# yxyxcyx/Real-Time-Recommendation-System-with-Feature-Store

Hardware: AMD Instinct MI355X
Metric: user-item pairs scored/sec (train) + top-K queries/sec, emb_dim=128 (higher is better)
Workload: dtype f32; 1 GPU; C2: MovieLens-1M two-tower train step, emb 128, batch 1024, 16 negatives, hidden [256,128], dropout 0.2, tau 0.05, Adam+clip; global_batch=1024, emb_dim=128, num_negatives=16, parallelism=dp1

## Files before the change

### include/rtrec_hip.h

```cpp
#ifndef RTREC_HIP_H
#define RTREC_HIP_H

#include <stddef.h>
#include <stdint.h>

#ifdef __cplusplus
extern "C" {
#endif

typedef enum {
    RT_OK = 0,
    RT_ERR_INVALID = -1,
    RT_ERR_UNSUPPORTED = -2,
    RT_ERR_WORKSPACE = -3,
    RT_ERR_HIP = -4
} rt_status;

typedef enum { RT_F32 = 0, RT_F16 = 1, RT_BF16 = 2 } rt_dtype;

typedef enum {
    RT_ACT_RELU = 0,
    RT_ACT_GELU = 1,
    RT_ACT_LEAKY_RELU = 2,
    RT_ACT_TANH = 3,
    RT_ACT_SIGMOID = 4,
    RT_ACT_NONE = 5
} rt_act;

int rt_abi_version(void);
const char* rt_status_string(int status);
const char* rt_last_error(void);

int rt_gather_rows(const void* table, int64_t row_begin, int64_t n_rows, int64_t row_bytes,
                   const int64_t* ids, int64_t n_ids, void* out, int32_t* oob_count, void* stream);

int rt_scatter_add_rows_f32(float* grad_table, int64_t n_rows, int dim, const int64_t* ids,
                            int64_t n_ids, const float* grad_out, int64_t padding_idx, void* stream);

int rt_l2_renorm_f32(float* x, int64_t n, int d, void* stream);

size_t rt_flatip_topk_workspace_bytes(int64_t nq, int64_t nx, int d, int dtype, int k);
int rt_flatip_topk(const void* queries, int64_t nq, const void* items, int64_t nx, int d, int dtype,
                   int k, const uint32_t* exclude_bits, int64_t exclude_words, int64_t id_offset,
                   float* out_scores, int64_t* out_ids, void* workspace, size_t workspace_bytes,
                   void* stream);

size_t rt_flatip_topk_shard_workspace_bytes(int64_t nq, int64_t nx, int d, int dtype, int k);
int rt_flatip_topk_shard_plan(int64_t nq, int64_t nx, int d, int dtype, int k, int stride, int64_t* stage_counts);
int rt_flatip_topk_shard_sample(const void* queries, int64_t nq, const void* items, int64_t nx, int d, int dtype,
                                int k, int stride, float* top32, int64_t* stage_counts, void* workspace,
                                size_t workspace_bytes, void* stream);
int rt_topk_sample_rank(int k, int64_t sampled_stages, int64_t stages, int* rank);
int rt_topk_sample_threshold(const float* lists, int n_lists, int64_t nq, int rank, float* thr, void* stream);
int rt_flatip_topk_shard_search(const void* queries, int64_t nq, const void* items, int64_t nx, int d, int dtype,
                                int k, const float* thr, int64_t id_offset, float* out_scores, int64_t* out_ids,
                                void* workspace, size_t workspace_bytes, void* stream);

int rt_flatip_topk_tuning(int v4_mode, int v4_stride, int v4_rank);

int rt_l2_augment_f32(const float* x, int64_t n, int d, float* out, int ld_out, int role, void* stream);
int rt_l2_finish_f32(const float* q_aug, int ld_q, const float* x_aug, int ld_x, int d, int64_t nq, int k_sel,
                     const int64_t* sel_ids, const float* sel_scores, int k, float* scores, int64_t* ids,
                     int32_t* unverified, int64_t id_offset, void* stream);

int rt_topk_merge(const float* scores, const int64_t* ids, int64_t nq, int n_lists, int k_in,
                  int k_out, float* out_scores, int64_t* out_ids, void* stream);

int rt_sample_negatives(const int64_t* pos_offsets, const int32_t* pos_items, int64_t n_users,
                        const int64_t* users, int64_t n, int64_t num_items, int num_neg, uint64_t seed,
                        const uint64_t* seed_offset, int64_t* out, void* stream);

int rt_feeder_batch(const int64_t* order, const int64_t* inter_u, const int64_t* inter_m, const int64_t* state,
                    int64_t batch, int64_t* users, int64_t* pos, void* stream);
int rt_feeder_commit(const double* loss, double* losses, int64_t n_losses, int64_t* state, void* stream);

#ifndef RT_STAT_SLOTS
#define RT_STAT_SLOTS 8
#endif
#if RT_STAT_SLOTS > 15
#error "RT_STAT_SLOTS > 15: the host arenas (rtrec_amd/models/fused.py STAT_SLOTS) hold 16 slot rows, one of them for ticket counters"
#endif

typedef struct {
    const float* src;
    int64_t src_rows;
    int ld_src;
    const int64_t* ids;
    int64_t m;
    int k;
    int n;
    const float* w;
    const float* bias;
    int prev_mode;
    int prev_act;
    const double* prev_stats;
    const float* bn_gamma;
    const float* bn_beta;
    float* running_mean;
    float* running_var;
    float* save_mean;
    float* save_invstd;
    float bn_eps;
    float bn_momentum;
    float drop_p;
    uint64_t drop_seed;
    const uint64_t* seed_offset;
    float* z_out;
    int act;
    double* stats_out;
    float* l2_out;
    float* norms_out;
    int64_t* num_batches_tracked;
    int64_t seg_split;
    double* zero_buf;
    int64_t zero_words;
    float* wt_out;
    float* a_out;
    float* fin_save_mean;
    float* fin_save_invstd;
    float* fin_running_mean;
    float* fin_running_var;
    int64_t* fin_num_batches_tracked;
    float fin_eps;
    float fin_momentum;
    int prev_final;
    const uint16_t* w_planes;
    uint16_t* wt_planes_out;
    const float* next_w;
    uint16_t* next_w_planes;
    int next_n;
    int next_k;
} rt_linear_fwd_args;

int rt_linear_fwd_f32(const rt_linear_fwd_args* args, void* stream);

typedef struct {
    int64_t m; int k; int n;
    const float* w;
    float* dw;
    float* dbias;
    float* dz_ws;
    int grad_mode;
    const float* dout;
    const float* l2_out;
    const float* norms;
    const float* g;
    const float* z;
    int act;
    const double* g_stats;
    const float* save_mean;
    const float* save_invstd;
    const float* bn_gamma;
    float* dgamma;
    float* dbeta;
    const float* src; int64_t src_rows; int ld_src; const int64_t* ids;
    int prev_mode; int prev_act;
    const float* prev_mean; const float* prev_invstd;
    const float* prev_gamma; const float* prev_beta;
    float prev_drop_p; uint64_t prev_drop_seed; const uint64_t* seed_offset;
    float* g_prev;
    double* g_prev_stats;
    float* dsrc;
    int64_t seg_split;
    double* dbias_slots;
    const float* wt;
    int fuse_dz;
    const float* a_in;
    float* dw_part;
    const float* fold_src;
    float* fold_dst;
    int64_t fold_words;
    int fold_splits;
    int fold_in;
    const uint16_t* wt_planes;
} rt_linear_bwd_args;

int rt_linear_bwd_f32(const rt_linear_bwd_args* args, void* stream);
int rt_linear_bwd_dz_fused(const rt_linear_bwd_args* args, int n_args);
int rt_linear_bwd_dw_splits(const rt_linear_bwd_args* args, int n_args, int64_t* splits);
int rt_linear_bwd_dz_f32(const rt_linear_bwd_args* args, void* stream);
int rt_linear_bwd_dw_f32(const rt_linear_bwd_args* args, void* stream);
int rt_linear_fwd_f32_multi(const rt_linear_fwd_args* args, int n_args, void* stream);
int rt_linear_bwd_dz_f32_multi(const rt_linear_bwd_args* args, int n_args, void* stream);
int rt_linear_bwd_dw_f32_multi(const rt_linear_bwd_args* args, int n_args, void* stream);

size_t rt_twotower_loss_workspace_bytes(int64_t b, int d);
int rt_twotower_loss_fwd_bwd(const void* u, const void* p, const void* q, int dtype, int64_t b,
                             int d, int n_neg, float inv_tau, const float* user_bias,
                             const float* item_bias, float w_explicit, float w_in_batch,
                             double* loss_out, float* du, float* dp, float* dq, float* d_user_bias,
                             float* d_item_bias, void* workspace, size_t workspace_bytes, void* stream);

int rt_twotower_loss_fwd(const void* u, const void* p, const void* q, int dtype, int64_t b, int d,
                         int n_neg, float inv_tau, const float* user_bias, const float* item_bias,
                         float w_explicit, float w_in_batch, double* loss_out, void* workspace,
                         size_t workspace_bytes, void* stream);

size_t rt_inbatch_loss_workspace_bytes(int64_t b, int64_t n_items, int d);
int rt_inbatch_loss_fwd_bwd(const void* u, const void* p, int dtype, int64_t b, int64_t n_items, int d,
                            int64_t label_offset, float inv_tau, double* loss_out, float* du, float* dp,
                            void* workspace, size_t workspace_bytes, void* stream);

int rt_similarity_f32(const float* u, const float* v, int64_t b, int d, float inv_tau,
                      const float* user_bias, const float* item_bias, float* out, void* stream);

int rt_grad_sqnorm(const float* grads, const int64_t* offsets, int n_tensors, double* sumsq_out,
                   int32_t* step_counter, int64_t* seed_counter, void* stream);
int rt_clip_adam_step(float* params, float* grads, float* exp_avg, float* exp_avg_sq,
                      int64_t n, const double* sumsq, int n_tensors, float max_norm, float lr,
                      const float* lr_dev, float beta1, float beta2, float eps, float weight_decay,
                      int step, const int32_t* step_dev, double* zero_buf, int64_t zero_words,
                      void* stream);

#define RT_METRICS_MAX_K 16

int rt_exclusion_bitmap(const int64_t* offsets, const int32_t* items, int64_t n_csr_rows, const int64_t* rows,
                        int64_t n_rows, int64_t n_items, uint32_t* bits, int64_t words, void* stream);
int rt_rank_metrics(const int64_t* preds, int64_t n_rows, int list_len, const int64_t* gt_offsets,
                    const int32_t* gt_items, const int64_t* gt_rows, int64_t n_gt_rows,
                    const int64_t* ex_offsets, const int32_t* ex_items, const int64_t* ex_rows,
                    int64_t n_ex_rows, const int32_t* k_values, int n_k, int64_t num_items,
                    double* per_row, int32_t* valid, uint32_t* coverage_bits, void* stream);
int rt_rank_metrics_reduce(const double* per_row, const int32_t* valid, int64_t n_rows, int n_cols,
                           const uint32_t* coverage_bits, int64_t num_items, double* out, void* stream);

#ifdef __cplusplus
}
#endif

#endif
```

### real-time-recommendation-system-with-feature-store_amd/csrc/mlp.hip

```cpp
#include "rt_common.h"
#include "split3.h"

namespace rt {
namespace mlp {

typedef float f32x16 __attribute__((ext_vector_type(16)));



constexpr float kNormEps = 1e-12f;

struct FwdLaunch {
    rt_linear_fwd_args a0, a1;
    unsigned split;
};
struct BwdLaunch {
    rt_linear_bwd_args a0, a1;
    unsigned split;
    int64_t rps0, rps1;
    unsigned tn0, tk0, tn1, tk1;
    bool vec0, vec1;
    int ngroups;
    unsigned ksplit = 1;
};

constexpr int kFoldG = 8;
__device__ __forceinline__ void fold_side(const BwdLaunch& L, int which) {
    const int64_t nt = static_cast<int64_t>(gridDim.x) * blockDim.x;
    const int64_t gt = static_cast<int64_t>(blockIdx.x) * blockDim.x + threadIdx.x;
    for (int g = 0; g < L.ngroups; ++g) {
        const rt_linear_bwd_args& f = g ? L.a1 : L.a0;
        if (!f.fold_src || f.fold_in != which || f.fold_splits <= 0) continue;
        const int64_t n4 = f.fold_words / 4;
        const int ng = (f.fold_splits + kFoldG - 1) / kFoldG;
        for (int64_t it = gt; it < n4 * ng; it += nt) {
            const int64_t e = it % n4;
            const int s0 = static_cast<int>(it / n4) * kFoldG;
            float4 v[kFoldG];
#pragma unroll
            for (int j = 0; j < kFoldG; ++j)
                v[j] = s0 + j < f.fold_splits
                           ? reinterpret_cast<const float4*>(f.fold_src + static_cast<int64_t>(s0 + j) * f.fold_words)[e]
                           : make_float4(0.f, 0.f, 0.f, 0.f);
            float4 t = v[0];
#pragma unroll
            for (int j = 1; j < kFoldG; ++j) { t.x += v[j].x; t.y += v[j].y; t.z += v[j].z; t.w += v[j].w; }
            float* d = f.fold_dst + 4 * e;
            if (ng == 1) {
                const float4 o = *reinterpret_cast<const float4*>(d);
                *reinterpret_cast<float4*>(d) = make_float4(o.x + t.x, o.y + t.y, o.z + t.z, o.w + t.w);
            } else {
                atomicAdd(d, t.x); atomicAdd(d + 1, t.y); atomicAdd(d + 2, t.z); atomicAdd(d + 3, t.w);
            }
        }
    }
}


#ifdef RT_PHASE_PROBE
__device__ unsigned long long* g_probe_buf = nullptr;
__device__ unsigned int g_probe_ctr[64];
__device__ unsigned int g_probe_cap = 0;
struct PhaseProbe {
    uint64_t rt0 = 0, t0 = 0, m[4] = {0, 0, 0, 0};
    __device__ __forceinline__ void start() {
        if (threadIdx.x == 0) {
            rt0 = __builtin_amdgcn_s_memrealtime();
            t0 = __builtin_amdgcn_s_memtime();
        }
    }
    __device__ __forceinline__ void mark(int i) {
        if (threadIdx.x == 0) m[i] = __builtin_amdgcn_s_memtime() - t0;
    }
    __device__ __forceinline__ void end(unsigned tag) {
        if (threadIdx.x == 0) {
            asm volatile("s_waitcnt vmcnt(0)" ::: "memory");
            m[3] = __builtin_amdgcn_s_memtime() - t0;
            const uint64_t rt1 = __builtin_amdgcn_s_memrealtime();
            const unsigned xcc = __builtin_amdgcn_s_getreg((20) | (0 << 6) | ((4 - 1) << 11));
            const unsigned sh = blockIdx.x & 63u;
            const unsigned slot = atomicAdd(&g_probe_ctr[sh], 1u);
            if (slot < g_probe_cap && g_probe_buf) {
                unsigned long long* o = g_probe_buf + (static_cast<uint64_t>(slot) * 64 + sh) * 8;
                o[0] = (static_cast<uint64_t>(tag) << 32) | blockIdx.x;
                o[1] = rt0; o[2] = m[0]; o[3] = m[1]; o[4] = m[2]; o[5] = m[3]; o[6] = rt1; o[7] = xcc;
            }
        }
    }
};
#define RT_PP_DECL PhaseProbe pp_; pp_.start();
#define RT_PP_MARK(i) pp_.mark(i);
#define RT_PP_END(tag) pp_.end(tag);
#else
#define RT_PP_DECL
#define RT_PP_MARK(i)
#define RT_PP_END(tag)
#endif

#if !defined(RT_NO_WT_STORES)
#define RT_WT_STORES 1
#endif
__device__ __forceinline__ void st_act(float* p, float v) {
#ifdef RT_WT_STORES
    __hip_atomic_store(p, v, __ATOMIC_RELAXED, __HIP_MEMORY_SCOPE_AGENT);
#else
    *p = v;
#endif
}
__device__ __forceinline__ void st_act4(float* p, float4 v) {
#ifdef RT_WT_STORES
    typedef float f4v __attribute__((ext_vector_type(4)));
    const f4v x = {v.x, v.y, v.z, v.w};
    asm volatile("global_store_dwordx4 %0, %1, off sc1" ::"v"(p), "v"(x) : "memory");
#else
    *reinterpret_cast<float4*>(p) = v;
#endif
}

__device__ __forceinline__ f32x16 mfma(float a, float b, f32x16 c) {
    return __builtin_amdgcn_mfma_f32_32x32x2f32(a, b, c, 0, 0, 0);
}

using fsplit::Pieces;
using fsplit::s16x8;
using fsplit::split8;
using fsplit::mfma3;
using fsplit::split3;

struct Pro {
    int mode;
    int act;
    float drop_p, drop_scale;
    uint64_t seed;
    const float* scale;
    const float* shift;
};

__device__ __forceinline__ float pro_apply(const Pro& p, int64_t r, int c, float v) {
    if (p.mode == 0) return v;
    v = act_eval(p.act, v);
    if (p.mode != 3) v = __builtin_fmaf(v, p.scale[c], p.shift[c]);
    if (p.drop_p > 0.f) v = dropout_keep(p.seed, r, c, p.drop_p) ? v * p.drop_scale : 0.f;
    return v;
}

__device__ __forceinline__ void slot_sums(const double* __restrict__ base, int w, int c, double& s1, double& s2) {
    double v1[RT_STAT_SLOTS], v2[RT_STAT_SLOTS];
#pragma unroll
    for (int sl = 0; sl < RT_STAT_SLOTS; ++sl) {
        v1[sl] = base[static_cast<int64_t>(sl) * 2 * w + c];
        v2[sl] = base[static_cast<int64_t>(sl) * 2 * w + w + c];
    }
    s1 = 0.0;
    s2 = 0.0;
#pragma unroll
    for (int sl = 0; sl < RT_STAT_SLOTS; ++sl) {
        s1 += v1[sl];
        s2 += v2[sl];
    }
}

__device__ __forceinline__ void bn_affine(float gamma, float beta, float mean, float invstd, float& scale,
                                          float& shift) {
    scale = gamma * invstd;
    shift = __builtin_fmaf(-mean, scale, beta);
}

__device__ __forceinline__ void ticket_release() {
#ifdef RT_TICKET_WBL2
    __builtin_amdgcn_fence(__ATOMIC_RELEASE, "agent");
#endif
    asm volatile("s_waitcnt vmcnt(0)" ::: "memory");
}

__device__ __forceinline__ void bn_finalize_last(const rt_linear_fwd_args& a, unsigned nblk) {
    __shared__ int last_s;
    const int tid = threadIdx.x, n = a.n;
    const bool two = a.seg_split > 0;
    const int nseg = two ? 2 : 1;
    asm volatile("s_waitcnt vmcnt(0)" ::: "memory");
    __syncthreads();
    if (tid == 0) {
        ticket_release();
        unsigned long long* cnt =
            reinterpret_cast<unsigned long long*>(a.stats_out + static_cast<int64_t>(nseg) * RT_STAT_SLOTS * 2 * n);
        last_s = atomicAdd(cnt, 1ull) == static_cast<unsigned long long>(nblk) - 1ull ? 1 : 0;
    }
    __syncthreads();
    if (!last_s) return;
    for (int c = tid; c < n; c += blockDim.x) {
        for (int sg = 0; sg < nseg; ++sg) {
            const int64_t ms = two ? (sg == 0 ? a.seg_split : a.m - a.seg_split) : a.m;
            double* ps = a.stats_out + static_cast<int64_t>(sg) * RT_STAT_SLOTS * 2 * n;
            double v1[RT_STAT_SLOTS], v2[RT_STAT_SLOTS];
#pragma unroll
            for (int sl = 0; sl < RT_STAT_SLOTS; ++sl) {
                v1[sl] = atomicAdd(&ps[static_cast<int64_t>(sl) * 2 * n + c], 0.0);
                v2[sl] = atomicAdd(&ps[static_cast<int64_t>(sl) * 2 * n + n + c], 0.0);
            }
            double s1 = 0.0, s2 = 0.0;
#pragma unroll
            for (int sl = 0; sl < RT_STAT_SLOTS; ++sl) {
                s1 += v1[sl];
                s2 += v2[sl];
            }
            const double md = s1 / static_cast<double>(ms);
            double vd = s2 / static_cast<double>(ms) - md * md;
            vd = vd > 0.0 ? vd : 0.0;
            const float mean = static_cast<float>(md);
            const float invstd = static_cast<float>(1.0 / sqrt(vd + static_cast<double>(a.fin_eps)));
            const float var_f = static_cast<float>(ms > 1 ? vd * static_cast<double>(ms) / static_cast<double>(ms - 1) : vd);
            a.fin_save_mean[sg * n + c] = mean;
            if (a.fin_save_invstd) a.fin_save_invstd[sg * n + c] = invstd;
            if (a.fin_running_mean) {
                const float mo = a.fin_momentum;
                a.fin_running_mean[c] = (1.f - mo) * a.fin_running_mean[c] + mo * mean;
                a.fin_running_var[c] = (1.f - mo) * a.fin_running_var[c] + mo * var_f;
            }
        }
    }
    if (tid == 0 && a.fin_num_batches_tracked) *a.fin_num_batches_tracked += nseg;
}

constexpr int FM = 32;

__host__ __device__ __forceinline__ int pad8(int k) { return (k + 31) / 32 * 32; }

template <int TPW, bool KVEC, bool WPL>
__global__ __launch_bounds__(256) __attribute__((amdgpu_waves_per_eu(TPW == 1 ? 3 : 2))) void linear_fwd_kernel(FwdLaunch L) {
    static_assert(!WPL || (TPW == 1 && KVEC), "split-weight planes: one-tile waves, k % 4 == 0");
    const bool g1 = blockIdx.x >= L.split;
    const rt_linear_fwd_args& a = g1 ? L.a1 : L.a0;
    const unsigned bid = blockIdx.x - (g1 ? L.split : 0u);
    constexpr int NT = 4 * TPW;
    extern __shared__ __attribute__((aligned(16))) float sm[];
    const int k = a.k, n = a.n;
    const int kp = pad8(k), aplane = FM * kp, aw = 3 * aplane / 2;
    const int nch = kp / 8, am = ((nch & -nch) < 16 ? (nch & -nch) : 16) - 1;
    float* scale = sm;
    float* shift = scale + kp;
    float* As = shift + kp;
    uint16_t* const Ap = reinterpret_cast<uint16_t*>(As);
    float* rowpart = As + aw;
    int64_t* srow = reinterpret_cast<int64_t*>(rowpart + NT * FM);

    const int tid = threadIdx.x, lane = tid & 63, w = tid >> 6, h = lane >> 5, c32 = lane & 31;
    const int64_t row0 = static_cast<int64_t>(bid) * FM;
    const int64_t m = a.m;
    auto put_a = [&](int r, int c, float4 o) {
        if (a.a_out && c < k && row0 + r < m) st_act4(a.a_out + (row0 + r) * k + c, o);
        uint32_t h0, m0, l0, h1, m1, l1;
        split3(o.x, o.y, h0, m0, l0);
        split3(o.z, o.w, h1, m1, l1);
        uint16_t* q = Ap + r * kp + ((((c >> 3) ^ (r & am)) << 3) | (c & 7));
        *reinterpret_cast<uint2*>(q) = make_uint2(h0, h1);
        *reinterpret_cast<uint2*>(q + aplane) = make_uint2(m0, m1);
        *reinterpret_cast<uint2*>(q + 2 * aplane) = make_uint2(l0, l1);
    };
    RT_PP_DECL
    if (blockIdx.x == 0 && a.zero_buf)
        for (int64_t e = tid; e < a.zero_words; e += 256) a.zero_buf[e] = 0.0;

    const int vpr = kp / 4;
    const bool vec = (a.ld_src % 4) == 0 && (reinterpret_cast<uintptr_t>(a.src) & 15) == 0;
    const bool fast = vec && (a.k % 4) == 0 && (256 % vpr) == 0 &&
                      (a.prev_mode == 0 || act_is_piecewise_linear(a.prev_act));
    const bool early = fast && !a.ids && 8 * (256 / vpr) >= FM;
    if (a.wt_out) {
        const int tk = (k + 31) / 32, tiles = tk * ((n + 31) / 32);
        const int nblk = static_cast<int>(g1 ? gridDim.x - L.split : L.split);
        for (int wt = static_cast<int>(bid); wt < tiles; wt += nblk) {
            const int n0 = (wt / tk) * 32, k0 = (wt % tk) * 32;
            const int r = tid >> 3, c = (tid & 7) * 4;
            if (n0 + r < n) {
#pragma unroll
                for (int j = 0; j < 4; ++j)
                    if (k0 + c + j < k) a.wt_out[static_cast<int64_t>(k0 + c + j) * n + n0 + r] = a.w[static_cast<int64_t>(n0 + r) * k + k0 + c + j];
            }
        }
    }
    if (a.wt_planes_out || a.next_w_planes) {
        const int nblk = static_cast<int>(g1 ? gridDim.x - L.split : L.split);
        if (a.wt_planes_out) {
            const int64_t plane = static_cast<int64_t>(n) * k;
            const int nq = (n + 3) / 4;
            for (int64_t e = static_cast<int64_t>(bid) * 256 + tid; e < static_cast<int64_t>(k) * nq;
                 e += static_cast<int64_t>(nblk) * 256) {
                const int kk = static_cast<int>(e / nq), n0 = static_cast<int>(e % nq) * 4;
                float x[4];
#pragma unroll
                for (int j = 0; j < 4; ++j) x[j] = n0 + j < n ? a.w[static_cast<int64_t>(n0 + j) * k + kk] : 0.f;
                uint32_t h0, m0, l0, h1, m1, l1;
                split3(x[0], x[1], h0, m0, l0);
                split3(x[2], x[3], h1, m1, l1);
                uint16_t* q = a.wt_planes_out + static_cast<int64_t>(kk) * n + n0;
                if (n0 + 4 <= n && (n % 4) == 0) {
                    *reinterpret_cast<uint2*>(q) = make_uint2(h0, h1);
                    *reinterpret_cast<uint2*>(q + plane) = make_uint2(m0, m1);
                    *reinterpret_cast<uint2*>(q + 2 * plane) = make_uint2(l0, l1);
                } else {
                    const uint32_t hv[2] = {h0, h1}, mv[2] = {m0, m1}, lv[2] = {l0, l1};
                    for (int j = 0; j < 4 && n0 + j < n; ++j) {
                        const int sh = 16 * (j & 1);
                        q[j] = static_cast<uint16_t>(hv[j >> 1] >> sh);
                        q[j + plane] = static_cast<uint16_t>(mv[j >> 1] >> sh);
                        q[j + 2 * plane] = static_cast<uint16_t>(lv[j >> 1] >> sh);
                    }
                }
            }
        }
        if (a.next_w_planes) {
            const int64_t tot8 = static_cast<int64_t>(a.next_n) * a.next_k / 8;
            const float4* src4 = reinterpret_cast<const float4*>(a.next_w);
            s16x8* dst = reinterpret_cast<s16x8*>(a.next_w_planes);
            for (int64_t e = static_cast<int64_t>(bid) * 256 + tid; e < tot8; e += static_cast<int64_t>(nblk) * 256) {
                const float4 u = src4[2 * e], v = src4[2 * e + 1];
                const float x[8] = {u.x, u.y, u.z, u.w, v.x, v.y, v.z, v.w};
                const Pieces pc = split8(x);
                dst[e] = pc.hi;
                dst[e + tot8] = pc.mid;
                dst[e + 2 * tot8] = pc.lo;
            }
        }
    }
    const float* wrow[TPW];
    bool tile_on[TPW], row_ok[TPW];
#pragma unroll
    for (int i = 0; i < TPW; ++i) {
        tile_on[i] = (w + 4 * i) * 32 < n;
        const int nn = (w + 4 * i) * 32 + c32;
        row_ok[i] = nn < n;
        wrow[i] = a.w + static_cast<int64_t>(row_ok[i] ? nn : 0) * k;
    }
    float4 wv[TPW][4], wn[TPW][4];
    auto load_w = [&](int s, float4 (&dst)[TPW][4]) {
#pragma unroll
        for (int i = 0; i < TPW; ++i)
#pragma unroll
            for (int j = 0; j < 4; ++j) {
                const int kk = s + 16 * (j >> 1) + 8 * h + 4 * (j & 1);
                float4 v = make_float4(0.f, 0.f, 0.f, 0.f);
                if (tile_on[i] && row_ok[i]) {
                    const float* wr = wrow[i] + kk;
                    if constexpr (KVEC) {
                        if (kk < k) v = *reinterpret_cast<const float4*>(wr);
                    } else {
                        if (kk < k) v.x = wr[0];
                        if (kk + 1 < k) v.y = wr[1];
                        if (kk + 2 < k) v.z = wr[2];
                        if (kk + 3 < k) v.w = wr[3];
                    }
                }
                dst[i][j] = v;
            }
    };
    uint4 pv[2][3], pn[2][3];
    const int64_t wplane = static_cast<int64_t>(n) * k;
    auto load_p = [&](int s, uint4 (&dst)[2][3]) {
#pragma unroll
        for (int b = 0; b < 2; ++b) {
            const int kk = s + 16 * b + 8 * h;
            const bool ok = tile_on[0] && row_ok[0] && kk < k;
            const uint16_t* q = a.w_planes + (static_cast<int64_t>(row_ok[0] ? w * 32 + c32 : 0) * k + (ok ? kk : 0));
#pragma unroll
            for (int p = 0; p < 3; ++p)
                dst[b][p] = ok ? *reinterpret_cast<const uint4*>(q + p * wplane) : make_uint4(0u, 0u, 0u, 0u);
        }
    };
    if constexpr (WPL) load_p(0, pn);
    else if constexpr (TPW == 1) load_w(0, wn);
    float4 pre[8];
    if (early) {
        const int c = (tid % vpr) * 4, rstep = 256 / vpr, r0 = tid / vpr;
#pragma unroll
        for (int u = 0; u < 8; ++u) {
            const int r = r0 + u * rstep;
            const int64_t gr = row0 + r;
            pre[u] = make_float4(0.f, 0.f, 0.f, 0.f);
            if (r < FM && c < k && gr < m && gr < a.src_rows)
                pre[u] = *reinterpret_cast<const float4*>(a.src + gr * a.ld_src + c);
        }
    }

    const bool two = a.seg_split > 0;
    const int my_seg = (two && row0 >= a.seg_split) ? 1 : 0;
    if (a.prev_mode == 1 && a.prev_final) {
        for (int c = tid; c < k; c += 256)
            bn_affine(a.bn_gamma[c], a.bn_beta[c], a.save_mean[my_seg * k + c], a.save_invstd[my_seg * k + c], scale[c],
                      shift[c]);
    } else if (a.prev_mode == 1 || a.prev_mode == 2) {
        const int nseg = two ? 2 : 1;
        for (int c = tid; c < k; c += 256) {
            for (int sg = 0; sg < nseg; ++sg) {
                if (bid != 0 && sg != my_seg) continue;
                const int64_t ms = two ? (sg == 0 ? a.seg_split : m - a.seg_split) : m;
                float mean, invstd, var_f = 0.f;
                if (a.prev_mode == 1) {
                    const double* ps = a.prev_stats + static_cast<int64_t>(sg) * RT_STAT_SLOTS * 2 * k;
                    double s1, s2;
                    slot_sums(ps, k, c, s1, s2);
                    const double md = s1 / static_cast<double>(ms);
                    double vd = s2 / static_cast<double>(ms) - md * md;
                    vd = vd > 0.0 ? vd : 0.0;
                    mean = static_cast<float>(md);
                    invstd = static_cast<float>(1.0 / sqrt(vd + static_cast<double>(a.bn_eps)));
                    var_f = static_cast<float>(ms > 1 ? vd * static_cast<double>(ms) / static_cast<double>(ms - 1) : vd);
                } else {
                    mean = a.running_mean[c];
                    invstd = static_cast<float>(1.0 / sqrt(static_cast<double>(a.running_var[c]) + a.bn_eps));
                }
                if (sg == my_seg) bn_affine(a.bn_gamma[c], a.bn_beta[c], mean, invstd, scale[c], shift[c]);
                if (bid == 0) {
                    if (c == 0 && a.prev_mode == 1 && a.num_batches_tracked) *a.num_batches_tracked += 1;
                    if (a.save_mean) a.save_mean[sg * k + c] = mean;
                    if (a.save_invstd) a.save_invstd[sg * k + c] = invstd;
                    if (a.prev_mode == 1 && a.running_mean) {
                        const float mo = a.bn_momentum;
                        a.running_mean[c] = (1.f - mo) * a.running_mean[c] + mo * mean;
                        a.running_var[c] = (1.f - mo) * a.running_var[c] + mo * var_f;
                    }
                }
            }
        }
    }
    RT_PP_MARK(0)
    if (tid < FM) {
        const int64_t gr = row0 + tid;
        int64_t sr = -1;
        if (gr < m) {
            sr = a.ids ? a.ids[gr] : gr;
            if (sr < 0 || sr >= a.src_rows) sr = -1;
        }
        srow[tid] = sr;
    }
    __syncthreads();
    const uint64_t seed = a.drop_seed + (a.seed_offset ? *a.seed_offset : 0ull);
    const Pro pro{a.prev_mode, a.prev_act, a.drop_p, a.drop_p > 0.f ? 1.f / (1.f - a.drop_p) : 1.f, seed,
                  scale, shift};
    {
        const int total = FM * vpr;
        if (fast) {
            const int c = (tid % vpr) * 4, rstep = 256 / vpr;
            const bool bn = pro.mode == 1 || pro.mode == 2;
            const float4 sc4 = bn ? *reinterpret_cast<const float4*>(scale + c) : make_float4(1.f, 1.f, 1.f, 1.f);
            const float4 sh4 = bn ? *reinterpret_cast<const float4*>(shift + c) : make_float4(0.f, 0.f, 0.f, 0.f);
            const float sl = act_slope(pro.act);
            const bool drop = pro.drop_p > 0.f;
            for (int r0 = tid / vpr; r0 < FM; r0 += 8 * rstep) {
                float4 v[8];
#pragma unroll
                for (int u = 0; u < 8; ++u) {
                    const int r = r0 + u * rstep;
                    v[u] = make_float4(0.f, 0.f, 0.f, 0.f);
                    if (early) {
                        v[u] = pre[u];
                    } else if (r < FM && c < k) {
                        const int64_t sr = srow[r];
                        if (sr >= 0) v[u] = *reinterpret_cast<const float4*>(a.src + sr * a.ld_src + c);
                    }
                }
#pragma unroll
                for (int u = 0; u < 8; ++u) {
                    const int r = r0 + u * rstep;
                    if (r >= FM) break;
                    const int64_t gr = row0 + r;
                    const bool ok = srow[r] >= 0 && c < k;
                    auto tf = [&](float x, int cc, float scv, float shv) {
                        if (pro.mode == 0) return x;
                        x = act_pwl(sl, x);
                        if (bn) x = __builtin_fmaf(x, scv, shv);
                        if (drop) x = dropout_keep(pro.seed, gr, cc, pro.drop_p) ? x * pro.drop_scale : 0.f;
                        return x;
                    };
                    float4 o;
                    o.x = ok ? tf(v[u].x, c, sc4.x, sh4.x) : 0.f;
                    o.y = ok ? tf(v[u].y, c + 1, sc4.y, sh4.y) : 0.f;
                    o.z = ok ? tf(v[u].z, c + 2, sc4.z, sh4.z) : 0.f;
                    o.w = ok ? tf(v[u].w, c + 3, sc4.w, sh4.w) : 0.f;
                    put_a(r, c, o);
                }
            }
        } else
        for (int base = tid; base < total; base += 256 * 4) {
            float4 v[4];
#pragma unroll
            for (int u = 0; u < 4; ++u) {
                const int e = base + u * 256;
                v[u] = make_float4(0.f, 0.f, 0.f, 0.f);
                if (e < total) {
                    const int r = e / vpr, c = (e - r * vpr) * 4;
                    const int64_t sr = srow[r];
                    if (sr >= 0 && c < k) {
                        const float* sp = a.src + sr * a.ld_src + c;
                        if (vec && c + 4 <= k) v[u] = *reinterpret_cast<const float4*>(sp);
                        else {
                            v[u].x = sp[0];
                            if (c + 1 < k) v[u].y = sp[1];
                            if (c + 2 < k) v[u].z = sp[2];
                            if (c + 3 < k) v[u].w = sp[3];
                        }
                    }
                }
            }
#pragma unroll
            for (int u = 0; u < 4; ++u) {
                const int e = base + u * 256;
                if (e < total) {
                    const int r = e / vpr, c = (e - r * vpr) * 4;
                    const bool ok = srow[r] >= 0;
                    const int64_t gr = row0 + r;
                    float4 o;
                    o.x = (ok && c < k) ? pro_apply(pro, gr, c, v[u].x) : 0.f;
                    o.y = (ok && c + 1 < k) ? pro_apply(pro, gr, c + 1, v[u].y) : 0.f;
                    o.z = (ok && c + 2 < k) ? pro_apply(pro, gr, c + 2, v[u].z) : 0.f;
                    o.w = (ok && c + 3 < k) ? pro_apply(pro, gr, c + 3, v[u].w) : 0.f;
                    put_a(r, c, o);
                }
            }
        }
    }
    __syncthreads();
    RT_PP_MARK(1)

    f32x16 acc[TPW];
#pragma unroll
    for (int i = 0; i < TPW; ++i) acc[i] = f32x16{};
    const uint16_t* ap = Ap + c32 * kp;
    const int asw = c32 & am;
    if constexpr (TPW != 1) load_w(0, wn);
    if constexpr (WPL) {
        for (int s = 0; s < kp; s += 32) {
#pragma unroll
            for (int b = 0; b < 2; ++b)
#pragma unroll
                for (int p = 0; p < 3; ++p) pv[b][p] = pn[b][p];
            if (s + 32 < kp) load_p(s + 32, pn);
#pragma unroll
            for (int b = 0; b < 2; ++b) {
                const int ao = (((s + 16 * b) >> 3) + h) ^ asw;
                Pieces pa;
                pa.hi = *reinterpret_cast<const s16x8*>(ap + 8 * ao);
                pa.mid = *reinterpret_cast<const s16x8*>(ap + aplane + 8 * ao);
                pa.lo = *reinterpret_cast<const s16x8*>(ap + 2 * aplane + 8 * ao);
                if (tile_on[0]) {
                    const Pieces pb{__builtin_bit_cast(s16x8, pv[b][0]), __builtin_bit_cast(s16x8, pv[b][1]),
                                    __builtin_bit_cast(s16x8, pv[b][2])};
                    acc[0] = mfma3(pa, pb, acc[0]);
                }
            }
        }
    } else
    for (int s = 0; s < kp; s += 32) {
#pragma unroll
        for (int i = 0; i < TPW; ++i)
#pragma unroll
            for (int j = 0; j < 4; ++j) wv[i][j] = wn[i][j];
        if (s + 32 < kp) load_w(s + 32, wn);
#pragma unroll
        for (int b = 0; b < 2; ++b) {
            const int ao = (((s + 16 * b) >> 3) + h) ^ asw;
            Pieces pa;
            pa.hi = *reinterpret_cast<const s16x8*>(ap + 8 * ao);
            pa.mid = *reinterpret_cast<const s16x8*>(ap + aplane + 8 * ao);
            pa.lo = *reinterpret_cast<const s16x8*>(ap + 2 * aplane + 8 * ao);
#pragma unroll
            for (int i = 0; i < TPW; ++i) {
                if (!tile_on[i]) continue;
                const float4 u = wv[i][2 * b], v = wv[i][2 * b + 1];
                const float x[8] = {u.x, u.y, u.z, u.w, v.x, v.y, v.z, v.w};
                acc[i] = mfma3(pa, split8(x), acc[i]);
            }
        }
    }

    RT_PP_MARK(2)
    const bool l2 = a.l2_out != nullptr;
    if (l2 && !a.z_out && !a.stats_out && n * (FM + 1) <= aw) {
        __syncthreads();
        float* zsq = As;
#pragma unroll
        for (int i = 0; i < TPW; ++i) {
            const int col = (w + 4 * i) * 32 + c32;
            if ((w + 4 * i) * 32 >= n) continue;
            const bool col_ok = col < n;
            const float b = (col_ok && a.bias) ? a.bias[col] : 0.f;
#pragma unroll
            for (int r = 0; r < 16; ++r) {
                const int lr = (r & 3) + 8 * (r >> 2) + 4 * h;
                const float z = acc[i][r] + b;
                acc[i][r] = z;
                if (col_ok) zsq[col * (FM + 1) + lr] = (row0 + lr < m) ? z * z : 0.f;
            }
        }
        __syncthreads();
        {
            const int row = tid >> 3, part = tid & 7;
            float ss = 0.f;
            for (int c = part; c < n; c += 8) ss += zsq[c * (FM + 1) + row];
            ss += __shfl_xor(ss, 1, 64);
            ss += __shfl_xor(ss, 2, 64);
            ss += __shfl_xor(ss, 4, 64);
            if (part == 0) {
                const float nrm = sqrtf(ss);
                rowpart[row] = 1.f / fmaxf(nrm, kNormEps);
                if (row0 + row < m && a.norms_out) a.norms_out[row0 + row] = nrm;
            }
        }
        __syncthreads();
#pragma unroll
        for (int i = 0; i < TPW; ++i) {
            const int col = (w + 4 * i) * 32 + c32;
            if ((w + 4 * i) * 32 >= n) continue;
#pragma unroll
            for (int r = 0; r < 16; ++r) {
                const int lr = (r & 3) + 8 * (r >> 2) + 4 * h;
                const int64_t gr = row0 + lr;
                if (gr < m && col < n) st_act(a.l2_out + gr * n + col, acc[i][r] * rowpart[lr]);
            }
        }
        RT_PP_END(1)
        return;
    }
    double* const stats = a.stats_out ? a.stats_out + (static_cast<int64_t>(my_seg) * RT_STAT_SLOTS +
                                                       bid % RT_STAT_SLOTS) * 2 * n : nullptr;
#pragma unroll
    for (int i = 0; i < TPW; ++i) {
        const int ct = w + 4 * i;
        const int col = ct * 32 + c32;
        const bool col_ok = col < n;
        const float b = (col_ok && a.bias) ? a.bias[col] : 0.f;
        float s1 = 0.f, s2 = 0.f;
        if (row0 + FM <= m && a.z_out && !l2 && act_is_piecewise_linear(a.act)) {
            if (ct * 32 >= n) continue;
            float* zp = a.z_out + (row0 + 4 * h) * n + col;
            const float sl = act_slope(a.act);
#pragma unroll
            for (int r = 0; r < 16; ++r) {
                const float z = acc[i][r] + b;
                if (col_ok) st_act(zp + ((r & 3) + 8 * (r >> 2)) * n, z);
                const float av = act_pwl(sl, z);
                s1 += av;
                s2 += av * av;
            }
            if (!col_ok) s1 = s2 = 0.f;
        } else
#pragma unroll
        for (int r = 0; r < 16; ++r) {
            const int lr = (r & 3) + 8 * (r >> 2) + 4 * h;
            const int64_t gr = row0 + lr;
            const float z = acc[i][r] + b;
            acc[i][r] = z;
            const bool ok = col_ok && gr < m;
            if (ok && a.z_out) st_act(a.z_out + gr * n + col, z);
            if (ok && stats) {
                const float av = act_eval(a.act, z);
                s1 += av;
                s2 += av * av;
            }
            if (l2) {
                float q = ok ? z * z : 0.f;
#pragma unroll
                for (int o = 1; o < 32; o <<= 1) q += __shfl_xor(q, o, 64);
                if (c32 == 0) rowpart[ct * FM + lr] = q;
            }
        }
        if (stats) {
            s1 += __shfl_xor(s1, 32, 64);
            s2 += __shfl_xor(s2, 32, 64);
            if (h == 0 && col_ok) {
                atomicAdd(&stats[col], static_cast<double>(s1));
                atomicAdd(&stats[n + col], static_cast<double>(s2));
            }
        }
    }
    if (stats && a.fin_save_mean) bn_finalize_last(a, g1 ? gridDim.x - L.split : L.split);
    if (l2) {
        __syncthreads();
        const int nt_used = (n + 31) / 32;
#pragma unroll
        for (int i = 0; i < TPW; ++i) {
            const int col = (w + 4 * i) * 32 + c32;
#pragma unroll
            for (int r = 0; r < 16; ++r) {
                const int lr = (r & 3) + 8 * (r >> 2) + 4 * h;
                const int64_t gr = row0 + lr;
                if (gr < m && col < n) {
                    float ss = 0.f;
                    for (int t = 0; t < nt_used; ++t) ss += rowpart[t * FM + lr];
                    const float nrm = sqrtf(ss);
                    a.l2_out[gr * n + col] = acc[i][r] / fmaxf(nrm, kNormEps);
                    if (col == 0 && a.norms_out) a.norms_out[gr] = nrm;
                }
            }
        }
    }
    RT_PP_END(1)
}

template <int TPWK, bool WPL, bool KS>
__global__ __launch_bounds__(256) __attribute__((amdgpu_waves_per_eu(3))) void linear_bwd_dz_kernel(BwdLaunch L) {
#ifdef RT_FOLD_FIRST
    fold_side(L, 0);
#endif
    const unsigned kpart = KS ? blockIdx.x % L.ksplit : 0u, bx = KS ? blockIdx.x / L.ksplit : blockIdx.x;
    const bool prim = kpart == 0;
    const int tb = static_cast<int>(kpart) * 4 * TPWK;
    const bool g1 = bx >= L.split;
    const rt_linear_bwd_args& a = g1 ? L.a1 : L.a0;
    const unsigned bid = bx - (g1 ? L.split : 0u);
    extern __shared__ __attribute__((aligned(16))) float sm[];
    const int n = a.n, k = a.k;
    const int64_t m = a.m;
    const int np = pad8(n), ldz = np + 4;
    float* Dz = sm;
    const int tid = threadIdx.x, lane = tid & 63, w = tid >> 6, h = lane >> 5, c32 = lane & 31;
    const int64_t row0 = static_cast<int64_t>(bid) * FM;
    const bool two = a.seg_split > 0;
    const int my_seg = (two && row0 >= a.seg_split) ? 1 : 0;
    const int64_t seg_m = two ? (my_seg == 0 ? a.seg_split : m - a.seg_split) : m;
    RT_PP_DECL

    float wv[TPWK][8], wn[TPWK][8];
    const float* __restrict__ Wt = a.w;
#ifdef RT_NO_WT_ROWS
    const float* __restrict__ WtT = nullptr;
#else
    const float* __restrict__ WtT = (a.wt && (n % 8) == 0) ? a.wt : nullptr;
#endif
    auto load_w = [&](int s, float (&dst)[TPWK][8]) {
#pragma unroll
        for (int i = 0; i < TPWK; ++i) {
            const int kk = (tb + w + 4 * i) * 32 + c32;
            const bool on = (tb + w + 4 * i) * 32 < k && kk < k;
            if (WtT) {
                const int nn = s + 8 * h;
                float4 v0 = make_float4(0.f, 0.f, 0.f, 0.f), v1 = v0;
                if (on && nn < n) {
                    const float* p = WtT + static_cast<int64_t>(kk) * n + nn;
                    v0 = *reinterpret_cast<const float4*>(p);
                    v1 = *reinterpret_cast<const float4*>(p + 4);
                }
                dst[i][0] = v0.x; dst[i][1] = v0.y; dst[i][2] = v0.z; dst[i][3] = v0.w;
                dst[i][4] = v1.x; dst[i][5] = v1.y; dst[i][6] = v1.z; dst[i][7] = v1.w;
            } else {
#pragma unroll
                for (int j = 0; j < 8; ++j) {
                    const int nn = s + 8 * h + j;
                    dst[i][j] = (on && nn < n) ? Wt[static_cast<int64_t>(nn) * k + kk] : 0.f;
                }
            }
        }
    };
    uint4 pv[TPWK][3], pn[TPWK][3];
    const uint16_t* __restrict__ WtP = a.wt_planes;
    const int64_t tplane = static_cast<int64_t>(k) * n;
    auto load_p = [&](int s, uint4 (&dst)[TPWK][3]) {
#pragma unroll
        for (int i = 0; i < TPWK; ++i) {
            const int kk = (tb + w + 4 * i) * 32 + c32;
            const int nn = s + 8 * h;
            const bool ok = (tb + w + 4 * i) * 32 < k && kk < k && nn < n;
            const uint16_t* q = WtP + (ok ? static_cast<int64_t>(kk) * n + nn : 0);
#pragma unroll
            for (int p = 0; p < 3; ++p)
                dst[i][p] = ok ? *reinterpret_cast<const uint4*>(q + p * tplane) : make_uint4(0u, 0u, 0u, 0u);
        }
    };
    if constexpr (TPWK == 1) {
        if (a.g_prev || a.dsrc) {
            if constexpr (WPL) load_p(0, pn);
            else load_w(0, wn);
        }
    }

    const int l4 = n / 4;
    if (a.grad_mode == 0 && (n % 4) == 0 && l4 <= 64 && (l4 & (l4 - 1)) == 0 && np == n) {
        const int rpp = 64 / l4, sub = lane / l4, li = lane % l4, c = 4 * li;
        float4 lv[8], dv[8];
        float nr[8];
#pragma unroll
        for (int p = 0; p < 8; ++p) {
            const int r = w * 8 + p * rpp + sub;
            const int64_t gr = row0 + r;
            lv[p] = make_float4(0.f, 0.f, 0.f, 0.f);
            dv[p] = lv[p];
            nr[p] = 1.f;
            if (p * rpp < 8 && gr < m) {
                lv[p] = *reinterpret_cast<const float4*>(a.l2_out + gr * n + c);
                dv[p] = *reinterpret_cast<const float4*>(a.dout + gr * n + c);
                nr[p] = a.norms[gr];
            }
        }
#pragma unroll
        for (int p = 0; p < 8; ++p) {
            if (p * rpp >= 8) break;
            const int r = w * 8 + p * rpp + sub;
            const int64_t gr = row0 + r;
            float dot = lv[p].x * dv[p].x + lv[p].y * dv[p].y + lv[p].z * dv[p].z + lv[p].w * dv[p].w;
            for (int o = 1; o < l4; o <<= 1) dot += __shfl_xor(dot, o, 64);
            const bool big = nr[p] > kNormEps;
            const float inv = 1.f / (big ? nr[p] : kNormEps);
            float4 d = make_float4(0.f, 0.f, 0.f, 0.f);
            if (gr < m) {
                d.x = big ? (dv[p].x - lv[p].x * dot) * inv : dv[p].x * inv;
                d.y = big ? (dv[p].y - lv[p].y * dot) * inv : dv[p].y * inv;
                d.z = big ? (dv[p].z - lv[p].z * dot) * inv : dv[p].z * inv;
                d.w = big ? (dv[p].w - lv[p].w * dot) * inv : dv[p].w * inv;
                if (prim) st_act4(a.dz_ws + gr * n + c, d);
            }
            *reinterpret_cast<float4*>(Dz + r * ldz + c) = d;
        }
    } else if (a.grad_mode == 0) {
        for (int rr = w * 8; rr < w * 8 + 8; ++rr) {
            const int64_t gr = row0 + rr;
            if (gr < m) {
                float dot = 0.f;
                for (int c = lane; c < n; c += 64) dot += a.l2_out[gr * n + c] * a.dout[gr * n + c];
                dot = wave_sum(dot);
                const float nrm = a.norms[gr];
                const bool big = nrm > kNormEps;
                const float inv = 1.f / (big ? nrm : kNormEps);
                for (int c = lane; c < np; c += 64) {
                    float dz = 0.f;
                    if (c < n) {
                        const float dv = a.dout[gr * n + c];
                        dz = big ? (dv - a.l2_out[gr * n + c] * dot) * inv : dv * inv;
                        if (prim) a.dz_ws[gr * n + c] = dz;
                    }
                    Dz[rr * ldz + c] = dz;
                }
            } else {
                for (int c = lane; c < np; c += 64) Dz[rr * ldz + c] = 0.f;
            }
        }
    } else {
        float* cA = Dz + FM * ldz;
        float* cB = cA + np;
        float* cC = cB + np;
        float* cM = cC + np;
        float* cI = cM + np;
        const float inv_m = 1.f / static_cast<float>(seg_m);
        const double* gst = a.g_stats ? a.g_stats + static_cast<int64_t>(my_seg) * RT_STAT_SLOTS * 2 * n : nullptr;
        const int vpr = np / 4;
        const bool vec = (n % 4) == 0;
        const bool fast = vec && (256 % vpr) == 0 && act_is_piecewise_linear(a.act) && a.grad_mode != 3;
        const bool early = fast && 8 * (256 / vpr) >= FM;
        float4 pg[8];
        if (early) {
            const int c = (tid % vpr) * 4, rstep = 256 / vpr, r0 = tid / vpr;
#pragma unroll
            for (int u = 0; u < 8; ++u) {
                const int r = r0 + u * rstep;
                const int64_t gr = row0 + r;
                pg[u] = make_float4(0.f, 0.f, 0.f, 0.f);
                if (r < FM && gr < m && c < n) pg[u] = *reinterpret_cast<const float4*>(a.g + gr * n + c);
            }
        }
        for (int c = tid; c < np; c += 256) {
            float A = 1.f, Bc = 0.f, C = 0.f, M = 0.f, I = 1.f;
            if (c < n && (a.grad_mode == 1 || a.grad_mode == 2)) {
                I = a.save_invstd[my_seg * n + c];
                M = a.save_mean[my_seg * n + c];
                A = a.bn_gamma[c] * I;
                if (a.grad_mode == 1) {
                    double gs1, gs2;
                    slot_sums(gst, n, c, gs1, gs2);
                    Bc = static_cast<float>(gs1) * inv_m;
                    C = static_cast<float>(gs2) * inv_m;
                }
            }
            cA[c] = A; cB[c] = Bc; cC[c] = C; cM[c] = M; cI[c] = I;
        }
        __syncthreads();
        const int total = FM * vpr;
        if (fast) {
            const int c = (tid % vpr) * 4, rstep = 256 / vpr;
            const float4 fA = *reinterpret_cast<const float4*>(cA + c), fB = *reinterpret_cast<const float4*>(cB + c);
            const float4 fC = *reinterpret_cast<const float4*>(cC + c), fM = *reinterpret_cast<const float4*>(cM + c);
            const float4 fI = *reinterpret_cast<const float4*>(cI + c);
            const float sl = act_slope(a.act);
            for (int r0 = tid / vpr; r0 < FM; r0 += 8 * rstep) {
                float4 gv[8], zv[8];
#pragma unroll
                for (int u = 0; u < 8; ++u) {
                    const int r = r0 + u * rstep;
                    const int64_t gr = row0 + r;
                    gv[u] = make_float4(0.f, 0.f, 0.f, 0.f);
                    zv[u] = gv[u];
                    if (early) {
                        gv[u] = pg[u];
                        if (r < FM && gr < m && c < n) zv[u] = *reinterpret_cast<const float4*>(a.z + gr * n + c);
                    } else if (r < FM && gr < m && c < n) {
                        gv[u] = *reinterpret_cast<const float4*>(a.g + gr * n + c);
                        zv[u] = *reinterpret_cast<const float4*>(a.z + gr * n + c);
                    }
                }
#pragma unroll
                for (int u = 0; u < 8; ++u) {
                    const int r = r0 + u * rstep;
                    if (r >= FM) break;
                    const int64_t gr = row0 + r;
                    auto one = [&](float g, float z, float A, float B, float C, float M, float I) {
                        const float xh = (act_pwl(sl, z) - M) * I;
                        return A * (g - B - xh * C) * (z > 0.f ? 1.f : sl);
                    };
                    float4 d;
                    d.x = one(gv[u].x, zv[u].x, fA.x, fB.x, fC.x, fM.x, fI.x);
                    d.y = one(gv[u].y, zv[u].y, fA.y, fB.y, fC.y, fM.y, fI.y);
                    d.z = one(gv[u].z, zv[u].z, fA.z, fB.z, fC.z, fM.z, fI.z);
                    d.w = one(gv[u].w, zv[u].w, fA.w, fB.w, fC.w, fM.w, fI.w);
                    if (gr >= m || c >= n) d = make_float4(0.f, 0.f, 0.f, 0.f);
                    *reinterpret_cast<float4*>(Dz + r * ldz + c) = d;
                    if (prim && gr < m && c < n) st_act4(a.dz_ws + gr * n + c, d);
                }
            }
        } else
        for (int base = tid; base < total; base += 256 * 4) {
            float4 gv[4], zv[4];
#pragma unroll
            for (int u = 0; u < 4; ++u) {
                const int e = base + u * 256;
                gv[u] = make_float4(0.f, 0.f, 0.f, 0.f);
                zv[u] = gv[u];
                if (e < total) {
                    const int r = e / vpr, c = (e - r * vpr) * 4;
                    const int64_t gr = row0 + r;
                    if (gr < m && c < n) {
                        const int64_t off = gr * n + c;
                        if (vec) {
                            gv[u] = *reinterpret_cast<const float4*>(a.g + off);
                            zv[u] = *reinterpret_cast<const float4*>(a.z + off);
                        } else {
                            gv[u].x = a.g[off]; zv[u].x = a.z[off];
                            if (c + 1 < n) { gv[u].y = a.g[off + 1]; zv[u].y = a.z[off + 1]; }
                            if (c + 2 < n) { gv[u].z = a.g[off + 2]; zv[u].z = a.z[off + 2]; }
                            if (c + 3 < n) { gv[u].w = a.g[off + 3]; zv[u].w = a.z[off + 3]; }
                        }
                    }
                }
            }
#pragma unroll
            for (int u = 0; u < 4; ++u) {
                const int e = base + u * 256;
                if (e >= total) continue;
                const int r = e / vpr, c = (e - r * vpr) * 4;
                const int64_t gr = row0 + r;
                float dzv[4];
                const float gs[4] = {gv[u].x, gv[u].y, gv[u].z, gv[u].w};
                const float zs[4] = {zv[u].x, zv[u].y, zv[u].z, zv[u].w};
#pragma unroll
                for (int j = 0; j < 4; ++j) {
                    const int cc = c + j;
                    float dz = 0.f;
                    if (gr < m && cc < n) {
                        const float xh = (act_eval(a.act, zs[j]) - cM[cc]) * cI[cc];
                        const float dr = (a.grad_mode == 3) ? gs[j] : cA[cc] * (gs[j] - cB[cc] - xh * cC[cc]);
                        dz = dr * act_grad_eval(a.act, zs[j]);
                    }
                    dzv[j] = dz;
                }
                *reinterpret_cast<float4*>(Dz + r * ldz + c) = make_float4(dzv[0], dzv[1], dzv[2], dzv[3]);
                if (prim && gr < m && c < n) {
                    const int64_t off = gr * n + c;
                    if (vec) *reinterpret_cast<float4*>(a.dz_ws + off) = make_float4(dzv[0], dzv[1], dzv[2], dzv[3]);
                    else
                        for (int j = 0; j < 4 && c + j < n; ++j) a.dz_ws[off + j] = dzv[j];
                }
            }
        }
    }
    RT_PP_MARK(0)
    if (prim && a.dbias && a.dbias_slots) {
        __syncthreads();
        double* sl = a.dbias_slots + static_cast<int64_t>(bid % RT_STAT_SLOTS) * n;
        for (int c = tid; c < n; c += 256) {
            float cs = 0.f;
#pragma unroll 8
            for (int r = 0; r < FM; ++r) cs += Dz[r * ldz + c];
            atomicAdd(&sl[c], static_cast<double>(cs));
        }
    }
    if (prim && bid == 0 && (a.grad_mode == 1 || a.grad_mode == 2) && a.dgamma) {
        for (int c = tid; c < n; c += 256) {
            for (int sg = 0; sg < (two ? 2 : 1); ++sg) {
                const double* gs = a.g_stats + static_cast<int64_t>(sg) * RT_STAT_SLOTS * 2 * n;
                double gs1, gs2;
                slot_sums(gs, n, c, gs1, gs2);
                atomicAdd(&a.dgamma[c], static_cast<float>(gs2));
                atomicAdd(&a.dbeta[c], static_cast<float>(gs1));
            }
        }
    }
    if (!a.g_prev && !a.dsrc) {
#ifndef RT_FOLD_FIRST
        fold_side(L, 0);
#endif
        RT_PP_END(2)
        return;
    }
    __syncthreads();
    RT_PP_MARK(1)

    const int ldb = np + 8;
    uint16_t* const planes = reinterpret_cast<uint16_t*>(Dz + FM * ldz + 5 * np);
    const int plane = FM * ldb;
    for (int e = tid; e < FM * (np / 4); e += 256) {
        const int r = e / (np / 4), c = (e - r * (np / 4)) * 4;
        const float4 v = *reinterpret_cast<const float4*>(Dz + r * ldz + c);
        uint32_t h0, m0, l0, h1, m1, l1;
        split3(v.x, v.y, h0, m0, l0);
        split3(v.z, v.w, h1, m1, l1);
        uint16_t* q = planes + r * ldb + c;
        *reinterpret_cast<uint2*>(q) = make_uint2(h0, h1);
        *reinterpret_cast<uint2*>(q + plane) = make_uint2(m0, m1);
        *reinterpret_cast<uint2*>(q + 2 * plane) = make_uint2(l0, l1);
    }
    __syncthreads();
    f32x16 acc[TPWK];
#pragma unroll
    for (int i = 0; i < TPWK; ++i) acc[i] = f32x16{};
    const uint16_t* ap = planes + c32 * ldb + 8 * h;
    const bool want_stats = a.g_prev && a.g_prev_stats && (a.prev_mode == 1 || a.prev_mode == 2);
    const bool fast = row0 + FM <= m && !a.dsrc && a.g_prev && act_is_piecewise_linear(a.prev_act);
    float zpre[TPWK][16], pmean[TPWK], pinv[TPWK];
#pragma unroll
    for (int i = 0; i < TPWK; ++i) {
        const int kk = (tb + w + 4 * i) * 32 + c32;
        const bool ld = fast && want_stats && kk < k;
        pmean[i] = ld ? a.prev_mean[my_seg * k + kk] : 0.f;
        pinv[i] = ld ? a.prev_invstd[my_seg * k + kk] : 0.f;
        const float* zp = a.src + (row0 + 4 * h) * a.ld_src + kk;
#pragma unroll
        for (int r = 0; r < 16; ++r) zpre[i][r] = ld ? zp[((r & 3) + 8 * (r >> 2)) * a.ld_src] : 0.f;
    }
    if constexpr (WPL) {
        if constexpr (TPWK != 1) load_p(0, pn);
        for (int s = 0; s < np; s += 16) {
#pragma unroll
            for (int i = 0; i < TPWK; ++i)
#pragma unroll
                for (int p = 0; p < 3; ++p) pv[i][p] = pn[i][p];
            if (s + 16 < np) load_p(s + 16, pn);
            Pieces pa;
            pa.hi = *reinterpret_cast<const s16x8*>(ap + s);
            pa.mid = *reinterpret_cast<const s16x8*>(ap + plane + s);
            pa.lo = *reinterpret_cast<const s16x8*>(ap + 2 * plane + s);
#pragma unroll
            for (int i = 0; i < TPWK; ++i) {
                if ((tb + w + 4 * i) * 32 >= k) continue;
                const Pieces pb{__builtin_bit_cast(s16x8, pv[i][0]), __builtin_bit_cast(s16x8, pv[i][1]),
                                __builtin_bit_cast(s16x8, pv[i][2])};
                acc[i] = mfma3(pa, pb, acc[i]);
            }
        }
    } else {
    if constexpr (TPWK != 1) load_w(0, wn);
    for (int s = 0; s < np; s += 16) {
#pragma unroll
        for (int i = 0; i < TPWK; ++i)
#pragma unroll
            for (int j = 0; j < 8; ++j) wv[i][j] = wn[i][j];
        if (s + 16 < np) load_w(s + 16, wn);
        Pieces pa;
        pa.hi = *reinterpret_cast<const s16x8*>(ap + s);
        pa.mid = *reinterpret_cast<const s16x8*>(ap + plane + s);
        pa.lo = *reinterpret_cast<const s16x8*>(ap + 2 * plane + s);
#pragma unroll
        for (int i = 0; i < TPWK; ++i) {
            if ((tb + w + 4 * i) * 32 >= k) continue;
            acc[i] = mfma3(pa, split8(wv[i]), acc[i]);
        }
    }
    }
    RT_PP_MARK(2)
    const float pscale = a.prev_drop_p > 0.f ? 1.f / (1.f - a.prev_drop_p) : 1.f;
    const uint64_t pseed = a.prev_drop_seed + (a.seed_offset ? *a.seed_offset : 0ull);
    double* const gps = want_stats ? a.g_prev_stats + (static_cast<int64_t>(my_seg) * RT_STAT_SLOTS +
                                                        bid % RT_STAT_SLOTS) * 2 * k : nullptr;
    const float psl = act_slope(a.prev_act);
#pragma unroll
    for (int i = 0; i < TPWK; ++i) {
        const int kk = (tb + w + 4 * i) * 32 + c32;
        const bool col_ok = kk < k;
        float s1 = 0.f, s2 = 0.f;
        if ((tb + w + 4 * i) * 32 >= k) continue;
        if (fast) {
            const int64_t rb = row0 + 4 * h;
            float* gp = a.g_prev + rb * k + kk;
            const float* zv = zpre[i];
            const float pm = pmean[i], pi = pinv[i];
            const bool drop = a.prev_drop_p > 0.f;
#pragma unroll
            for (int r = 0; r < 16; ++r) {
                const int lr = (r & 3) + 8 * (r >> 2);
                float gv = acc[i][r];
                if (drop) gv = dropout_keep(pseed, rb + lr, kk, a.prev_drop_p) ? gv * pscale : 0.f;
                if (col_ok) st_act(gp + lr * k, gv);
                const float xh = (act_pwl(psl, zv[r]) - pm) * pi;
                s1 += gv;
                s2 += gv * xh;
            }
            if (!want_stats || !col_ok) s1 = s2 = 0.f;
        } else
#pragma unroll
        for (int r = 0; r < 16; ++r) {
            const int64_t gr = row0 + (r & 3) + 8 * (r >> 2) + 4 * h;
            if (gr < m && col_ok) {
                const float da = acc[i][r];
                if (a.dsrc) a.dsrc[gr * k + kk] = da;
                if (a.g_prev) {
                    float gv = da;
                    if (a.prev_drop_p > 0.f)
                        gv = dropout_keep(pseed, gr, kk, a.prev_drop_p) ? da * pscale : 0.f;
                    a.g_prev[gr * k + kk] = gv;
                    if (want_stats) {
                        const float xh = (act_eval(a.prev_act, a.src[gr * a.ld_src + kk]) -
                                          a.prev_mean[my_seg * k + kk]) * a.prev_invstd[my_seg * k + kk];
                        s1 += gv;
                        s2 += gv * xh;
                    }
                }
            }
        }
        if (want_stats) {
            s1 += __shfl_xor(s1, 32, 64);
            s2 += __shfl_xor(s2, 32, 64);
            if (h == 0 && col_ok) {
                atomicAdd(&gps[kk], static_cast<double>(s1));
                atomicAdd(&gps[k + kk], static_cast<double>(s2));
            }
        }
    }
#ifndef RT_FOLD_FIRST
    fold_side(L, 0);
#endif
    RT_PP_END(2)
}

constexpr int DW_R = 32;
constexpr int DW_G = 2;
constexpr int DW_NT = 256 * DW_G;
constexpr int DW_MAXR = 2048;

__host__ __device__ constexpr int dw_ld(int x) { return x + ((x / 32) % 2 == 0 ? 32 : 0); }

template <int PRO>
__device__ __forceinline__ float pro_col(const Pro& p, float slope, int64_t r, int c, float sc, float sh, float v) {
    if constexpr (PRO == 0) {
        return v;
    } else {
        if constexpr (PRO == 3) v = act_eval(p.act, v);
        else v = act_pwl(slope, v);
        v = __builtin_fmaf(v, sc, sh);
        if constexpr (PRO == 2) v = dropout_keep(p.seed, r, c, p.drop_p) ? v * p.drop_scale : 0.f;
        if constexpr (PRO == 3) {
            if (p.drop_p > 0.f) v = dropout_keep(p.seed, r, c, p.drop_p) ? v * p.drop_scale : 0.f;
        }
        return v;
    }
}

template <int BN, int BK, int PRO, bool VEC, bool DZF>
__global__ __launch_bounds__(DW_NT) void linear_bwd_dw_kernel(BwdLaunch L) {
    constexpr int NTN = BN / 32, WK = 4 / NTN, T = (BK / 32) / WK;
    static_assert(NTN * 32 == BN && 4 % NTN == 0 && T >= 1 && T * WK * 32 == BK, "dW tile");
    constexpr int LDN = dw_ld(BN), LDK = dw_ld(BK);
    constexpr int VN = BN / 4, VK = BK / 4;
    constexpr int LN = (DW_R * VN + DW_NT - 1) / DW_NT, LK = (DW_R * VK + DW_NT - 1) / DW_NT;
    static_assert(DW_NT % VN == 0 && DW_NT % VK == 0, "fixed staging columns per thread");
    static_assert(2 * DW_R * LDN >= 4 * T * 16 * 64, "row-group reduction fits in the dz buffers");
    static_assert(2 * DW_R * LDK >= (DW_NT / 64) * VN * 4, "dbias partials fit in the A buffers");
    __shared__ __attribute__((aligned(16))) float Ld[2][DW_R * LDN];
    __shared__ __attribute__((aligned(16))) float La[2][DW_R * LDK];
    __shared__ int srow[PRO == 0 ? DW_MAXR : 1];
    __shared__ __attribute__((aligned(16))) float aff_s[2][2][BK];
    __shared__ __attribute__((aligned(16))) float dzc_s[DZF ? 2 : 1][5][DZF ? BN : 4];

#ifdef RT_FOLD_FIRST
    fold_side(L, 1);
#endif
    const bool g1 = blockIdx.x >= L.split;
    const rt_linear_bwd_args a = g1 ? L.a1 : L.a0;
    const int64_t rows_per_split = g1 ? L.rps1 : L.rps0;
    const unsigned bid = blockIdx.x - (g1 ? L.split : 0u);
    const unsigned tn = g1 ? L.tn1 : L.tn0, tk = g1 ? L.tk1 : L.tk0;
    const unsigned bx = bid % tn, by = (bid / tn) % tk, bz = bid / (tn * tk);
    const int n = a.n, k = a.k;
    const int64_t m = a.m;
    const int tid = threadIdx.x, lane = tid & 63, wg = tid >> 6, w = wg & 3, grp = wg >> 2, h = lane >> 5,
              c = lane & 31;
    const int n0 = static_cast<int>(bx) * BN, k0 = static_cast<int>(by) * BK;
    const int64_t r_begin = static_cast<int64_t>(bz) * rows_per_split;
    const int64_t r_end = (r_begin + rows_per_split) < m ? (r_begin + rows_per_split) : m;
    if (r_begin >= m) {
#ifndef RT_FOLD_FIRST
        fold_side(L, 1);
#endif
        return;
    }
    RT_PP_DECL
    const bool gather = PRO == 0 && a.ids != nullptr && !a.a_in;
    const float* const asrc = a.a_in ? a.a_in : a.src;
    const int64_t ald = a.a_in ? static_cast<int64_t>(k) : static_cast<int64_t>(a.ld_src);
    const bool two = a.seg_split > 0;

    const int cn = (tid % VN) * 4, ck = (tid % VK) * 4;
    const int gn = n0 + cn, gk = k0 + ck;
    float4 sc0 = make_float4(1.f, 1.f, 1.f, 1.f), sc1 = sc0;
    float4 sh0 = make_float4(0.f, 0.f, 0.f, 0.f), sh1 = sh0;
    if ((a.prev_mode == 1 || a.prev_mode == 2) && !a.a_in) {
        if (tid < 2 * BK) {
            const int sg = tid / BK, cl = tid % BK, cc = k0 + cl;
            const int so = two ? sg * k : 0;
            float scv = 1.f, shv = 0.f;
            if (cc < k) bn_affine(a.prev_gamma[cc], a.prev_beta[cc], a.prev_mean[so + cc], a.prev_invstd[so + cc], scv, shv);
            aff_s[sg][0][cl] = scv;
            aff_s[sg][1][cl] = shv;
        }
        __syncthreads();
        sc0 = *reinterpret_cast<const float4*>(&aff_s[0][0][ck]);
        sh0 = *reinterpret_cast<const float4*>(&aff_s[0][1][ck]);
        sc1 = *reinterpret_cast<const float4*>(&aff_s[1][0][ck]);
        sh1 = *reinterpret_cast<const float4*>(&aff_s[1][1][ck]);
    }
    const uint64_t pseed = a.prev_drop_seed + (a.seed_offset ? *a.seed_offset : 0ull);
    const Pro pro{a.prev_mode, a.prev_act, a.prev_drop_p, a.prev_drop_p > 0.f ? 1.f / (1.f - a.prev_drop_p) : 1.f,
                  pseed, nullptr, nullptr};
    const float slope = act_slope(a.prev_act);
    if constexpr (DZF) {
        if (tid < 2 * BN) {
            const int sg = tid / BN, cl = tid % BN, c = n0 + cl;
            const int my = two ? sg : 0;
            const int64_t seg_m = two ? (my == 0 ? a.seg_split : m - a.seg_split) : m;
            float A = 1.f, Bc = 0.f, C = 0.f, M = 0.f, I = 1.f;
            if (c < n && (a.grad_mode == 1 || a.grad_mode == 2)) {
                I = a.save_invstd[my * n + c];
                M = a.save_mean[my * n + c];
                A = a.bn_gamma[c] * I;
                if (a.grad_mode == 1) {
                    double gs1, gs2;
                    slot_sums(a.g_stats + static_cast<int64_t>(my) * RT_STAT_SLOTS * 2 * n, n, c, gs1, gs2);
                    const float inv_m = 1.f / static_cast<float>(seg_m);
                    Bc = static_cast<float>(gs1) * inv_m;
                    C = static_cast<float>(gs2) * inv_m;
                }
            }
            dzc_s[sg][0][cl] = A; dzc_s[sg][1][cl] = Bc; dzc_s[sg][2][cl] = C;
            dzc_s[sg][3][cl] = M; dzc_s[sg][4][cl] = I;
        }
        if (bid == 0 && (a.grad_mode == 1 || a.grad_mode == 2) && a.dgamma) {
            for (int c = tid; c < n; c += DW_NT) {
                for (int sg = 0; sg < (two ? 2 : 1); ++sg) {
                    double gs1, gs2;
                    slot_sums(a.g_stats + static_cast<int64_t>(sg) * RT_STAT_SLOTS * 2 * n, n, c, gs1, gs2);
                    atomicAdd(&a.dgamma[c], static_cast<float>(gs2));
                    atomicAdd(&a.dbeta[c], static_cast<float>(gs1));
                }
            }
        }
        __syncthreads();
    }
    if (!DZF && a.dbias && a.dbias_slots && bid == 0) {
        for (int cc = tid; cc < n; cc += DW_NT) {
            double v = 0.0;
#pragma unroll
            for (int sl = 0; sl < RT_STAT_SLOTS; ++sl) v += a.dbias_slots[static_cast<int64_t>(sl) * n + cc];
            atomicAdd(&a.dbias[cc], static_cast<float>(v));
        }
    }
    const bool do_bias = a.dbias != nullptr && (DZF || a.dbias_slots == nullptr) && by == 0;
    const bool slot_bias = DZF && do_bias && a.dbias_slots != nullptr;

    if (gather) {
        for (int64_t t = tid; t < r_end - r_begin; t += DW_NT) {
            const int64_t id = a.ids[r_begin + t];
            srow[t] = (id < 0 || id >= a.src_rows) ? -1 : static_cast<int>(id);
        }
        __syncthreads();
    }

    float4 rd[LN], rz[DZF ? LN : 1], ra[LK];
    float4 bsum = make_float4(0.f, 0.f, 0.f, 0.f);
    const float dsl = act_slope(a.act);
    auto load = [&](int64_t base) {
#pragma unroll
        for (int j = 0; j < LN; ++j) {
            const int e = tid + DW_NT * j, row = e / VN;
            const int64_t r = base + row;
            float4 v = make_float4(0.f, 0.f, 0.f, 0.f);
            if constexpr (DZF) {
                float4 zv = v;
                if (e < DW_R * VN && r < r_end && gn < n) {
                    v = *reinterpret_cast<const float4*>(a.g + r * n + gn);
                    zv = *reinterpret_cast<const float4*>(a.z + r * n + gn);
                }
                rd[j] = v;
                rz[j] = zv;
                continue;
            }
            if (e < DW_R * VN && r < r_end) {
                const float* dz = a.dz_ws + r * n + gn;
                if constexpr (VEC) {
                    if (gn < n) v = *reinterpret_cast<const float4*>(dz);
                } else {
                    if (gn < n) v.x = dz[0];
                    if (gn + 1 < n) v.y = dz[1];
                    if (gn + 2 < n) v.z = dz[2];
                    if (gn + 3 < n) v.w = dz[3];
                }
            }
            rd[j] = v;
        }
#pragma unroll
        for (int j = 0; j < LK; ++j) {
            const int e = tid + DW_NT * j, row = e / VK;
            const int64_t r = base + row;
            float4 v = make_float4(0.f, 0.f, 0.f, 0.f);
            if (e < DW_R * VK && r < r_end) {
                const int64_t sr = gather ? srow[r - r_begin] : r;
                if (sr >= 0) {
                    const float* ap = asrc + sr * ald + gk;
                    if constexpr (VEC) {
                        if (gk < k) v = *reinterpret_cast<const float4*>(ap);
                    } else {
                        if (gk < k) v.x = ap[0];
                        if (gk + 1 < k) v.y = ap[1];
                        if (gk + 2 < k) v.z = ap[2];
                        if (gk + 3 < k) v.w = ap[3];
                    }
                }
            }
            ra[j] = v;
        }
    };
    auto store = [&](int buf, int64_t base) {
#pragma unroll
        for (int j = 0; j < LN; ++j) {
            const int e = tid + DW_NT * j, row = e / VN;
            if (e < DW_R * VN) {
                if constexpr (DZF) {
                    const int64_t r = base + row;
                    const int sg = (two && r >= a.seg_split) ? 1 : 0;
                    const bool ok = r < r_end;
                    float4 d;
                    auto one = [&](float g, float z, int i) {
                        const int cl = cn + i;
                        const float A = dzc_s[sg][0][cl], Bc = dzc_s[sg][1][cl], C = dzc_s[sg][2][cl];
                        const float M = dzc_s[sg][3][cl], I = dzc_s[sg][4][cl];
                        const float xh = (act_pwl(dsl, z) - M) * I;
                        return (ok && gn + i < n) ? A * (g - Bc - xh * C) * (z > 0.f ? 1.f : dsl) : 0.f;
                    };
                    d.x = one(rd[j].x, rz[j].x, 0);
                    d.y = one(rd[j].y, rz[j].y, 1);
                    d.z = one(rd[j].z, rz[j].z, 2);
                    d.w = one(rd[j].w, rz[j].w, 3);
                    rd[j] = d;
                }
                *reinterpret_cast<float4*>(&Ld[buf][row * LDN + cn]) = rd[j];
                bsum.x += rd[j].x; bsum.y += rd[j].y; bsum.z += rd[j].z; bsum.w += rd[j].w;
            }
        }
#pragma unroll
        for (int j = 0; j < LK; ++j) {
            const int e = tid + DW_NT * j, row = e / VK;
            if (e < DW_R * VK) {
                const int64_t r = base + row;
                const bool ok = r < r_end && (!gather || srow[r - r_begin] >= 0);
                const bool hi_seg = two && r >= a.seg_split;
                const float4 scs = hi_seg ? sc1 : sc0, shs = hi_seg ? sh1 : sh0;
                float4 v;
                v.x = (ok && gk < k) ? pro_col<PRO>(pro, slope, r, gk, scs.x, shs.x, ra[j].x) : 0.f;
                v.y = (ok && gk + 1 < k) ? pro_col<PRO>(pro, slope, r, gk + 1, scs.y, shs.y, ra[j].y) : 0.f;
                v.z = (ok && gk + 2 < k) ? pro_col<PRO>(pro, slope, r, gk + 2, scs.z, shs.z, ra[j].z) : 0.f;
                v.w = (ok && gk + 3 < k) ? pro_col<PRO>(pro, slope, r, gk + 3, scs.w, shs.w, ra[j].w) : 0.f;
                *reinterpret_cast<float4*>(&La[buf][row * LDK + ck]) = v;
            }
        }
    };

    f32x16 acc[T];
#pragma unroll
    for (int t = 0; t < T; ++t) acc[t] = f32x16{};
    const int ncol = (w % NTN) * 32 + c;
    const int kcol0 = (w / NTN) * T * 32 + c;
    int buf = 0;
    RT_PP_MARK(0)
    load(r_begin);
    store(0, r_begin);
    __syncthreads();
    RT_PP_MARK(1)
    for (int64_t base = r_begin; base < r_end; base += DW_R) {
        const bool more = base + DW_R < r_end;
        if (more) load(base + DW_R);
        const float* dl = &Ld[buf][(2 * grp + h) * LDN + ncol];
        const float* al = &La[buf][(2 * grp + h) * LDK + kcol0];
#pragma unroll
        for (int i = 0; i < DW_R / (2 * DW_G); ++i) {
            const float av = dl[2 * DW_G * i * LDN];
#pragma unroll
            for (int t = 0; t < T; ++t) acc[t] = mfma(av, al[2 * DW_G * i * LDK + 32 * t], acc[t]);
        }
        if (more) store(buf ^ 1, base + DW_R);
        __syncthreads();
        buf ^= 1;
    }

    RT_PP_MARK(2)
    float* red = &Ld[0][0];
    float* bred = &La[0][0];
    if (do_bias) {
#pragma unroll
        for (int o = VN; o < 64; o <<= 1) {
            bsum.x += __shfl_xor(bsum.x, o, 64);
            bsum.y += __shfl_xor(bsum.y, o, 64);
            bsum.z += __shfl_xor(bsum.z, o, 64);
            bsum.w += __shfl_xor(bsum.w, o, 64);
        }
        if (lane < VN) *reinterpret_cast<float4*>(&bred[(wg * VN + lane) * 4]) = bsum;
    }
#pragma unroll
    for (int t = 0; t < T; ++t)
#pragma unroll
        for (int r = 0; r < 16; ++r)
            if ((r >> 3) != grp) red[((w * T + t) * 16 + r) * 64 + lane] = acc[t][r];
    __syncthreads();
    if (do_bias && tid < VN) {
        float4 sb = make_float4(0.f, 0.f, 0.f, 0.f);
#pragma unroll
        for (int o = 0; o < DW_NT / 64; ++o) {
            const float4 v = *reinterpret_cast<const float4*>(&bred[(o * VN + tid) * 4]);
            sb.x += v.x; sb.y += v.y; sb.z += v.z; sb.w += v.w;
        }
        const int cb = n0 + tid * 4;
        if (slot_bias) {
            double* sl = a.dbias_slots + static_cast<int64_t>(bz % RT_STAT_SLOTS) * n;
            if (cb < n) atomicAdd(&sl[cb], static_cast<double>(sb.x));
            if (cb + 1 < n) atomicAdd(&sl[cb + 1], static_cast<double>(sb.y));
            if (cb + 2 < n) atomicAdd(&sl[cb + 2], static_cast<double>(sb.z));
            if (cb + 3 < n) atomicAdd(&sl[cb + 3], static_cast<double>(sb.w));
        } else {
            if (cb < n) atomicAdd(&a.dbias[cb], sb.x);
            if (cb + 1 < n) atomicAdd(&a.dbias[cb + 1], sb.y);
            if (cb + 2 < n) atomicAdd(&a.dbias[cb + 2], sb.z);
            if (cb + 3 < n) atomicAdd(&a.dbias[cb + 3], sb.w);
        }
    }
    auto add_row = [&](int t, int r, int kk) {
        const int nn = n0 + (w % NTN) * 32 + (r & 3) + 8 * (r >> 2) + 4 * h;
        const float v = acc[t][r] + red[((w * T + t) * 16 + r) * 64 + lane];
        if (nn < n) {
            if (a.dw_part) {
#ifdef RT_DW_PART_PLAIN
                a.dw_part[(static_cast<int64_t>(bz) * n + nn) * k + kk] = v;
#else
                st_act(a.dw_part + (static_cast<int64_t>(bz) * n + nn) * k + kk, v);
#endif
            }
            else atomicAdd(&a.dw[static_cast<int64_t>(nn) * k + kk], v);
        }
    };
#pragma unroll
    for (int t = 0; t < T; ++t) {
        const int kk = k0 + kcol0 + 32 * t;
        if (kk >= k) continue;
#pragma unroll
        for (int r = 0; r < 16; ++r)
            if ((r >> 3) == grp) add_row(t, r, kk);
    }
    if (slot_bias) {
        __shared__ int last_s;
        asm volatile("s_waitcnt vmcnt(0)" ::: "memory");
        __syncthreads();
        if (tid == 0) {
            ticket_release();
            unsigned long long* cnt = reinterpret_cast<unsigned long long*>(a.dbias_slots + static_cast<int64_t>(RT_STAT_SLOTS) * n);
            const unsigned long long nsplit = static_cast<unsigned long long>((m + rows_per_split - 1) / rows_per_split);
            last_s = atomicAdd(&cnt[bx], 1ull) == nsplit - 1 ? 1 : 0;
        }
        __syncthreads();
        if (last_s) {
            for (int cl = tid; cl < BN; cl += DW_NT) {
                const int c = n0 + cl;
                if (c >= n) continue;
                double v = 0.0;
#pragma unroll
                for (int sl = 0; sl < RT_STAT_SLOTS; ++sl) v += atomicAdd(&a.dbias_slots[static_cast<int64_t>(sl) * n + c], 0.0);
                atomicAdd(&a.dbias[c], static_cast<float>(v));
            }
        }
    }
#ifndef RT_FOLD_FIRST
    fold_side(L, 1);
#endif
    RT_PP_END(3)
}

}
}

using namespace rt;

template <typename K>
static void allow_lds(K kernel, size_t bytes) {
    static size_t set = 0;
    if (bytes > set) {
        (void)hipFuncSetAttribute(reinterpret_cast<const void*>(kernel), hipFuncAttributeMaxDynamicSharedMemorySize,
                            static_cast<int>(bytes));
        set = bytes;
    }
}

static int validate_fwd(const rt_linear_fwd_args* args) {
    if (!args) return RT_ERR_INVALID;
    const rt_linear_fwd_args& a = *args;
    if (a.m < 0 || a.k <= 0 || a.n <= 0 || !a.src || !a.w || a.ld_src < a.k) return RT_ERR_INVALID;
    if (a.n > 512 || a.k > 8192) return RT_ERR_UNSUPPORTED;
    if (a.prev_mode < 0 || a.prev_mode > 3) return RT_ERR_INVALID;
    if (a.seg_split < 0 || (a.seg_split > 0 && (a.seg_split >= a.m || a.seg_split % mlp::FM != 0)))
        return RT_ERR_INVALID;
    if (a.prev_mode == 1 && (!a.prev_stats || !a.bn_gamma || !a.bn_beta)) return RT_ERR_INVALID;
    if (a.prev_mode == 2 && (!a.running_mean || !a.running_var || !a.bn_gamma || !a.bn_beta)) return RT_ERR_INVALID;
    if (a.a_out && ((a.k % 4) != 0 || (reinterpret_cast<uintptr_t>(a.a_out) & 15) != 0)) return RT_ERR_INVALID;
    if (a.fin_save_mean && (!a.stats_out || !a.fin_save_invstd || (!a.fin_running_mean != !a.fin_running_var)))
        return RT_ERR_INVALID;
    if (a.prev_final && (a.prev_mode != 1 || !a.save_mean || !a.save_invstd)) return RT_ERR_INVALID;
    if (a.w_planes && ((a.k % 8) != 0 || a.n > 128 || (reinterpret_cast<uintptr_t>(a.w_planes) & 15) ||
                       (reinterpret_cast<uintptr_t>(a.w) & 15)))
        return RT_ERR_INVALID;
    if (a.next_w_planes && (!a.next_w || a.next_n <= 0 || a.next_k <= 0 || (a.next_k % 8) != 0 ||
                            (reinterpret_cast<uintptr_t>(a.next_w) & 15) ||
                            (reinterpret_cast<uintptr_t>(a.next_w_planes) & 15)))
        return RT_ERR_INVALID;
    const int kp = mlp::pad8(a.k);
    const int tpw = a.n <= 128 ? 1 : a.n <= 256 ? 2 : 4;
    const size_t lds = (2 * kp + 3 * mlp::FM * kp / 2 + 4 * tpw * mlp::FM) * sizeof(float) + mlp::FM * sizeof(int64_t) + 16;
    if (lds > 160 * 1024) return RT_ERR_UNSUPPORTED;
    return RT_OK;
}

extern "C" int rt_linear_fwd_f32_multi(const rt_linear_fwd_args* args, int n_args, void* stream) {
    if (!args || n_args < 1 || n_args > 2) return RT_ERR_INVALID;
#ifdef RT_NO_AIN
    rt_linear_fwd_args noa[2];
    for (int g = 0; g < n_args; ++g) { noa[g] = args[g]; noa[g].a_out = nullptr; }
    args = noa;
#endif
    int tpw = 1, kp_max = 0;
    bool kvec = true, wpl = true;
    unsigned blocks[2] = {0u, 0u};
    for (int g = 0; g < n_args; ++g) {
        const int v = validate_fwd(&args[g]);
        if (v) return v;
        const rt_linear_fwd_args& a = args[g];
        wpl = wpl && a.w_planes != nullptr;
        const int t = a.n <= 128 ? 1 : a.n <= 256 ? 2 : 4;
        tpw = t > tpw ? t : tpw;
        kvec = kvec && (a.k % 4) == 0 && (reinterpret_cast<uintptr_t>(a.w) & 15) == 0;
        const int kp = mlp::pad8(a.k);
        kp_max = kp > kp_max ? kp : kp_max;
        blocks[g] = static_cast<unsigned>((a.m + mlp::FM - 1) / mlp::FM);
    }
    const size_t lds = (2 * kp_max + 3 * mlp::FM * kp_max / 2 + 4 * tpw * mlp::FM) * sizeof(float) +
                       mlp::FM * sizeof(int64_t) + 16;
    if (lds > 160 * 1024) return RT_ERR_UNSUPPORTED;
    mlp::FwdLaunch L{};
    L.a0 = args[0];
    L.a1 = n_args > 1 ? args[1] : args[0];
    L.split = blocks[0];
    const unsigned total = blocks[0] + (n_args > 1 ? blocks[1] : 0u);
    if (total == 0) return RT_OK;
    hipStream_t st = as_stream(stream);
    const dim3 grid(total);
#define RT_FWD(T, V, P)                                                                           \
    do {                                                                                          \
        allow_lds(mlp::linear_fwd_kernel<T, V, P>, lds);                                          \
        hipLaunchKernelGGL((mlp::linear_fwd_kernel<T, V, P>), grid, dim3(256), lds, st, L);       \
    } while (0)
    if (kvec && tpw == 1 && wpl) {
        RT_FWD(1, true, true);
    } else if (kvec) {
        if (tpw == 1) RT_FWD(1, true, false); else if (tpw == 2) RT_FWD(2, true, false); else RT_FWD(4, true, false);
    } else {
        if (tpw == 1) RT_FWD(1, false, false); else if (tpw == 2) RT_FWD(2, false, false); else RT_FWD(4, false, false);
    }
#undef RT_FWD
    return check_launch("linear_fwd_kernel");
}

extern "C" int rt_linear_fwd_f32(const rt_linear_fwd_args* args, void* stream) {
    return rt_linear_fwd_f32_multi(args, 1, stream);
}

static bool dz_fusable(const rt_linear_bwd_args& a) {
#ifdef RT_NO_DZ_FUSE
    return false;
#endif
    return a.fuse_dz && !a.g_prev && !a.dsrc && a.grad_mode >= 1 && a.grad_mode <= 3 &&
           act_is_piecewise_linear(a.act) && (a.n % 4) == 0 && a.g && a.z &&
           (reinterpret_cast<uintptr_t>(a.g) & 15) == 0 && (reinterpret_cast<uintptr_t>(a.z) & 15) == 0;
}
static bool all_dz_fusable(const rt_linear_bwd_args* args, int n_args) {
    for (int g = 0; g < n_args; ++g)
        if (!dz_fusable(args[g])) return false;
    return true;
}

static int validate_bwd(const rt_linear_bwd_args* args) {
    if (!args) return RT_ERR_INVALID;
    const rt_linear_bwd_args& a = *args;
    if (a.m < 0 || a.k <= 0 || a.n <= 0 || !a.w || !a.dw || !a.dz_ws || !a.src || a.ld_src < a.k)
        return RT_ERR_INVALID;
    const bool need_da = a.g_prev || a.dsrc;
    if (a.n > 2048 || (need_da && a.k > 512)) return RT_ERR_UNSUPPORTED;
    if (a.grad_mode == 0 && (!a.dout || !a.l2_out || !a.norms)) return RT_ERR_INVALID;
    if (a.grad_mode >= 1 && a.grad_mode <= 3 && (!a.g || !a.z)) return RT_ERR_INVALID;
    if ((a.grad_mode == 1 || a.grad_mode == 2) && (!a.g_stats || !a.save_mean || !a.save_invstd || !a.bn_gamma))
        return RT_ERR_INVALID;
    if (a.grad_mode < 0 || a.grad_mode > 3) return RT_ERR_INVALID;
    if (a.seg_split < 0 || (a.seg_split > 0 && (a.seg_split >= a.m || a.seg_split % mlp::FM != 0)))
        return RT_ERR_INVALID;
    if ((a.prev_mode == 1 || a.prev_mode == 2) &&
        (!a.prev_mean || !a.prev_invstd || !a.prev_gamma || !a.prev_beta))
        return RT_ERR_INVALID;
    if (a.fold_src && (!a.fold_dst || a.fold_words % 4 != 0 || a.fold_splits <= 0 || a.fold_in < 0 || a.fold_in > 1 ||
                       (reinterpret_cast<uintptr_t>(a.fold_src) & 15) || (reinterpret_cast<uintptr_t>(a.fold_dst) & 15)))
        return RT_ERR_INVALID;
    if (a.wt_planes && ((a.n % 8) != 0 || (reinterpret_cast<uintptr_t>(a.wt_planes) & 15))) return RT_ERR_INVALID;
    return RT_OK;
}

extern "C" int rt_linear_bwd_dz_f32_multi(const rt_linear_bwd_args* args, int n_args, void* stream) {
    if (!args || n_args < 1 || n_args > 2) return RT_ERR_INVALID;
    int tpwk = 1;
    size_t lds = 0;
    unsigned blocks[2] = {0u, 0u};
    bool wpl = true;
    for (int g = 0; g < n_args; ++g) {
        const int v = validate_bwd(&args[g]);
        if (v) return v;
        const rt_linear_bwd_args& a = args[g];
        const bool need_da = a.g_prev || a.dsrc;
        wpl = wpl && (!need_da || a.wt_planes != nullptr);
        const int t = !need_da ? 1 : a.k <= 128 ? 1 : a.k <= 256 ? 2 : 4;
        tpwk = t > tpwk ? t : tpwk;
        const int np = mlp::pad8(a.n);
        const size_t l = (static_cast<size_t>(mlp::FM) * (np + 4) + 5 * static_cast<size_t>(np)) * sizeof(float) +
                         3 * static_cast<size_t>(mlp::FM) * (np + 8) * sizeof(uint16_t) + 16;
        lds = l > lds ? l : lds;
        blocks[g] = static_cast<unsigned>((a.m + mlp::FM - 1) / mlp::FM);
    }
    if (all_dz_fusable(args, n_args)) {
        for (int g = 0; g < n_args; ++g)
            if (args[g].fold_src && args[g].fold_in == 0) return RT_ERR_INVALID;
        return RT_OK;
    }
    mlp::BwdLaunch L{};
    L.a0 = args[0];
    L.a1 = n_args > 1 ? args[1] : args[0];
    L.ngroups = n_args;
    L.split = blocks[0];
    const unsigned total = blocks[0] + (n_args > 1 ? blocks[1] : 0u);
    if (total == 0) return RT_OK;
    bool any_da = false;
    for (int g = 0; g < n_args; ++g) any_da = any_da || args[g].g_prev || args[g].dsrc;
    static const int ks_env = [] { const char* e = getenv("RT_DZ_KSPLIT"); return e ? atoi(e) : 0; }();
    unsigned ks = (tpwk == 2 && any_da && total <= 256u) ? 2u : 1u;
    if (ks_env == 1 || (ks_env == 2 && tpwk == 2 && any_da)) ks = static_cast<unsigned>(ks_env);
    L.ksplit = ks;
    if (ks == 2) tpwk = 1;
    const dim3 grid(total * ks);
    hipStream_t st = as_stream(stream);
#define RT_DZ(T, P, K)                                                                        \
    do {                                                                                      \
        allow_lds(mlp::linear_bwd_dz_kernel<T, P, K>, lds);                                   \
        hipLaunchKernelGGL((mlp::linear_bwd_dz_kernel<T, P, K>), grid, dim3(256), lds, st, L); \
    } while (0)
    if (ks > 1) {
        if (wpl) RT_DZ(1, true, true); else RT_DZ(1, false, true);
    } else {
        switch (tpwk) {
            case 1: if (wpl) RT_DZ(1, true, false); else RT_DZ(1, false, false); break;
            case 2: if (wpl) RT_DZ(2, true, false); else RT_DZ(2, false, false); break;
            default: RT_DZ(4, false, false); break;
        }
    }
#undef RT_DZ
    return check_launch("linear_bwd_dz_kernel");
}

extern "C" int rt_linear_bwd_dz_fused(const rt_linear_bwd_args* args, int n_args) {
    return (args && n_args >= 1 && n_args <= 2 && all_dz_fusable(args, n_args)) ? 1 : 0;
}

extern "C" int rt_linear_bwd_dz_f32(const rt_linear_bwd_args* args, void* stream) {
    return rt_linear_bwd_dz_f32_multi(args, 1, stream);
}

#ifndef RT_DW_BLOCKS
#define RT_DW_BLOCKS 384
#endif
#ifndef RT_DW_BLOCKS_SMALLK
#define RT_DW_BLOCKS_SMALLK 256
#endif
static void dw_plan(const rt_linear_bwd_args* args, int n_args, bool small_k, unsigned* tn, unsigned* tk,
                    int64_t* splits, int64_t& rps) {
    const int bn = small_k ? 128 : 64, bk = small_k ? 32 : 64;
#ifndef RT_DW_CAP_SMALLK
#define RT_DW_CAP_SMALLK 128
#endif
    const int64_t cap = small_k ? RT_DW_CAP_SMALLK : 64;
    int64_t work = 0, rmin = mlp::DW_R;
    for (int g = 0; g < n_args; ++g) {
        const rt_linear_bwd_args& a = args[g];
        tn[g] = static_cast<unsigned>((a.n + bn - 1) / bn);
        tk[g] = static_cast<unsigned>((a.k + bk - 1) / bk);
        work += a.m * tn[g] * tk[g];
        const int64_t r = (a.m + cap - 1) / cap;
        rmin = r > rmin ? r : rmin;
    }
    const int64_t target = small_k ? RT_DW_BLOCKS_SMALLK : RT_DW_BLOCKS;
    rps = (work + target - 1) / target;
    rps = rps > rmin ? rps : rmin;
    rps = (rps + mlp::DW_R - 1) / mlp::DW_R * mlp::DW_R;
    for (int g = 0; g < n_args; ++g)
        if (args[g].ids && rps > mlp::DW_MAXR) rps = mlp::DW_MAXR;
    for (int g = 0; g < n_args; ++g) splits[g] = args[g].m > 0 ? (args[g].m + rps - 1) / rps : 0;
}

static int dw_prologue(const rt_linear_bwd_args& a) {
    if (a.prev_mode == 0 || a.a_in) return 0;
    return !act_is_piecewise_linear(a.prev_act) ? 3 : (a.prev_drop_p > 0.f ? 2 : 1);
}
static bool dw_mixed(const rt_linear_bwd_args* args, int n_args) {
    return n_args == 2 && (dw_prologue(args[0]) == 0) != (dw_prologue(args[1]) == 0);
}

static int dw_launch(const rt_linear_bwd_args* args, int n_args, bool dzf, hipStream_t st) {
    mlp::BwdLaunch L{};
    unsigned blocks[2] = {0u, 0u};
    int pro = -1;
    bool small_k = true;
    for (int g = 0; g < n_args; ++g) small_k = small_k && args[g].k <= 32;
    unsigned tns[2] = {1u, 1u}, tks[2] = {1u, 1u};
    int64_t nsplit[2] = {0, 0}, rps = mlp::DW_R;
    dw_plan(args, n_args, small_k, tns, tks, nsplit, rps);
    for (int g = 0; g < n_args; ++g) {
        const rt_linear_bwd_args& a = args[g];
        const int64_t nb = static_cast<int64_t>(tns[g]) * tks[g] * nsplit[g];
        if (nb > (1ll << 30)) return RT_ERR_UNSUPPORTED;
        blocks[g] = static_cast<unsigned>(nb);
        (g ? L.tn1 : L.tn0) = tns[g] ? tns[g] : 1u;
        (g ? L.tk1 : L.tk0) = tks[g] ? tks[g] : 1u;
        (g ? L.rps1 : L.rps0) = rps;
        const int p = dw_prologue(a);
        pro = p > pro ? p : pro;
        const float* asrc = a.a_in ? a.a_in : a.src;
        const int ald = a.a_in ? a.k : a.ld_src;
        (g ? L.vec1 : L.vec0) = (a.n % 4) == 0 && (a.k % 4) == 0 && (ald % 4) == 0 &&
                                (reinterpret_cast<uintptr_t>(asrc) & 15) == 0 &&
                                (reinterpret_cast<uintptr_t>(a.dz_ws) & 15) == 0;
    }
    L.a0 = args[0];
    L.a1 = n_args > 1 ? args[1] : args[0];
    L.ngroups = n_args;
    if (n_args == 1) { L.tn1 = L.tn0; L.tk1 = L.tk0; L.rps1 = L.rps0; L.vec1 = L.vec0; }
    L.split = blocks[0];
    const unsigned total = blocks[0] + (n_args > 1 ? blocks[1] : 0u);
    if (total == 0) return RT_OK;
    const dim3 grid(total);
    const bool vec = L.vec0 && L.vec1;
#define RT_DW(BN, BK, P)                                                                                                 \
    do {                                                                                                                 \
        if (dzf) {                                                                                                       \
            if (vec) hipLaunchKernelGGL((mlp::linear_bwd_dw_kernel<BN, BK, P, true, true>), grid, dim3(mlp::DW_NT), 0, st, L);  \
            else hipLaunchKernelGGL((mlp::linear_bwd_dw_kernel<BN, BK, P, false, true>), grid, dim3(mlp::DW_NT), 0, st, L);     \
        } else {                                                                                                         \
            if (vec) hipLaunchKernelGGL((mlp::linear_bwd_dw_kernel<BN, BK, P, true, false>), grid, dim3(mlp::DW_NT), 0, st, L); \
            else hipLaunchKernelGGL((mlp::linear_bwd_dw_kernel<BN, BK, P, false, false>), grid, dim3(mlp::DW_NT), 0, st, L);    \
        }                                                                                                                \
    } while (0)
    if (small_k) {
        switch (pro) { case 0: RT_DW(128, 32, 0); break; case 1: RT_DW(128, 32, 1); break;
                       case 2: RT_DW(128, 32, 2); break; default: RT_DW(128, 32, 3); }
    } else {
        switch (pro) { case 0: RT_DW(64, 64, 0); break; case 1: RT_DW(64, 64, 1); break;
                       case 2: RT_DW(64, 64, 2); break; default: RT_DW(64, 64, 3); }
    }
#undef RT_DW
    return check_launch("linear_bwd_dw_kernel");
}

extern "C" int rt_linear_bwd_dw_f32_multi(const rt_linear_bwd_args* args, int n_args, void* stream) {
    if (!args || n_args < 1 || n_args > 2) return RT_ERR_INVALID;
#ifdef RT_NO_AIN
    rt_linear_bwd_args noa[2];
    for (int g = 0; g < n_args; ++g) { noa[g] = args[g]; noa[g].a_in = nullptr; }
    args = noa;
#endif
    for (int g = 0; g < n_args; ++g) {
        const int v = validate_bwd(&args[g]);
        if (v) return v;
        if (args[g].ids && args[g].prev_mode != 0) return RT_ERR_UNSUPPORTED;
    }
    hipStream_t st = as_stream(stream);
    const bool dzf = all_dz_fusable(args, n_args);
    if (dw_mixed(args, n_args)) {
        const int r0 = dw_launch(&args[0], 1, dzf, st);
        return r0 ? r0 : dw_launch(&args[1], 1, dzf, st);
    }
    return dw_launch(args, n_args, dzf, st);
}

extern "C" int rt_linear_bwd_dw_splits(const rt_linear_bwd_args* args, int n_args, int64_t* splits) {
    if (!args || !splits || n_args < 1 || n_args > 2) return RT_ERR_INVALID;
#ifdef RT_NO_DW_PART
    return RT_ERR_UNSUPPORTED;
#endif
    bool small_k = true;
    for (int g = 0; g < n_args; ++g) {
        const int v = validate_bwd(&args[g]);
        if (v) return v;
        small_k = small_k && args[g].k <= 32;
    }
    unsigned tns[2] = {1u, 1u}, tks[2] = {1u, 1u};
    int64_t nsplit[2] = {0, 0}, rps = mlp::DW_R;
    if (dw_mixed(args, n_args)) {
        for (int g = 0; g < 2; ++g) {
            dw_plan(&args[g], 1, args[g].k <= 32, tns, tks, nsplit, rps);
            splits[g] = nsplit[0];
        }
        return RT_OK;
    }
    dw_plan(args, n_args, small_k, tns, tks, nsplit, rps);
    for (int g = 0; g < n_args; ++g) splits[g] = nsplit[g];
    return RT_OK;
}

extern "C" int rt_linear_bwd_dw_f32(const rt_linear_bwd_args* args, void* stream) {
    return rt_linear_bwd_dw_f32_multi(args, 1, stream);
}

#ifdef RT_PHASE_PROBE
extern "C" int rt_probe_setup(void* buf, unsigned cap) {
    unsigned long long* p = static_cast<unsigned long long*>(buf);
    const unsigned zero[64] = {};
    if (hipMemcpyToSymbol(HIP_SYMBOL(mlp::g_probe_buf), &p, sizeof(p)) != hipSuccess) return RT_ERR_HIP;
    if (hipMemcpyToSymbol(HIP_SYMBOL(mlp::g_probe_cap), &cap, sizeof(cap)) != hipSuccess) return RT_ERR_HIP;
    if (hipMemcpyToSymbol(HIP_SYMBOL(mlp::g_probe_ctr), zero, sizeof(zero)) != hipSuccess) return RT_ERR_HIP;
    return RT_OK;
}
extern "C" int rt_probe_count(unsigned* out) {
    return hipMemcpyFromSymbol(out, HIP_SYMBOL(mlp::g_probe_ctr), 64 * sizeof(unsigned)) == hipSuccess ? RT_OK
                                                                                                       : RT_ERR_HIP;
}
#endif

extern "C" int rt_linear_bwd_f32(const rt_linear_bwd_args* args, void* stream) {
    const int rc = rt_linear_bwd_dz_f32(args, stream);
    return rc ? rc : rt_linear_bwd_dw_f32(args, stream);
}
```

### real-time-recommendation-system-with-feature-store_amd/csrc/optim.hip

```cpp
#include "rt_common.h"

namespace rt {
namespace optim {

#ifndef RT_NORM_CHUNK
#define RT_NORM_CHUNK 1024
#endif
constexpr int kChunk = RT_NORM_CHUNK;

__global__ __launch_bounds__(256) void grad_sqnorm_kernel(const float* __restrict__ g,
                                                          const int64_t* __restrict__ offsets,
                                                          double* __restrict__ out, int32_t* step_counter,
                                                          int64_t* seed_counter) {
    __shared__ double red[4];
    const int t = blockIdx.y;
    if (blockIdx.x == 0 && t == 0 && threadIdx.x == 0) {
        if (step_counter) *step_counter += 1;
        if (seed_counter) *seed_counter += 1;
    }
    const int64_t lo = offsets[t], hi = offsets[t + 1];
    if (lo + static_cast<int64_t>(blockIdx.x) * kChunk >= hi) return;
    double s = 0.0;
    for (int64_t c0 = lo + static_cast<int64_t>(blockIdx.x) * kChunk; c0 < hi;
         c0 += static_cast<int64_t>(gridDim.x) * kChunk) {
        const int64_t c1 = (c0 + kChunk) < hi ? (c0 + kChunk) : hi;
#pragma unroll 4
        for (int64_t e = c0 + threadIdx.x; e < c1; e += 256) {
            const double v = g[e];
            s += v * v;
        }
    }
    s = wave_sum(s);
    if ((threadIdx.x & 63) == 0) red[threadIdx.x >> 6] = s;
    __syncthreads();
    if (threadIdx.x == 0) atomicAdd(&out[t], red[0] + red[1] + red[2] + red[3]);
}

__global__ __launch_bounds__(256) void clip_adam_kernel(float* __restrict__ p, float* __restrict__ g,
                                                        float* __restrict__ m, float* __restrict__ v, int64_t n,
                                                        const double* __restrict__ sumsq, int n_tensors,
                                                        float max_norm, float lr, const float* lr_dev, float b1,
                                                        float b2, float eps, float wd, int step,
                                                        const int32_t* step_dev, double* __restrict__ zbuf,
                                                        int64_t zwords) {
    __shared__ float coef_s, step_size_s, bc2_sqrt_s;
    const int64_t e0 = static_cast<int64_t>(blockIdx.x) * 256 + threadIdx.x;
    float p0 = 0.f, g0 = 0.f, m0 = 0.f, v0 = 0.f;
    if (e0 < n) { p0 = p[e0]; g0 = g[e0]; m0 = m[e0]; v0 = v[e0]; }
    if (threadIdx.x < 64) {
        double tot = 0.0;
        for (int t = threadIdx.x; t < n_tensors; t += 64) tot += sumsq[t];
        tot = wave_sum(tot);
        if (threadIdx.x == 0) {
            const float total = static_cast<float>(sqrt(tot));
            const float coef = max_norm / (total + 1e-6f);
            coef_s = coef < 1.f ? coef : 1.f;
            const int st = step_dev ? *step_dev : step;
            const float lr_v = lr_dev ? *lr_dev : lr;
            const double bc1 = 1.0 - pow(static_cast<double>(b1), st);
            const double bc2 = 1.0 - pow(static_cast<double>(b2), st);
            step_size_s = static_cast<float>(lr_v / bc1);
            bc2_sqrt_s = static_cast<float>(sqrt(bc2));
        }
    }
    __syncthreads();
    const float coef = coef_s, step_size = step_size_s, bc2s = bc2_sqrt_s;
    const int64_t stride = static_cast<int64_t>(gridDim.x) * 256;
    auto update = [&](int64_t e, float pv, float graw, float mo, float vo) {
        float gv = graw * coef;
        if (wd != 0.f) gv = gv + wd * pv;
        const float mv = mo + (1.f - b1) * (gv - mo);
        const float vv = vo * b2 + (1.f - b2) * gv * gv;
        const float denom = sqrtf(vv) / bc2s + eps;
        m[e] = mv;
        v[e] = vv;
        p[e] = pv - step_size * (mv / denom);
        g[e] = 0.f;
    };
    if (e0 < n) update(e0, p0, g0, m0, v0);
    for (int64_t e = e0 + stride; e < n; e += stride) update(e, p[e], g[e], m[e], v[e]);
    for (int64_t e = static_cast<int64_t>(blockIdx.x) * 256 + threadIdx.x; e < zwords; e += stride) zbuf[e] = 0.0;
}

}
}

using namespace rt;

extern "C" int rt_grad_sqnorm(const float* grads, const int64_t* offsets, int n_tensors, double* sumsq_out,
                              int32_t* step_counter, int64_t* seed_counter, void* stream) {
    if (n_tensors < 0 || (n_tensors > 0 && (!grads || !offsets || !sumsq_out))) return RT_ERR_INVALID;
    if (n_tensors == 0) return RT_OK;
    const dim3 grid(64, static_cast<unsigned>(n_tensors));
    hipLaunchKernelGGL(optim::grad_sqnorm_kernel, grid, dim3(256), 0, as_stream(stream), grads, offsets, sumsq_out,
                       step_counter, seed_counter);
    return check_launch("grad_sqnorm_kernel");
}

extern "C" int rt_clip_adam_step(float* params, float* grads, float* exp_avg, float* exp_avg_sq, int64_t n,
                                 const double* sumsq, int n_tensors, float max_norm, float lr, const float* lr_dev,
                                 float beta1, float beta2, float eps, float weight_decay, int step,
                                 const int32_t* step_dev, double* zero_buf, int64_t zero_words, void* stream) {
    if (n < 0 || !params || !grads || !exp_avg || !exp_avg_sq || !sumsq || n_tensors <= 0) return RT_ERR_INVALID;
    if (!step_dev && step < 1) return RT_ERR_INVALID;
    if (zero_words < 0 || (zero_words > 0 && !zero_buf)) return RT_ERR_INVALID;
    if (n == 0) return RT_OK;
    int64_t blocks = (n + 255) / 256;
    if (blocks > 1024) blocks = 1024;
    hipLaunchKernelGGL(optim::clip_adam_kernel, dim3(static_cast<unsigned>(blocks)), dim3(256), 0, as_stream(stream),
                       params, grads, exp_avg, exp_avg_sq, n, sumsq, n_tensors, max_norm, lr, lr_dev, beta1, beta2,
                       eps, weight_decay, step, step_dev, zero_buf, zero_words);
    return check_launch("clip_adam_kernel");
}
```

### real-time-recommendation-system-with-feature-store_amd/rtrec_amd/models/fused.py

```python
from __future__ import annotations

import ctypes
import itertools
import os
from dataclasses import dataclass, field
from typing import List, Optional

import torch
import torch.nn as nn

from .. import native
from ..native import LinearBwdArgs, LinearFwdArgs, call, ptr
from ..profiling import TIMER

ACT_CODE = {nn.ReLU: 0, nn.GELU: 1, nn.LeakyReLU: 2, nn.Tanh: 3, nn.Sigmoid: 4}
ACT_NONE = 5

_seed_counter = itertools.count(1)


def act_code(mod: Optional[nn.Module]) -> int:
    if mod is None:
        return ACT_NONE
    for cls, code in ACT_CODE.items():
        if isinstance(mod, cls):
            if cls is nn.LeakyReLU and abs(mod.negative_slope - 0.1) > 1e-12:
                raise NotImplementedError("LeakyReLU slope other than 0.1 (two_tower.py:82)")
            return code
    raise NotImplementedError(f"activation {type(mod).__name__}")


@dataclass
class Block:
    linear: nn.Linear
    act: int = ACT_NONE
    bn: Optional[nn.BatchNorm1d] = None
    drop: Optional[nn.Dropout] = None

    def drop_p(self) -> float:
        return float(self.drop.p) if (self.drop is not None and self.drop.training and self.drop.p > 0) else 0.0

    def bn_mode(self) -> int:
        if self.bn is None:
            return 3
        return 1 if self.bn.training else 2


def blocks_from_sequential(seq: nn.Sequential) -> List[Block]:
    mods = list(seq)
    blocks: List[Block] = []
    i = 0
    while i < len(mods):
        lin = mods[i]
        if not isinstance(lin, nn.Linear):
            raise NotImplementedError(f"unexpected module {type(lin).__name__} at {i}")
        b = Block(lin)
        i += 1
        if i < len(mods) and not isinstance(mods[i], (nn.Linear, nn.BatchNorm1d, nn.Dropout)):
            b.act = act_code(mods[i])
            i += 1
        if i < len(mods) and isinstance(mods[i], nn.BatchNorm1d):
            b.bn = mods[i]
            i += 1
        if i < len(mods) and isinstance(mods[i], nn.Dropout):
            b.drop = mods[i]
            i += 1
        blocks.append(b)
    return blocks


class ParamSlab:

    def __init__(self, module: nn.Module):
        self.module = module
        self.params: List[nn.Parameter] = []
        self.data: Optional[torch.Tensor] = None
        self.grad: Optional[torch.Tensor] = None
        self.offsets: List[int] = []
        self.offsets_dev: Optional[torch.Tensor] = None
        self.grad_gen = 0

    def _valid(self) -> bool:
        ps = [p for p in self.module.parameters()]
        if self.data is None or len(ps) != len(self.params) or any(a is not b for a, b in zip(ps, self.params)):
            return False
        base = self.data.data_ptr()
        for p, off in zip(self.params, self.offsets):
            if p.device != self.data.device or p.data_ptr() != base + off * 4:
                return False
        return True

    def ensure(self) -> "ParamSlab":
        if self._valid():
            return self
        ps = list(self.module.parameters())
        if not ps:
            raise ValueError("module has no parameters")
        dev = ps[0].device
        for p in ps:
            if p.dtype != torch.float32 or p.device != dev:
                raise TypeError("parameter slab needs fp32 parameters on one device")
        sizes = [p.numel() for p in ps]
        offs, cur = [], 0
        for s in sizes:
            offs.append(cur)
            cur += (s + 3) // 4 * 4
        data = torch.zeros(cur, dtype=torch.float32, device=dev)
        grad = torch.zeros(cur, dtype=torch.float32, device=dev)
        with torch.no_grad():
            for p, o, s in zip(ps, offs, sizes):
                data[o:o + s].copy_(p.data.reshape(-1))
        for p, o, s in zip(ps, offs, sizes):
            p.data = data[o:o + s].view(p.shape)
            old = p.grad
            p.grad = grad[o:o + s].view(p.shape)
            if old is not None:
                p.grad.copy_(old)
        self.params, self.offsets, self.data, self.grad = ps, offs, data, grad
        self.grad_gen += 1
        self.__dict__["_grad_views"] = {}
        ends = [o + s for o, s in zip(offs, sizes)]
        self.bounds = list(zip(offs, ends))
        self.offsets_dev = None
        return self

    def attach_grads(self):
        self.ensure()
        self.grad_gen += 1
        for p, (o, e) in zip(self.params, self.bounds):
            view = self.grad[o:e]
            if p.grad is None:
                view.zero_()
                p.grad = view.view(p.shape)
            elif p.grad.data_ptr() != view.data_ptr():
                view.copy_(p.grad.reshape(-1))
                p.grad = view.view(p.shape)

    def grad_of(self, p: torch.Tensor) -> torch.Tensor:
        cache = self.__dict__.setdefault("_grad_views", {})
        v = cache.get(id(p))
        if v is not None and v[0] is p and v[1].data_ptr() >= self.grad.data_ptr():
            return v[1]
        for q, (o, e) in zip(self.params, self.bounds):
            if q is p:
                view = self.grad[o:e].view(p.shape)
                cache[id(p)] = (p, view)
                return view
        raise KeyError("parameter not in slab")

    def tensor_offsets(self) -> torch.Tensor:
        if self.offsets_dev is None:
            b = [o for o, _ in self.bounds] + [self.bounds[-1][1]]
            self.offsets_dev = torch.tensor(b, dtype=torch.int64, device=self.data.device)
        return self.offsets_dev


@dataclass
class ChainCtx:
    m: int
    src: torch.Tensor
    ids: Optional[torch.Tensor]
    zs: List[Optional[torch.Tensor]] = field(default_factory=list)
    save_mean: List[Optional[torch.Tensor]] = field(default_factory=list)
    save_invstd: List[Optional[torch.Tensor]] = field(default_factory=list)
    seeds: List[int] = field(default_factory=list)
    drop_ps: List[float] = field(default_factory=list)
    bn_modes: List[int] = field(default_factory=list)
    out: Optional[torch.Tensor] = None
    norms: Optional[torch.Tensor] = None
    normalize: bool = True
    seg_split: int = 0
    wts: List[Optional[torch.Tensor]] = field(default_factory=list)
    w_planes: List[Optional[torch.Tensor]] = field(default_factory=list)
    wt_planes: List[Optional[torch.Tensor]] = field(default_factory=list)
    ains: List[Optional[torch.Tensor]] = field(default_factory=list)


def _stream(t: torch.Tensor):
    return ctypes.c_void_p(torch.cuda.current_stream(t.device).cuda_stream)


STAT_SLOTS = 16
DBIAS_ROWS = STAT_SLOTS + 1
FINALIZE_BN_IN_PRODUCER = os.environ.get("RTREC_BN_FINAL", "0") == "1"
_WPL = os.environ.get("RTREC_W_PLANES", "0")
SPLIT_W_PLANES = _WPL in ("1", "fwd", "dz")
SPLIT_W_PLANES_FWD = _WPL in ("1", "fwd")
SPLIT_W_PLANES_DZ = _WPL in ("1", "dz")


def stats_arena_size(blocks: List[Block], n_seg: int = 1) -> int:
    return max(1, n_seg * STAT_SLOTS * 2 * sum(b.linear.out_features for b in blocks[:-1])
               + DBIAS_ROWS * sum(b.linear.out_features for b in blocks))


def _zero_on_entry(layer, zero_buf: Optional[torch.Tensor]):
    if zero_buf is not None:
        layer.zero_buf = zero_buf.data_ptr()
        layer.zero_words = zero_buf.numel()


def chain_forward(blocks: List[Block], src: torch.Tensor, ids: Optional[torch.Tensor] = None,
                  normalize: bool = True, seed_offset: Optional[torch.Tensor] = None,
                  stats_arena: Optional[torch.Tensor] = None, seg_split: int = 0,
                  zero_buf: Optional[torch.Tensor] = None, seed_base: Optional[int] = None) -> ChainCtx:
    ctx, layers = _forward_plan(blocks, src, ids, normalize, seed_offset, stats_arena, seg_split, seed_base)
    _zero_on_entry(layers[0], zero_buf)
    st = _stream(src)
    for a in layers:
        _launch_fwd([a], st)
    return ctx


def chain_forward_pair(first: tuple, second: tuple, zero_buf: Optional[torch.Tensor] = None) -> tuple:
    c1, l1 = _forward_plan(*first)
    c2, l2 = _forward_plan(*second)
    _zero_on_entry(l1[0], zero_buf)
    st = _stream(first[1])
    if len(l1) == len(l2):
        for a, b in zip(l1, l2):
            _launch_fwd([a, b], st)
    else:
        for a in l1 + l2:
            _launch_fwd([a], st)
    return c1, c2


def _launch_fwd(group: list, st) -> None:
    flops = sum(2.0 * a.m * a.k * a.n for a in group)
    nbytes = sum(4.0 * (a.m * a.k + a.n * a.k + a.m * a.n) for a in group)
    with TIMER.region("linear_fwd", flops=flops, bytes_=nbytes):
        if len(group) == 1:
            call("rt_linear_fwd_f32", ctypes.byref(group[0]), st)
        else:
            arr = (LinearFwdArgs * len(group))(*group)
            call("rt_linear_fwd_f32_multi", arr, len(group), st)


def layer_seed(seed_base: int, layer: int) -> int:
    z = (seed_base * 0x100000001B3 + (layer + 1) * 0x9E3779B97F4A7C15) & 0xFFFFFFFFFFFFFFFF
    z = ((z ^ (z >> 30)) * 0xBF58476D1CE4E5B9) & 0xFFFFFFFFFFFFFFFF
    z = ((z ^ (z >> 27)) * 0x94D049BB133111EB) & 0xFFFFFFFFFFFFFFFF
    return z ^ (z >> 31)


def _forward_plan(blocks: List[Block], src: torch.Tensor, ids: Optional[torch.Tensor] = None,
                  normalize: bool = True, seed_offset: Optional[torch.Tensor] = None,
                  stats_arena: Optional[torch.Tensor] = None, seg_split: int = 0,
                  seed_base: Optional[int] = None):
    native.require_device(src, what="tower forward")
    if src.dtype != torch.float32:
        raise TypeError("tower input must be fp32 (the reference towers are fp32)")
    src = src.contiguous()
    m = int(ids.numel()) if ids is not None else int(src.shape[0])
    if ids is not None:
        ids = ids.contiguous().to(torch.int64)
    dev = src.device
    L = len(blocks) - 1
    k0 = blocks[0].linear.in_features
    if src.dim() != 2 or src.shape[1] != k0:
        raise RuntimeError(f"mat1 and mat2 shapes cannot be multiplied ({m}x{src.shape[-1]} and "
                           f"{k0}x{blocks[0].linear.out_features})")
    n_seg = 2 if seg_split else 1
    if seg_split and (seg_split % 32 != 0 or not 0 < seg_split < m):
        raise ValueError("seg_split must be a multiple of 32 inside (0, m)")
    seg_rows = [seg_split, m - seg_split] if seg_split else [m]
    for b in blocks[:-1]:
        if b.bn is not None and b.bn.training and min(seg_rows) <= 1:
            raise ValueError("Expected more than 1 value per channel when training (BatchNorm1d)")
    ctx = ChainCtx(m=m, src=src, ids=ids, normalize=normalize, seg_split=seg_split)
    widths = [b.linear.out_features for b in blocks[:-1]]
    if stats_arena is None:
        stats_arena = torch.zeros(stats_arena_size(blocks, n_seg), dtype=torch.float64, device=dev)
    stats, off = [], 0
    for wdt in widths:
        stats.append(stats_arena[off:off + n_seg * STAT_SLOTS * 2 * wdt])
        off += n_seg * STAT_SLOTS * 2 * wdt
    layers = []
    cur_src, cur_ids, ld = src, ids, src.shape[1]
    for li, b in enumerate(blocks):
        lin = b.linear
        a = LinearFwdArgs()
        a.src = cur_src.data_ptr()
        a.src_rows = cur_src.shape[0]
        a.ld_src = ld
        a.ids = cur_ids.data_ptr() if cur_ids is not None else None
        a.m = m
        a.k = lin.in_features
        a.n = lin.out_features
        a.w = lin.weight.data_ptr()
        a.bias = lin.bias.data_ptr() if lin.bias is not None else None
        a.seed_offset = seed_offset.data_ptr() if seed_offset is not None else None
        a.seg_split = seg_split
        if li == 0:
            a.prev_mode = 0
        else:
            pb = blocks[li - 1]
            a.prev_mode = pb.bn_mode()
            a.prev_act = pb.act
            a.drop_p = pb.drop_p()
            a.drop_seed = ctx.seeds[li - 1]
            if pb.bn is not None:
                a.prev_stats = stats[li - 1].data_ptr()
                a.bn_gamma = pb.bn.weight.data_ptr()
                a.bn_beta = pb.bn.bias.data_ptr()
                a.running_mean = pb.bn.running_mean.data_ptr()
                a.running_var = pb.bn.running_var.data_ptr()
                sm = torch.empty(n_seg * lin.in_features, dtype=torch.float32, device=dev)
                si = torch.empty(n_seg * lin.in_features, dtype=torch.float32, device=dev)
                ctx.save_mean[li - 1], ctx.save_invstd[li - 1] = sm, si
                a.save_mean = sm.data_ptr()
                a.save_invstd = si.data_ptr()
                a.bn_eps = float(pb.bn.eps)
                a.bn_momentum = float(pb.bn.momentum if pb.bn.momentum is not None else 0.1)
                if pb.bn.training and pb.bn.num_batches_tracked is not None:
                    a.num_batches_tracked = pb.bn.num_batches_tracked.data_ptr()
                prod = layers[li - 1]
                if a.prev_mode == 1 and prod.stats_out and FINALIZE_BN_IN_PRODUCER:
                    prod.fin_save_mean, prod.fin_save_invstd = a.save_mean, a.save_invstd
                    prod.fin_running_mean, prod.fin_running_var = a.running_mean, a.running_var
                    prod.fin_num_batches_tracked = a.num_batches_tracked
                    prod.fin_eps, prod.fin_momentum = a.bn_eps, a.bn_momentum
                    a.prev_final = 1
        a.act = b.act
        wt = wtp = None
        if li > 0 and lin.training:
            if SPLIT_W_PLANES and SPLIT_W_PLANES_DZ and lin.out_features % 8 == 0:
                wtp = torch.empty((3, lin.in_features, lin.out_features), dtype=torch.int16, device=dev)
                a.wt_planes_out = wtp.data_ptr()
            else:
                wt = torch.empty((lin.in_features, lin.out_features), dtype=torch.float32, device=dev)
                a.wt_out = wt.data_ptr()
        ctx.wts.append(wt)
        ctx.wt_planes.append(wtp)
        wp = None
        if SPLIT_W_PLANES and SPLIT_W_PLANES_FWD and li > 0 and lin.in_features % 8 == 0 and lin.out_features <= 128:
            wp = torch.empty((3, lin.out_features, lin.in_features), dtype=torch.int16, device=dev)
            prev = layers[li - 1]
            prev.next_w = lin.weight.data_ptr()
            prev.next_w_planes = wp.data_ptr()
            prev.next_n, prev.next_k = lin.out_features, lin.in_features
            a.w_planes = wp.data_ptr()
        ctx.w_planes.append(wp)
        ain = None
        if li > 0 and lin.training and lin.in_features % 4 == 0:
            ain = torch.empty((m, lin.in_features), dtype=torch.float32, device=dev)
            a.a_out = ain.data_ptr()
        ctx.ains.append(ain)
        if li < L:
            z = torch.empty((m, lin.out_features), dtype=torch.float32, device=dev)
            a.z_out = z.data_ptr()
            if b.bn is not None and b.bn.training:
                a.stats_out = stats[li].data_ptr()
            ctx.zs.append(z)
            ctx.save_mean.append(None)
            ctx.save_invstd.append(None)
            ctx.seeds.append(layer_seed(seed_base, li) if seed_base is not None else
                             next(_seed_counter) * 0x9E3779B97F4A7C15 & 0xFFFFFFFFFFFFFFFF)
            ctx.drop_ps.append(b.drop_p())
            ctx.bn_modes.append(b.bn_mode())
            cur_src, cur_ids, ld = z, None, lin.out_features
        else:
            out = torch.empty((m, lin.out_features), dtype=torch.float32, device=dev)
            if normalize:
                norms = torch.empty(m, dtype=torch.float32, device=dev)
                a.l2_out = out.data_ptr()
                a.norms_out = norms.data_ptr()
                ctx.norms = norms
            else:
                a.z_out = out.data_ptr()
            ctx.out = out
        layers.append(a)
    return ctx, layers


def chain_backward(blocks: List[Block], ctx: ChainCtx, dout: torch.Tensor, slab: ParamSlab,
                   want_dsrc: bool = False, seed_offset: Optional[torch.Tensor] = None,
                   stats_arena: Optional[torch.Tensor] = None, attach: bool = True) -> Optional[torch.Tensor]:
    layers, dsrc, keep = _backward_plan(blocks, ctx, dout, slab, want_dsrc, seed_offset, stats_arena, attach)
    st = _stream(dout)
    groups = [[a] for a in layers]
    keep += _plan_partials(groups, dout.device)
    for g in groups:
        _launch_bwd(g, st)
    return dsrc


def chain_backward_pair(first: tuple, second: tuple) -> None:
    l1, _, keep1 = _backward_plan(*first)
    l2, _, keep2 = _backward_plan(*second)
    st = _stream(first[2])
    if len(l1) == len(l2):
        groups = [[a, b] for a, b in zip(l1, l2)]
        keep1 += _plan_partials(groups, first[2].device)
    else:
        groups = [[a] for a in l1 + l2]
    for g in groups:
        _launch_bwd(g, st)


def _plan_partials(groups: list, dev) -> list:
    lib = native.lib()
    if not hasattr(lib, "rt_linear_bwd_dw_splits"):
        return []
    keep = []
    for gi in range(len(groups) - 1):
        grp, nxt = groups[gi], groups[gi + 1]
        if len(grp) != len(nxt):
            continue
        arr = (LinearBwdArgs * len(grp))(*grp)
        splits = (ctypes.c_int64 * len(grp))()
        if lib.rt_linear_bwd_dw_splits(arr, len(grp), splits) != 0:
            continue
        narr = (LinearBwdArgs * len(nxt))(*nxt)
        fold_in = 1 if lib.rt_linear_bwd_dz_fused(narr, len(nxt)) else 0
        for a, b, sp in zip(grp, nxt, splits):
            words = a.n * a.k
            if sp < 1 or words % 4 or b.fold_src:
                continue
            part = torch.empty(sp * words, dtype=torch.float32, device=dev)
            keep.append(part)
            a.dw_part = part.data_ptr()
            b.fold_src, b.fold_dst, b.fold_words = part.data_ptr(), a.dw, words
            b.fold_splits, b.fold_in = sp, fold_in
    return keep


def _launch_bwd(group: list, st) -> None:
    da = [a.g_prev is not None or a.dsrc is not None for a in group]
    flops = sum((2.0 if d else 0.0) * a.m * a.k * a.n for a, d in zip(group, da))
    nbytes = sum(4.0 * (3 * a.m * a.n + (2 * a.m * a.k if d else 0) + a.n * a.k) for a, d in zip(group, da))
    arr = (LinearBwdArgs * len(group))(*group)
    lib = native.lib()
    fused = hasattr(lib, "rt_linear_bwd_dz_fused") and lib.rt_linear_bwd_dz_fused(arr, len(group))
    if not fused:
        with TIMER.region("linear_bwd_dz", flops=flops, bytes_=nbytes):
            call("rt_linear_bwd_dz_f32_multi", arr, len(group), st)
    with TIMER.region("linear_bwd_dw", flops=sum(2.0 * a.m * a.k * a.n for a in group),
                      bytes_=sum(4.0 * (a.m * a.n + a.m * a.k + a.n * a.k) for a in group)):
        call("rt_linear_bwd_dw_f32_multi", arr, len(group), st)


def _backward_plan(blocks: List[Block], ctx: ChainCtx, dout: torch.Tensor, slab: ParamSlab,
                   want_dsrc: bool = False, seed_offset: Optional[torch.Tensor] = None,
                   stats_arena: Optional[torch.Tensor] = None, attach: bool = True):
    dev = dout.device
    dout = dout.contiguous()
    m = ctx.m
    L = len(blocks) - 1
    if attach:
        slab.attach_grads()
    dz_bufs = [torch.empty((m, b.linear.out_features), dtype=torch.float32, device=dev) for b in blocks]
    layers = []
    widths = [b.linear.out_features for b in blocks[:-1]]
    n_seg = 2 if ctx.seg_split else 1
    gst_arena = stats_arena if stats_arena is not None else \
        torch.zeros(stats_arena_size(blocks, n_seg), dtype=torch.float64, device=dev)
    gstats, off = [], 0
    for wdt in widths:
        gstats.append(gst_arena[off:off + n_seg * STAT_SLOTS * 2 * wdt])
        off += n_seg * STAT_SLOTS * 2 * wdt
    bslots = []
    for b in blocks:
        bslots.append(gst_arena[off:off + DBIAS_ROWS * b.linear.out_features])
        off += DBIAS_ROWS * b.linear.out_features
    gs: List[Optional[torch.Tensor]] = [None] * L
    dsrc = torch.empty((m, blocks[0].linear.in_features), dtype=torch.float32, device=dev) if want_dsrc else None
    keep = [dout, gst_arena] + dz_bufs
    for li in range(L, -1, -1):
        b = blocks[li]
        lin = b.linear
        a = LinearBwdArgs()
        a.m, a.k, a.n = m, lin.in_features, lin.out_features
        a.w = lin.weight.data_ptr()
        a.dw = slab.grad_of(lin.weight).data_ptr()
        a.dbias = slab.grad_of(lin.bias).data_ptr() if lin.bias is not None else None
        a.dbias_slots = bslots[li].data_ptr() if lin.bias is not None else None
        a.dz_ws = dz_bufs[li].data_ptr()
        a.seed_offset = seed_offset.data_ptr() if seed_offset is not None else None
        a.seg_split = ctx.seg_split
        if li == L:
            if ctx.normalize:
                a.grad_mode = 0
                a.dout = dout.data_ptr()
                a.l2_out = ctx.out.data_ptr()
                a.norms = ctx.norms.data_ptr()
            else:
                a.grad_mode = 3
                a.g = dout.data_ptr()
                a.z = dout.data_ptr()
                a.act = ACT_NONE
        else:
            a.grad_mode = ctx.bn_modes[li]
            a.g = gs[li].data_ptr()
            a.z = ctx.zs[li].data_ptr()
            a.act = b.act
            if b.bn is not None:
                a.g_stats = gstats[li].data_ptr()
                a.save_mean = ctx.save_mean[li].data_ptr()
                a.save_invstd = ctx.save_invstd[li].data_ptr()
                a.bn_gamma = b.bn.weight.data_ptr()
                a.dgamma = slab.grad_of(b.bn.weight).data_ptr()
                a.dbeta = slab.grad_of(b.bn.bias).data_ptr()
        if li == 0 and not want_dsrc:
            a.fuse_dz = 1
        if li == 0:
            a.src = ctx.src.data_ptr()
            a.src_rows = ctx.src.shape[0]
            a.ld_src = ctx.src.shape[1]
            a.ids = ctx.ids.data_ptr() if ctx.ids is not None else None
            a.prev_mode = 0
            if want_dsrc:
                if ctx.ids is not None:
                    raise NotImplementedError("input gradient through a fused gather")
                a.dsrc = dsrc.data_ptr()
        else:
            pb = blocks[li - 1]
            a.src = ctx.zs[li - 1].data_ptr()
            a.src_rows = m
            a.ld_src = pb.linear.out_features
            a.prev_mode = ctx.bn_modes[li - 1]
            a.prev_act = pb.act
            a.prev_drop_p = ctx.drop_ps[li - 1]
            a.prev_drop_seed = ctx.seeds[li - 1]
            if pb.bn is not None:
                a.prev_mean = ctx.save_mean[li - 1].data_ptr()
                a.prev_invstd = ctx.save_invstd[li - 1].data_ptr()
                a.prev_gamma = pb.bn.weight.data_ptr()
                a.prev_beta = pb.bn.bias.data_ptr()
                a.g_prev_stats = gstats[li - 1].data_ptr()
            g = torch.empty((m, pb.linear.out_features), dtype=torch.float32, device=dev)
            gs[li - 1] = g
            keep.append(g)
            a.g_prev = g.data_ptr()
            if li < len(ctx.wts) and ctx.wts[li] is not None:
                a.wt = ctx.wts[li].data_ptr()
            if li < len(ctx.wt_planes) and ctx.wt_planes[li] is not None:
                a.wt_planes = ctx.wt_planes[li].data_ptr()
            if li < len(ctx.ains) and ctx.ains[li] is not None:
                a.a_in = ctx.ains[li].data_ptr()
        layers.append(a)
    return layers, dsrc, keep
```

### real-time-recommendation-system-with-feature-store_amd/rtrec_amd/native.py

```python
from __future__ import annotations

import ctypes
import os
import threading
from typing import Optional

import torch

PKG_DIR = os.path.dirname(os.path.dirname(os.path.abspath(__file__)))
LIB_PATH = os.environ.get("RTREC_HIP_LIB", os.path.join(PKG_DIR, "lib", "librtrec_hip.so"))

RT_F32, RT_F16, RT_BF16 = 0, 1, 2
ACTS = {"relu": 0, "gelu": 1, "leaky_relu": 2, "tanh": 3, "sigmoid": 4, "none": 5}

c_i64 = ctypes.c_int64
c_int = ctypes.c_int
c_f32 = ctypes.c_float
c_u64 = ctypes.c_uint64
c_size = ctypes.c_size_t
vp = ctypes.c_void_p


class NativeUnavailable(RuntimeError):
    """librtrec_hip.so is missing or unusable (no CPU fallback exists)."""


class RTError(RuntimeError):

    def __init__(self, what: str, status: int, message: str):
        super().__init__(f"{what} failed: {message} (status {status})")
        self.status = status


class LinearFwdArgs(ctypes.Structure):
    _fields_ = [
        ("src", vp), ("src_rows", c_i64), ("ld_src", c_int), ("ids", vp), ("m", c_i64), ("k", c_int),
        ("n", c_int), ("w", vp), ("bias", vp),
        ("prev_mode", c_int), ("prev_act", c_int), ("prev_stats", vp), ("bn_gamma", vp), ("bn_beta", vp),
        ("running_mean", vp), ("running_var", vp), ("save_mean", vp), ("save_invstd", vp),
        ("bn_eps", c_f32), ("bn_momentum", c_f32), ("drop_p", c_f32), ("drop_seed", c_u64),
        ("seed_offset", vp), ("z_out", vp), ("act", c_int), ("stats_out", vp), ("l2_out", vp), ("norms_out", vp),
        ("num_batches_tracked", vp), ("seg_split", c_i64), ("zero_buf", vp), ("zero_words", c_i64),
        ("wt_out", vp), ("a_out", vp),
        ("fin_save_mean", vp), ("fin_save_invstd", vp), ("fin_running_mean", vp), ("fin_running_var", vp),
        ("fin_num_batches_tracked", vp), ("fin_eps", c_f32), ("fin_momentum", c_f32), ("prev_final", c_int),
        ("w_planes", vp), ("wt_planes_out", vp), ("next_w", vp), ("next_w_planes", vp), ("next_n", c_int),
        ("next_k", c_int),
    ]


class LinearBwdArgs(ctypes.Structure):
    _fields_ = [
        ("m", c_i64), ("k", c_int), ("n", c_int), ("w", vp), ("dw", vp), ("dbias", vp), ("dz_ws", vp),
        ("grad_mode", c_int), ("dout", vp), ("l2_out", vp), ("norms", vp),
        ("g", vp), ("z", vp), ("act", c_int), ("g_stats", vp), ("save_mean", vp), ("save_invstd", vp),
        ("bn_gamma", vp), ("dgamma", vp), ("dbeta", vp),
        ("src", vp), ("src_rows", c_i64), ("ld_src", c_int), ("ids", vp),
        ("prev_mode", c_int), ("prev_act", c_int), ("prev_mean", vp), ("prev_invstd", vp),
        ("prev_gamma", vp), ("prev_beta", vp), ("prev_drop_p", c_f32), ("prev_drop_seed", c_u64),
        ("seed_offset", vp), ("g_prev", vp), ("g_prev_stats", vp), ("dsrc", vp), ("seg_split", c_i64),
        ("dbias_slots", vp), ("wt", vp), ("fuse_dz", c_int), ("a_in", vp), ("dw_part", vp),
        ("fold_src", vp), ("fold_dst", vp), ("fold_words", c_i64), ("fold_splits", c_int), ("fold_in", c_int),
        ("wt_planes", vp),
    ]


SIGNATURES = {
    "rt_abi_version": (c_int, []),
    "rt_status_string": (ctypes.c_char_p, [c_int]),
    "rt_last_error": (ctypes.c_char_p, []),
    "rt_gather_rows": (c_int, [vp, c_i64, c_i64, c_i64, vp, c_i64, vp, vp, vp]),
    "rt_scatter_add_rows_f32": (c_int, [vp, c_i64, c_int, vp, c_i64, vp, c_i64, vp]),
    "rt_l2_renorm_f32": (c_int, [vp, c_i64, c_int, vp]),
    "rt_flatip_topk_workspace_bytes": (c_size, [c_i64, c_i64, c_int, c_int, c_int]),
    "rt_flatip_topk": (c_int, [vp, c_i64, vp, c_i64, c_int, c_int, c_int, vp, c_i64, c_i64, vp, vp, vp,
                               c_size, vp]),
    "rt_topk_merge": (c_int, [vp, vp, c_i64, c_int, c_int, c_int, vp, vp, vp]),
    "rt_flatip_topk_tuning": (c_int, [c_int, c_int, c_int]),
    "rt_flatip_topk_shard_workspace_bytes": (c_size, [c_i64, c_i64, c_int, c_int, c_int]),
    "rt_flatip_topk_shard_plan": (c_int, [c_i64, c_i64, c_int, c_int, c_int, c_int, vp]),
    "rt_flatip_topk_shard_sample": (c_int, [vp, c_i64, vp, c_i64, c_int, c_int, c_int, c_int, vp, vp, vp, c_size,
                                            vp]),
    "rt_topk_sample_rank": (c_int, [c_int, c_i64, c_i64, vp]),
    "rt_topk_sample_threshold": (c_int, [vp, c_int, c_i64, c_int, vp, vp]),
    "rt_flatip_topk_shard_search": (c_int, [vp, c_i64, vp, c_i64, c_int, c_int, c_int, vp, c_i64, vp, vp, vp,
                                            c_size, vp]),
    "rt_sample_negatives": (c_int, [vp, vp, c_i64, vp, c_i64, c_i64, c_int, c_u64, vp, vp, vp]),
    "rt_feeder_batch": (c_int, [vp, vp, vp, vp, c_i64, vp, vp, vp]),
    "rt_feeder_commit": (c_int, [vp, vp, c_i64, vp, vp]),
    "rt_linear_fwd_f32": (c_int, [ctypes.POINTER(LinearFwdArgs), vp]),
    "rt_linear_bwd_f32": (c_int, [ctypes.POINTER(LinearBwdArgs), vp]),
    "rt_linear_bwd_dz_f32": (c_int, [ctypes.POINTER(LinearBwdArgs), vp]),
    "rt_linear_bwd_dz_fused": (c_int, [ctypes.POINTER(LinearBwdArgs), c_int]),
    "rt_linear_bwd_dw_splits": (c_int, [ctypes.POINTER(LinearBwdArgs), c_int, ctypes.POINTER(c_i64)]),
    "rt_linear_bwd_dw_f32": (c_int, [ctypes.POINTER(LinearBwdArgs), vp]),
    "rt_linear_fwd_f32_multi": (c_int, [ctypes.POINTER(LinearFwdArgs), c_int, vp]),
    "rt_linear_bwd_dz_f32_multi": (c_int, [ctypes.POINTER(LinearBwdArgs), c_int, vp]),
    "rt_linear_bwd_dw_f32_multi": (c_int, [ctypes.POINTER(LinearBwdArgs), c_int, vp]),
    "rt_twotower_loss_workspace_bytes": (c_size, [c_i64, c_int]),
    "rt_twotower_loss_fwd_bwd": (c_int, [vp, vp, vp, c_int, c_i64, c_int, c_int, c_f32, vp, vp, c_f32,
                                         c_f32, vp, vp, vp, vp, vp, vp, vp, c_size, vp]),
    "rt_twotower_loss_fwd": (c_int, [vp, vp, vp, c_int, c_i64, c_int, c_int, c_f32, vp, vp, c_f32, c_f32,
                                     vp, vp, c_size, vp]),
    "rt_inbatch_loss_workspace_bytes": (c_size, [c_i64, c_i64, c_int]),
    "rt_inbatch_loss_fwd_bwd": (c_int, [vp, vp, c_int, c_i64, c_i64, c_int, c_i64, c_f32, vp, vp, vp, vp, c_size, vp]),
    "rt_similarity_f32": (c_int, [vp, vp, c_i64, c_int, c_f32, vp, vp, vp, vp]),
    "rt_grad_sqnorm": (c_int, [vp, vp, c_int, vp, vp, vp, vp]),
    "rt_clip_adam_step": (c_int, [vp, vp, vp, vp, c_i64, vp, c_int, c_f32, c_f32, vp, c_f32, c_f32, c_f32,
                                  c_f32, c_int, vp, vp, c_i64, vp]),
    "rt_l2_augment_f32": (c_int, [vp, c_i64, c_int, vp, c_int, c_int, vp]),
    "rt_l2_finish_f32": (c_int, [vp, c_int, vp, c_int, c_int, c_i64, c_int, vp, vp, c_int, vp, vp, vp, c_i64, vp]),
    "rt_exclusion_bitmap": (c_int, [vp, vp, c_i64, vp, c_i64, c_i64, vp, c_i64, vp]),
    "rt_rank_metrics": (c_int, [vp, c_i64, c_int, vp, vp, vp, c_i64, vp, vp, vp, c_i64, vp, c_int, c_i64, vp, vp,
                                vp, vp]),
    "rt_rank_metrics_reduce": (c_int, [vp, vp, c_i64, c_int, vp, c_i64, vp, vp]),
}

RT_METRICS_MAX_K = 16

_lib = None
_lock = threading.Lock()
_load_error: Optional[str] = None
MISSING: list = []


def lib():
    global _lib, _load_error
    if _lib is not None:
        return _lib
    with _lock:
        if _lib is not None:
            return _lib
        if not os.path.exists(LIB_PATH):
            _load_error = (f"{LIB_PATH} not found — build it with "
                           f"`make -C {PKG_DIR}` (or __graft_entry__.build())")
            raise NativeUnavailable(_load_error)
        try:
            handle = ctypes.CDLL(LIB_PATH)
        except OSError as e:
            _load_error = f"cannot load {LIB_PATH}: {e}"
            raise NativeUnavailable(_load_error) from e
        for name, (res, args) in SIGNATURES.items():
            if not hasattr(handle, name):
                MISSING.append(name)
                continue
            fn = getattr(handle, name)
            fn.restype = res
            fn.argtypes = args
        _lib = handle
        return _lib


def available() -> bool:
    try:
        lib()
        return True
    except NativeUnavailable:
        return False


def call(name: str, *args) -> int:
    fn = getattr(lib(), name)
    rc = fn(*args)
    if rc != 0:
        msg = lib().rt_status_string(rc).decode()
        last = lib().rt_last_error().decode()
        raise RTError(name, rc, msg + (f" [{last}]" if last else ""))
    return rc


def ptr(t: Optional[torch.Tensor]):
    return None if t is None else ctypes.c_void_p(t.data_ptr())


def stream_of(t: torch.Tensor):
    return ctypes.c_void_p(torch.cuda.current_stream(t.device).cuda_stream)


def require_device(*tensors: torch.Tensor, what: str = "rtrec kernel"):
    for t in tensors:
        if t is not None and t.device.type != "cuda":
            raise RuntimeError(f"{what}: expected a ROCm (cuda) device tensor, got {t.device}; "
                               "this MI355X build has no CPU fallback")
    lib()


def dtype_code(dt: torch.dtype) -> int:
    if dt == torch.float32:
        return RT_F32
    if dt == torch.float16:
        return RT_F16
    if dt == torch.bfloat16:
        return RT_BF16
    raise TypeError(f"unsupported dtype {dt}")
```

### real-time-recommendation-system-with-feature-store_amd/rtrec_amd/training/fused_step.py

```python
from __future__ import annotations

import ctypes
import itertools
from typing import Dict, Optional

import torch

from .. import kernels, native
from ..models.fused import (blocks_from_sequential, chain_backward, chain_backward_pair, chain_forward,
                            chain_forward_pair, stats_arena_size)
from ..models.two_tower import TwoTowerModel
from ..native import call, ptr
from ..profiling import TIMER


_STEP_SEEDS = itertools.count(0x5EED)


def _adjacent_or_cat(a: torch.Tensor, b: torch.Tensor) -> torch.Tensor:
    if (a.is_contiguous() and b.is_contiguous() and a.dtype == b.dtype and a.device == b.device
            and a.untyped_storage().data_ptr() == b.untyped_storage().data_ptr()
            and b.data_ptr() == a.data_ptr() + a.numel() * a.element_size()):
        return torch.as_strided(a, (a.numel() + b.numel(),), (1,))
    return torch.cat([a.reshape(-1), b.reshape(-1)])


class FusedTrainStep:
    def __init__(self, model: TwoTowerModel, lr: float = 1e-3, weight_decay: float = 1e-5, max_norm: float = 1.0,
                 betas=(0.9, 0.999), eps: float = 1e-8, explicit_weight: float = 0.7,
                 in_batch_weight: float = 0.3, process_group=None, dropout_seed: Optional[int] = None):
        self.model = model
        self.pg = process_group
        self.slab = model.slab()
        dev = self.slab.data.device
        native.require_device(self.slab.data, what="FusedTrainStep")
        self.dev = dev
        self.exp_avg = torch.zeros_like(self.slab.data)
        self.exp_avg_sq = torch.zeros_like(self.slab.data)
        self.step_dev = torch.zeros(1, dtype=torch.int32, device=dev)
        self.lr_dev = torch.tensor([lr], dtype=torch.float32, device=dev)
        self.seed_dev = torch.zeros(1, dtype=torch.int64, device=dev)
        if dropout_seed is None:
            dropout_seed = next(_STEP_SEEDS)
        self.dropout_seed = int(dropout_seed)
        self._sb_user, self._sb_pos, self._sb_neg = (self.dropout_seed * 4 + r for r in (1, 2, 3))
        self._loss_ws: Optional[torch.Tensor] = None
        self._loss_ws_retired = []
        ua = stats_arena_size(blocks_from_sequential(model.user_tower.mlp))
        ia = stats_arena_size(blocks_from_sequential(model.item_tower.mlp))
        self._arena_sizes = [ua, ia, ia, ua, ia, ia]
        self.arena = torch.zeros(sum(self._arena_sizes), dtype=torch.float64, device=dev)
        parts, off = [], 0
        for sz in self._arena_sizes:
            parts.append(self.arena[off:off + sz])
            off += sz
        (self.a_uf, self.a_pf, self.a_nf, self.a_ub, self.a_pb, self.a_nb) = parts
        self.small = torch.zeros(3 + len(self.slab.params), dtype=torch.float64, device=dev)
        self.loss_buf, self.sumsq = self.small[:3], self.small[3:]
        self.slab.grad.zero_()
        self._clean = True
        self._grad_gen = self.slab.grad_gen
        self.a_pqf = self.arena[ua:ua + 2 * ia]
        self.a_pqb = self.arena[2 * ua + 2 * ia:2 * ua + 4 * ia]
        self.lr, self.wd, self.max_norm = lr, weight_decay, max_norm
        self.b1, self.b2 = betas
        self.eps = eps
        self.we, self.wb = explicit_weight, in_batch_weight
        self.steps = 0
        self.graph: Optional[torch.cuda.CUDAGraph] = None
        self.graph_update: Optional[torch.cuda.CUDAGraph] = None
        self.static: Dict[str, torch.Tensor] = {}
        self.concurrent = True
        self.side = [torch.cuda.Stream(device=dev), torch.cuda.Stream(device=dev)]

    def set_lr(self, lr: float):
        self.lr = lr
        self.lr_dev.fill_(lr)

    def optimizer_state_dict(self) -> dict:
        step = float(self.step_dev.item())
        state = {}
        for i, (o, e) in enumerate(self.slab.bounds):
            shape = self.slab.params[i].shape
            state[i] = {"step": torch.tensor(step), "exp_avg": self.exp_avg[o:e].view(shape).clone(),
                        "exp_avg_sq": self.exp_avg_sq[o:e].view(shape).clone()}
        group = {"lr": self.lr, "betas": (self.b1, self.b2), "eps": self.eps, "weight_decay": self.wd,
                 "amsgrad": False, "maximize": False, "foreach": None, "capturable": False,
                 "differentiable": False, "fused": None, "params": list(range(len(self.slab.params)))}
        return {"state": state, "param_groups": [group]}

    def load_optimizer_state_dict(self, sd: dict):
        steps = set()
        for i, (o, e) in enumerate(self.slab.bounds):
            st = sd["state"].get(i, sd["state"].get(str(i)))
            if st is None:
                continue
            self.exp_avg[o:e].copy_(st["exp_avg"].reshape(-1))
            self.exp_avg_sq[o:e].copy_(st["exp_avg_sq"].reshape(-1))
            steps.add(int(float(st["step"])))
        if len(steps) > 1:
            raise ValueError("per-parameter Adam step counts differ; the fused step keeps one counter")
        if steps:
            self.step_dev.fill_(steps.pop())
        self.set_lr(float(sd["param_groups"][0]["lr"]))

    def _ensure_clean(self):
        if not self._clean or self.slab.grad_gen != self._grad_gen:
            self.slab.grad.zero_()
            self.arena.zero_()
            self._grad_gen = self.slab.grad_gen
        self._clean = False

    def _run(self, user_src, pos_src, neg_src, user_ids=None, pos_ids=None, neg_ids=None):
        self._ensure_clean()
        self._grads(user_src, pos_src, neg_src, user_ids, pos_ids, neg_ids)
        self._allreduce()
        out = self._update()
        self._clean = True
        return out

    def _grads(self, user_src, pos_src, neg_src, user_ids=None, pos_ids=None, neg_ids=None):
        m = self.model
        ub = blocks_from_sequential(m.user_tower.mlp)
        ib = blocks_from_sequential(m.item_tower.mlp)
        slab = self.slab
        st = native.stream_of(slab.data)
        so = self.seed_dev
        main = torch.cuda.current_stream(self.dev)
        s_u, s_p = self.side if self.concurrent else (main, main)
        b = user_ids.numel() if user_ids is not None else user_src.shape[0]
        merged = neg_src is not None and b % 32 == 0 and (
            (pos_ids is not None and neg_ids is not None and pos_src is neg_src) or
            (pos_ids is None and neg_ids is None))
        if merged:
            if pos_ids is not None:
                item_src, item_ids = pos_src, _adjacent_or_cat(pos_ids, neg_ids)
            else:
                item_src, item_ids = torch.cat([pos_src, neg_src]), None
            pq, u = chain_forward_pair((ib, item_src, item_ids, True, so, self.a_pqf, b, self._sb_pos),
                                       (ub, user_src, user_ids, True, so, self.a_uf, 0, self._sb_user),
                                       zero_buf=self.small)
            p_out, q_out = pq.out[:b], pq.out[b:]
        else:
            p = chain_forward(ib, pos_src, pos_ids, seed_offset=so, stats_arena=self.a_pf, zero_buf=self.small,
                              seed_base=self._sb_pos)
            q = chain_forward(ib, neg_src, neg_ids, seed_offset=so, stats_arena=self.a_nf,
                              seed_base=self._sb_neg) if (neg_src is not None) else None
            p_out, q_out = p.out, (q.out if q is not None else None)
        if not merged:
            s_u.wait_stream(main)
            with torch.cuda.stream(s_u):
                u = chain_forward(ub, user_src, user_ids, seed_offset=so, stats_arena=self.a_uf,
                                  seed_base=self._sb_user)
            main.wait_stream(s_u)
        d = u.out.shape[1]
        n_neg = (q_out.shape[0] // b) if q_out is not None else 0
        du = torch.empty_like(u.out)
        if merged:
            dpq = torch.empty_like(pq.out)
            dp, dq = dpq[:b], dpq[b:]
        else:
            dp = torch.empty_like(p_out)
            dq = torch.empty_like(q_out) if q_out is not None else None
        ws = self._loss_workspace(native.lib().rt_twotower_loss_workspace_bytes(b, d))
        ubias, ibias = m.user_bias, m.item_bias
        with TIMER.region("loss_fwd_bwd", flops=6.0 * b * b * d + 6.0 * b * (n_neg + 1) * d,
                          bytes_=4.0 * d * (4 * b + 2 * b * n_neg)):
            call("rt_twotower_loss_fwd_bwd", ptr(u.out), ptr(p_out), ptr(q_out) if q_out is not None else None, 0,
                 b, d, n_neg, 1.0 / m.temperature, ptr(ubias), ptr(ibias), self.we, self.wb, ptr(self.loss_buf),
                 ptr(du), ptr(dp), ptr(dq),
                 ptr(slab.grad_of(ubias)) if ubias is not None else None,
                 ptr(slab.grad_of(ibias)) if ibias is not None else None, ptr(ws), ws.numel(), st)
        if merged:
            chain_backward_pair((ib, pq, dpq, slab, False, so, self.a_pqb, False),
                                (ub, u, du, slab, False, so, self.a_ub, False))
        else:
            s_u.wait_stream(main)
            with torch.cuda.stream(s_u):
                chain_backward(ub, u, du, slab, seed_offset=so, stats_arena=self.a_ub, attach=False)
            s_p.wait_stream(main)
            with torch.cuda.stream(s_p):
                chain_backward(ib, p, dp, slab, seed_offset=so, stats_arena=self.a_pb, attach=False)
            if q is not None:
                chain_backward(ib, q, dq, slab, seed_offset=so, stats_arena=self.a_nb, attach=False)
            main.wait_stream(s_p)
        main.wait_stream(s_u)

    def _loss_workspace(self, nbytes: int) -> torch.Tensor:
        if self._loss_ws is None or self._loss_ws.numel() < nbytes:
            if self._loss_ws is not None:
                self._loss_ws_retired.append(self._loss_ws)
            self._loss_ws = torch.empty(max(nbytes, 256), dtype=torch.uint8, device=self.dev)
        return self._loss_ws

    def _allreduce(self):
        if self.pg is not None:
            import torch.distributed as dist
            if dist.get_backend(self.pg) == "nccl":
                dist.all_reduce(self.slab.grad, op=dist.ReduceOp.AVG, group=self.pg)
            else:
                dist.all_reduce(self.slab.grad, op=dist.ReduceOp.SUM, group=self.pg)
                self.slab.grad.mul_(1.0 / dist.get_world_size(self.pg))

    def _update(self):
        slab = self.slab
        st = native.stream_of(slab.data)
        nb = slab.data.numel() * 4.0
        with TIMER.region("clip_adam", flops=0.0, bytes_=nb * 7):
            call("rt_grad_sqnorm", ptr(slab.grad), ptr(slab.tensor_offsets()), len(slab.params), ptr(self.sumsq),
                 ptr(self.step_dev), ptr(self.seed_dev), st)
            call("rt_clip_adam_step", ptr(slab.data), ptr(slab.grad), ptr(self.exp_avg), ptr(self.exp_avg_sq),
                 slab.data.numel(), ptr(self.sumsq), len(slab.params), self.max_norm, self.lr, ptr(self.lr_dev),
                 self.b1, self.b2, self.eps, self.wd, 1, ptr(self.step_dev), ptr(self.arena), self.arena.numel(), st)
        return self.loss_buf

    def __call__(self, user_src: torch.Tensor, pos_src: torch.Tensor, neg_src: Optional[torch.Tensor],
                 user_ids: Optional[torch.Tensor] = None, pos_ids: Optional[torch.Tensor] = None,
                 neg_ids: Optional[torch.Tensor] = None) -> torch.Tensor:
        self.model.train()
        if neg_src is not None and neg_ids is None and neg_src.dim() == 3:
            neg_src = neg_src.reshape(-1, neg_src.shape[-1])
        self.steps += 1
        return self._run(user_src, pos_src, neg_src, user_ids, pos_ids, neg_ids)

    def _state_tensors(self):
        return [self.slab.data, self.exp_avg, self.exp_avg_sq, self.step_dev, self.seed_dev] + \
            [b for b in self.model.buffers()]

    def capture(self, user_src, pos_src, neg_src, user_ids=None, pos_ids=None, neg_ids=None, warmup: int = 2,
                restore: bool = True):
        self.model.train()
        snap = [t.clone() for t in self._state_tensors()] if restore else None
        s = torch.cuda.Stream(device=self.dev)
        s.wait_stream(torch.cuda.current_stream(self.dev))
        with torch.cuda.stream(s):
            for _ in range(warmup):
                self._run(user_src, pos_src, neg_src, user_ids, pos_ids, neg_ids)
        torch.cuda.current_stream(self.dev).wait_stream(s)
        if snap is not None:
            with torch.no_grad():
                for t, v in zip(self._state_tensors(), snap):
                    t.copy_(v)
            del snap
        g = torch.cuda.CUDAGraph()
        with torch.cuda.graph(g):
            self._grads(user_src, pos_src, neg_src, user_ids, pos_ids, neg_ids)
            if self.pg is None:
                self._update()
        self.graph = g
        self.graph_update = None
        if self.pg is not None:
            g2 = torch.cuda.CUDAGraph()
            with torch.cuda.graph(g2):
                self._update()
            self.graph_update = g2
        if not restore:
            self.steps += warmup
        return g

    def capture_body(self, body, extra_state=(), warmup: int = 2) -> torch.cuda.CUDAGraph:
        if self.pg is not None:
            raise RuntimeError("capture_body: data-parallel steps are captured as two graphs (capture())")
        self.model.train()
        tensors = self._state_tensors() + list(extra_state)
        snap = [t.clone() for t in tensors]
        s = torch.cuda.Stream(device=self.dev)
        s.wait_stream(torch.cuda.current_stream(self.dev))
        with torch.cuda.stream(s):
            for _ in range(warmup):
                self._ensure_clean()
                body()
                self._clean = True
        torch.cuda.current_stream(self.dev).wait_stream(s)
        with torch.no_grad():
            for t, v in zip(tensors, snap):
                t.copy_(v)
        del snap
        self._ensure_clean()
        g = torch.cuda.CUDAGraph()
        with torch.cuda.graph(g):
            body()
        self._clean = True
        return g

    def replay(self):
        self._ensure_clean()
        self.graph.replay()
        if self.graph_update is not None:
            self._allreduce()
            self.graph_update.replay()
        self._clean = True
        self.steps += 1
        return self.loss_buf



class FeederGraph:

    def __init__(self, step: FusedTrainStep, feeder):
        if feeder.num_negatives <= 0:
            raise ValueError("FeederGraph: the mixed-loss step needs negatives")
        self.step, self.feeder = step, feeder
        dev = step.dev
        b, nn_ = feeder.batch_size, feeder.num_negatives
        self.n_rows = int(feeder.inter_u.numel())
        self.n_full = self.n_rows // b
        self.order = torch.empty(self.n_rows, dtype=torch.int64, device=dev)
        self.state = torch.zeros(2, dtype=torch.int64, device=dev)
        ids = torch.empty(b * (2 + nn_), dtype=torch.int64, device=dev)
        self.users, self.pos, self.neg = ids[:b], ids[b:2 * b], ids[2 * b:]
        self.losses = torch.zeros(max(1, len(feeder)), dtype=torch.float64, device=dev)
        self.graph: Optional[torch.cuda.CUDAGraph] = None

    def _body(self):
        f, b = self.feeder, self.feeder.batch_size
        st = native.stream_of(self.order)
        call("rt_feeder_batch", ptr(self.order), ptr(f.inter_u), ptr(f.inter_m), ptr(self.state), b,
             ptr(self.users), ptr(self.pos), st)
        kernels.sample_negatives(f.csr.offsets, f.csr.items, self.users, f.num_items, f.num_negatives,
                                 seed=f.seed * 1_000_003, seed_offset=self.state[1:2],
                                 out=self.neg.view(b, f.num_negatives))
        self.step._grads(f.user_table, f.item_table, f.item_table, self.users, self.pos, self.neg)
        loss = self.step._update()
        call("rt_feeder_commit", ptr(loss), ptr(self.losses), self.losses.numel(), ptr(self.state), st)

    def _start_epoch(self, epoch: int):
        f = self.feeder
        if f.shuffle:
            g = torch.Generator(device=self.step.dev)
            g.manual_seed(f.seed + 7919 * epoch)
            self.order.copy_(torch.randperm(self.n_rows, device=self.step.dev, generator=g))
        else:
            torch.arange(self.n_rows, out=self.order)
        self.state.copy_(torch.tensor([0, epoch * 1_000_000], dtype=torch.int64))

    def run_epoch(self, max_batches: int = 0) -> torch.Tensor:
        f = self.feeder
        n_b = len(f)
        if max_batches > 0:
            n_b = min(n_b, max_batches)
        n_graph = min(n_b, self.n_full)
        epoch = f.epoch
        if self.graph is None:
            self._start_epoch(epoch)
            self.graph = self.step.capture_body(self._body, extra_state=(self.state, self.losses))
        self._start_epoch(epoch)
        self.step.model.train()
        for _ in range(n_graph):
            self.step._ensure_clean()
            self.graph.replay()
            self.step._clean = True
        self.step.steps += n_graph
        if n_b > n_graph:
            idx = self.order[n_graph * f.batch_size:]
            bt = f.batch(idx, salt=epoch * 1_000_000 + n_graph)
            loss = self.step(bt["user_table"], bt["item_table"], bt["item_table"], user_ids=bt["user_ids"],
                             pos_ids=bt["pos_ids"], neg_ids=bt["neg_ids"])
            self.losses[n_graph:n_graph + 1].copy_(loss[0:1])
        f.epoch += 1
        return self.losses[:n_b]
```

Measured before the change: 4.441 billion pairs/s.

## Launch weight-gradient tiles for all layers jointly and fold split partials into norm

Moves the dW tile body into a device function that uses dynamic shared memory. A new joint kernel then runs the weight-gradient tiles of up to six layers from both towers in one grid, which replaces one launch per layer group. Split-K partial gradients are now summed into the grad slab inside a new grad-sqnorm-fold kernel rather than by a separate fold pass. This cuts kernel launches and serialization in the backward pass and the clip/Adam stage. The cost is more complex planning, dynamic LDS sizing, and partial buffers that stay live until the optimizer runs.

```diff
diff --git a/include/rtrec_hip.h b/include/rtrec_hip.h
--- a/include/rtrec_hip.h
+++ b/include/rtrec_hip.h
@@ -183,6 +183,8 @@
 int rt_linear_fwd_f32_multi(const rt_linear_fwd_args* args, int n_args, void* stream);
 int rt_linear_bwd_dz_f32_multi(const rt_linear_bwd_args* args, int n_args, void* stream);
 int rt_linear_bwd_dw_f32_multi(const rt_linear_bwd_args* args, int n_args, void* stream);
+int rt_linear_bwd_dw_f32_joint(const rt_linear_bwd_args* args, int n_args, void* stream);
+int rt_linear_bwd_dw_joint_splits(const rt_linear_bwd_args* args, int n_args, int64_t* splits);
 
 size_t rt_twotower_loss_workspace_bytes(int64_t b, int d);
 int rt_twotower_loss_fwd_bwd(const void* u, const void* p, const void* q, int dtype, int64_t b,
@@ -204,8 +206,19 @@
 int rt_similarity_f32(const float* u, const float* v, int64_t b, int d, float inv_tau,
                       const float* user_bias, const float* item_bias, float* out, void* stream);
 
+#define RT_GRAD_FOLD_MAX 8
+typedef struct {
+    const float* part;
+    int64_t dst_off;
+    int64_t words;
+    int splits;
+    int tensor;
+} rt_grad_fold;
 int rt_grad_sqnorm(const float* grads, const int64_t* offsets, int n_tensors, double* sumsq_out,
                    int32_t* step_counter, int64_t* seed_counter, void* stream);
+int rt_grad_sqnorm_fold(float* grads, const int64_t* offsets, int n_tensors, double* sumsq_out,
+                        int32_t* step_counter, int64_t* seed_counter, const rt_grad_fold* folds,
+                        int n_folds, void* stream);
 int rt_clip_adam_step(float* params, float* grads, float* exp_avg, float* exp_avg_sq,
                       int64_t n, const double* sumsq, int n_tensors, float max_norm, float lr,
                       const float* lr_dev, float beta1, float beta2, float eps, float weight_decay,
diff --git a/real-time-recommendation-system-with-feature-store_amd/csrc/mlp.hip b/real-time-recommendation-system-with-feature-store_amd/csrc/mlp.hip
--- a/real-time-recommendation-system-with-feature-store_amd/csrc/mlp.hip
+++ b/real-time-recommendation-system-with-feature-store_amd/csrc/mlp.hip
@@ -1160,8 +1160,13 @@
     }
 }
 
+__host__ __device__ constexpr int dw_lds_floats(int BN, int BK, int PRO, bool DZF) {
+    return 2 * DW_R * dw_ld(BN) + 2 * DW_R * dw_ld(BK) + (PRO != 0 ? 4 * BK : 0) + (DZF ? 10 * BN : 0) + 4;
+}
+
 template <int BN, int BK, int PRO, bool VEC, bool DZF>
-__global__ __launch_bounds__(DW_NT) void linear_bwd_dw_kernel(BwdLaunch L) {
+__device__ __forceinline__ void dw_tile(const rt_linear_bwd_args& a_set, const int64_t rows_per_split,
+                                        const unsigned tn, const unsigned tk, const unsigned bid, float* smem) {
     constexpr int NTN = BN / 32, WK = 4 / NTN, T = (BK / 32) / WK;
     static_assert(NTN * 32 == BN && 4 % NTN == 0 && T >= 1 && T * WK * 32 == BK, "dW tile");
     constexpr int LDN = dw_ld(BN), LDK = dw_ld(BK);
@@ -1170,20 +1175,15 @@
     static_assert(DW_NT % VN == 0 && DW_NT % VK == 0, "fixed staging columns per thread");
     static_assert(2 * DW_R * LDN >= 4 * T * 16 * 64, "row-group reduction fits in the dz buffers");
     static_assert(2 * DW_R * LDK >= (DW_NT / 64) * VN * 4, "dbias partials fit in the A buffers");
-    __shared__ __attribute__((aligned(16))) float Ld[2][DW_R * LDN];
-    __shared__ __attribute__((aligned(16))) float La[2][DW_R * LDK];
-    __shared__ int srow[PRO == 0 ? DW_MAXR : 1];
-    __shared__ __attribute__((aligned(16))) float aff_s[2][2][BK];
-    __shared__ __attribute__((aligned(16))) float dzc_s[DZF ? 2 : 1][5][DZF ? BN : 4];
-
-#ifdef RT_FOLD_FIRST
-    fold_side(L, 1);
-#endif
-    const bool g1 = blockIdx.x >= L.split;
-    const rt_linear_bwd_args a = g1 ? L.a1 : L.a0;
-    const int64_t rows_per_split = g1 ? L.rps1 : L.rps0;
-    const unsigned bid = blockIdx.x - (g1 ? L.split : 0u);
-    const unsigned tn = g1 ? L.tn1 : L.tn0, tk = g1 ? L.tk1 : L.tk0;
+    float* const Ld = smem;
+    float* const La = Ld + 2 * DW_R * LDN;
+    float* const aff_s = La + 2 * DW_R * LDK;
+    float* const dzc_s = aff_s + (PRO != 0 ? 4 * BK : 0);
+    int* const last_s = reinterpret_cast<int*>(dzc_s + (DZF ? 10 * BN : 0));
+    int* const srow = last_s + 4;
+    static_assert(dw_lds_floats(BN, BK, PRO, DZF) * sizeof(float) % 16 == 0, "16-B carve offsets");
+
+    const rt_linear_bwd_args a = a_set;
     const unsigned bx = bid % tn, by = (bid / tn) % tk, bz = bid / (tn * tk);
     const int n = a.n, k = a.k;
     const int64_t m = a.m;
@@ -1192,12 +1192,7 @@
     const int n0 = static_cast<int>(bx) * BN, k0 = static_cast<int>(by) * BK;
     const int64_t r_begin = static_cast<int64_t>(bz) * rows_per_split;
     const int64_t r_end = (r_begin + rows_per_split) < m ? (r_begin + rows_per_split) : m;
-    if (r_begin >= m) {
-#ifndef RT_FOLD_FIRST
-        fold_side(L, 1);
-#endif
-        return;
-    }
+    if (r_begin >= m) return;
     RT_PP_DECL
     const bool gather = PRO == 0 && a.ids != nullptr && !a.a_in;
     const float* const asrc = a.a_in ? a.a_in : a.src;
@@ -1208,20 +1203,20 @@
     const int gn = n0 + cn, gk = k0 + ck;
     float4 sc0 = make_float4(1.f, 1.f, 1.f, 1.f), sc1 = sc0;
     float4 sh0 = make_float4(0.f, 0.f, 0.f, 0.f), sh1 = sh0;
-    if ((a.prev_mode == 1 || a.prev_mode == 2) && !a.a_in) {
+    if (PRO != 0 && (a.prev_mode == 1 || a.prev_mode == 2) && !a.a_in) {
         if (tid < 2 * BK) {
             const int sg = tid / BK, cl = tid % BK, cc = k0 + cl;
             const int so = two ? sg * k : 0;
             float scv = 1.f, shv = 0.f;
             if (cc < k) bn_affine(a.prev_gamma[cc], a.prev_beta[cc], a.prev_mean[so + cc], a.prev_invstd[so + cc], scv, shv);
-            aff_s[sg][0][cl] = scv;
-            aff_s[sg][1][cl] = shv;
+            aff_s[(sg * 2 + 0) * BK + cl] = scv;
+            aff_s[(sg * 2 + 1) * BK + cl] = shv;
         }
         __syncthreads();
-        sc0 = *reinterpret_cast<const float4*>(&aff_s[0][0][ck]);
-        sh0 = *reinterpret_cast<const float4*>(&aff_s[0][1][ck]);
-        sc1 = *reinterpret_cast<const float4*>(&aff_s[1][0][ck]);
-        sh1 = *reinterpret_cast<const float4*>(&aff_s[1][1][ck]);
+        sc0 = *reinterpret_cast<const float4*>(&aff_s[0 * BK + ck]);
+        sh0 = *reinterpret_cast<const float4*>(&aff_s[1 * BK + ck]);
+        sc1 = *reinterpret_cast<const float4*>(&aff_s[2 * BK + ck]);
+        sh1 = *reinterpret_cast<const float4*>(&aff_s[3 * BK + ck]);
     }
     const uint64_t pseed = a.prev_drop_seed + (a.seed_offset ? *a.seed_offset : 0ull);
     const Pro pro{a.prev_mode, a.prev_act, a.prev_drop_p, a.prev_drop_p > 0.f ? 1.f / (1.f - a.prev_drop_p) : 1.f,
@@ -1245,8 +1240,9 @@
                     C = static_cast<float>(gs2) * inv_m;
                 }
             }
-            dzc_s[sg][0][cl] = A; dzc_s[sg][1][cl] = Bc; dzc_s[sg][2][cl] = C;
-            dzc_s[sg][3][cl] = M; dzc_s[sg][4][cl] = I;
+            float* const dc = dzc_s + sg * 5 * BN + cl;
+            dc[0] = A; dc[BN] = Bc; dc[2 * BN] = C;
+            dc[3 * BN] = M; dc[4 * BN] = I;
         }
         if (bid == 0 && (a.grad_mode == 1 || a.grad_mode == 2) && a.dgamma) {
             for (int c = tid; c < n; c += DW_NT) {
@@ -1345,8 +1341,9 @@
                     float4 d;
                     auto one = [&](float g, float z, int i) {
                         const int cl = cn + i;
-                        const float A = dzc_s[sg][0][cl], Bc = dzc_s[sg][1][cl], C = dzc_s[sg][2][cl];
-                        const float M = dzc_s[sg][3][cl], I = dzc_s[sg][4][cl];
+                        const float* const dc = dzc_s + sg * 5 * BN + cl;
+                        const float A = dc[0], Bc = dc[BN], C = dc[2 * BN];
+                        const float M = dc[3 * BN], I = dc[4 * BN];
                         const float xh = (act_pwl(dsl, z) - M) * I;
                         return (ok && gn + i < n) ? A * (g - Bc - xh * C) * (z > 0.f ? 1.f : dsl) : 0.f;
                     };
@@ -1356,7 +1353,7 @@
                     d.w = one(rd[j].w, rz[j].w, 3);
                     rd[j] = d;
                 }
-                *reinterpret_cast<float4*>(&Ld[buf][row * LDN + cn]) = rd[j];
+                *reinterpret_cast<float4*>(&Ld[buf * DW_R * LDN + row * LDN + cn]) = rd[j];
                 bsum.x += rd[j].x; bsum.y += rd[j].y; bsum.z += rd[j].z; bsum.w += rd[j].w;
             }
         }
@@ -1373,7 +1370,7 @@
                 v.y = (ok && gk + 1 < k) ? pro_col<PRO>(pro, slope, r, gk + 1, scs.y, shs.y, ra[j].y) : 0.f;
                 v.z = (ok && gk + 2 < k) ? pro_col<PRO>(pro, slope, r, gk + 2, scs.z, shs.z, ra[j].z) : 0.f;
                 v.w = (ok && gk + 3 < k) ? pro_col<PRO>(pro, slope, r, gk + 3, scs.w, shs.w, ra[j].w) : 0.f;
-                *reinterpret_cast<float4*>(&La[buf][row * LDK + ck]) = v;
+                *reinterpret_cast<float4*>(&La[buf * DW_R * LDK + row * LDK + ck]) = v;
             }
         }
     };
@@ -1392,8 +1389,8 @@
     for (int64_t base = r_begin; base < r_end; base += DW_R) {
         const bool more = base + DW_R < r_end;
         if (more) load(base + DW_R);
-        const float* dl = &Ld[buf][(2 * grp + h) * LDN + ncol];
-        const float* al = &La[buf][(2 * grp + h) * LDK + kcol0];
+        const float* dl = &Ld[buf * DW_R * LDN + (2 * grp + h) * LDN + ncol];
+        const float* al = &La[buf * DW_R * LDK + (2 * grp + h) * LDK + kcol0];
 #pragma unroll
         for (int i = 0; i < DW_R / (2 * DW_G); ++i) {
             const float av = dl[2 * DW_G * i * LDN];
@@ -1406,8 +1403,8 @@
     }
 
     RT_PP_MARK(2)
-    float* red = &Ld[0][0];
-    float* bred = &La[0][0];
+    float* red = Ld;
+    float* bred = La;
     if (do_bias) {
 #pragma unroll
         for (int o = VN; o < 64; o <<= 1) {
@@ -1468,17 +1465,16 @@
             if ((r >> 3) == grp) add_row(t, r, kk);
     }
     if (slot_bias) {
-        __shared__ int last_s;
         asm volatile("s_waitcnt vmcnt(0)" ::: "memory");
         __syncthreads();
         if (tid == 0) {
             ticket_release();
             unsigned long long* cnt = reinterpret_cast<unsigned long long*>(a.dbias_slots + static_cast<int64_t>(RT_STAT_SLOTS) * n);
             const unsigned long long nsplit = static_cast<unsigned long long>((m + rows_per_split - 1) / rows_per_split);
-            last_s = atomicAdd(&cnt[bx], 1ull) == nsplit - 1 ? 1 : 0;
+            *last_s = atomicAdd(&cnt[bx], 1ull) == nsplit - 1 ? 1 : 0;
         }
         __syncthreads();
-        if (last_s) {
+        if (*last_s) {
             for (int cl = tid; cl < BN; cl += DW_NT) {
                 const int c = n0 + cl;
                 if (c >= n) continue;
@@ -1489,10 +1485,39 @@
             }
         }
     }
+    RT_PP_END(3)
+}
+
+extern __shared__ __attribute__((aligned(16))) float dw_smem[];
+
+template <int BN, int BK, int PRO, bool VEC, bool DZF>
+__global__ __launch_bounds__(DW_NT) void linear_bwd_dw_kernel(BwdLaunch L) {
+#ifdef RT_FOLD_FIRST
+    fold_side(L, 1);
+#endif
+    const bool g1 = blockIdx.x >= L.split;
+    dw_tile<BN, BK, PRO, VEC, DZF>(g1 ? L.a1 : L.a0, g1 ? L.rps1 : L.rps0, g1 ? L.tn1 : L.tn0, g1 ? L.tk1 : L.tk0,
+                                   blockIdx.x - (g1 ? L.split : 0u), dw_smem);
 #ifndef RT_FOLD_FIRST
     fold_side(L, 1);
 #endif
-    RT_PP_END(3)
+}
+
+constexpr int DWJ_MAX = 6;
+struct DwJointLaunch {
+    rt_linear_bwd_args a[DWJ_MAX];
+    int64_t rps[DWJ_MAX];
+    unsigned tn[DWJ_MAX], tk[DWJ_MAX], end[DWJ_MAX];
+    unsigned char body[DWJ_MAX];
+    int nsets;
+};
+template <bool VS>
+__global__ __launch_bounds__(DW_NT) void linear_bwd_dw_joint_kernel(DwJointLaunch L) {
+    int s = 0;
+    while (s + 1 < L.nsets && blockIdx.x >= L.end[s]) ++s;
+    const unsigned bid = blockIdx.x - (s ? L.end[s - 1] : 0u);
+    if (L.body[s] == 0) dw_tile<128, 32, 0, VS, true>(L.a[s], L.rps[s], L.tn[s], L.tk[s], bid, dw_smem);
+    else dw_tile<64, 64, 0, true, false>(L.a[s], L.rps[s], L.tn[s], L.tk[s], bid, dw_smem);
 }
 
 }
@@ -1702,13 +1727,13 @@
 #ifndef RT_DW_BLOCKS_SMALLK
 #define RT_DW_BLOCKS_SMALLK 256
 #endif
-static void dw_plan(const rt_linear_bwd_args* args, int n_args, bool small_k, unsigned* tn, unsigned* tk,
-                    int64_t* splits, int64_t& rps) {
-    const int bn = small_k ? 128 : 64, bk = small_k ? 32 : 64;
 #ifndef RT_DW_CAP_SMALLK
 #define RT_DW_CAP_SMALLK 128
 #endif
-    const int64_t cap = small_k ? RT_DW_CAP_SMALLK : 64;
+static void dw_plan(const rt_linear_bwd_args* args, int n_args, bool small_k, unsigned* tn, unsigned* tk,
+                    int64_t* splits, int64_t& rps, int64_t target_blocks = 0, int64_t split_cap = 0) {
+    const int bn = small_k ? 128 : 64, bk = small_k ? 32 : 64;
+    const int64_t cap = split_cap > 0 ? split_cap : small_k ? RT_DW_CAP_SMALLK : 64;
     int64_t work = 0, rmin = mlp::DW_R;
     for (int g = 0; g < n_args; ++g) {
         const rt_linear_bwd_args& a = args[g];
@@ -1718,7 +1743,7 @@
         const int64_t r = (a.m + cap - 1) / cap;
         rmin = r > rmin ? r : rmin;
     }
-    const int64_t target = small_k ? RT_DW_BLOCKS_SMALLK : RT_DW_BLOCKS;
+    const int64_t target = target_blocks > 0 ? target_blocks : small_k ? RT_DW_BLOCKS_SMALLK : RT_DW_BLOCKS;
     rps = (work + target - 1) / target;
     rps = rps > rmin ? rps : rmin;
     rps = (rps + mlp::DW_R - 1) / mlp::DW_R * mlp::DW_R;
@@ -1733,6 +1758,13 @@
 }
 static bool dw_mixed(const rt_linear_bwd_args* args, int n_args) {
     return n_args == 2 && (dw_prologue(args[0]) == 0) != (dw_prologue(args[1]) == 0);
+}
+
+static bool dw_vec(const rt_linear_bwd_args& a) {
+    const float* asrc = a.a_in ? a.a_in : a.src;
+    const int ald = a.a_in ? a.k : a.ld_src;
+    return (a.n % 4) == 0 && (a.k % 4) == 0 && (ald % 4) == 0 && (reinterpret_cast<uintptr_t>(asrc) & 15) == 0 &&
+           (reinterpret_cast<uintptr_t>(a.dz_ws) & 15) == 0;
 }
 
 static int dw_launch(const rt_linear_bwd_args* args, int n_args, bool dzf, hipStream_t st) {
@@ -1754,11 +1786,7 @@
         (g ? L.rps1 : L.rps0) = rps;
         const int p = dw_prologue(a);
         pro = p > pro ? p : pro;
-        const float* asrc = a.a_in ? a.a_in : a.src;
-        const int ald = a.a_in ? a.k : a.ld_src;
-        (g ? L.vec1 : L.vec0) = (a.n % 4) == 0 && (a.k % 4) == 0 && (ald % 4) == 0 &&
-                                (reinterpret_cast<uintptr_t>(asrc) & 15) == 0 &&
-                                (reinterpret_cast<uintptr_t>(a.dz_ws) & 15) == 0;
+        (g ? L.vec1 : L.vec0) = dw_vec(a);
     }
     L.a0 = args[0];
     L.a1 = n_args > 1 ? args[1] : args[0];
@@ -1769,14 +1797,18 @@
     if (total == 0) return RT_OK;
     const dim3 grid(total);
     const bool vec = L.vec0 && L.vec1;
+    size_t id_bytes = 0;
+    for (int g = 0; g < n_args; ++g)
+        if (args[g].ids && !args[g].a_in) id_bytes = static_cast<size_t>(rps) * sizeof(int);
 #define RT_DW(BN, BK, P)                                                                                                 \
     do {                                                                                                                 \
+        const size_t lds = mlp::dw_lds_floats(BN, BK, P, dzf) * sizeof(float) + id_bytes;                                \
         if (dzf) {                                                                                                       \
-            if (vec) hipLaunchKernelGGL((mlp::linear_bwd_dw_kernel<BN, BK, P, true, true>), grid, dim3(mlp::DW_NT), 0, st, L);  \
-            else hipLaunchKernelGGL((mlp::linear_bwd_dw_kernel<BN, BK, P, false, true>), grid, dim3(mlp::DW_NT), 0, st, L);     \
+            if (vec) hipLaunchKernelGGL((mlp::linear_bwd_dw_kernel<BN, BK, P, true, true>), grid, dim3(mlp::DW_NT), lds, st, L);  \
+            else hipLaunchKernelGGL((mlp::linear_bwd_dw_kernel<BN, BK, P, false, true>), grid, dim3(mlp::DW_NT), lds, st, L);     \
         } else {                                                                                                         \
-            if (vec) hipLaunchKernelGGL((mlp::linear_bwd_dw_kernel<BN, BK, P, true, false>), grid, dim3(mlp::DW_NT), 0, st, L); \
-            else hipLaunchKernelGGL((mlp::linear_bwd_dw_kernel<BN, BK, P, false, false>), grid, dim3(mlp::DW_NT), 0, st, L);    \
+            if (vec) hipLaunchKernelGGL((mlp::linear_bwd_dw_kernel<BN, BK, P, true, false>), grid, dim3(mlp::DW_NT), lds, st, L); \
+            else hipLaunchKernelGGL((mlp::linear_bwd_dw_kernel<BN, BK, P, false, false>), grid, dim3(mlp::DW_NT), lds, st, L);    \
         }                                                                                                                \
     } while (0)
     if (small_k) {
@@ -1840,6 +1872,163 @@
     return rt_linear_bwd_dw_f32_multi(args, 1, stream);
 }
 
+static int dwj_body(const rt_linear_bwd_args& a) {
+    if (dw_prologue(a) != 0) return -1;
+    if (a.k <= 32) return dz_fusable(a) ? 0 : -1;
+    return (!dz_fusable(a) && dw_vec(a) && !(a.ids && !a.a_in)) ? 1 : -1;
+}
+
+#ifndef RT_DWJ_SLOTS
+#define RT_DWJ_SLOTS 512
+#endif
+#ifndef RT_DWJ_BLOCKS_SMALLK
+#define RT_DWJ_BLOCKS_SMALLK 128
+#endif
+#ifndef RT_DWJ_CAP_SMALLK
+#define RT_DWJ_CAP_SMALLK 64
+#endif
+#ifndef RT_DWJ_MIN_BLOCKS
+#define RT_DWJ_MIN_BLOCKS 128
+#endif
+struct DwJointPlan {
+    int body[mlp::DWJ_MAX];
+    unsigned tn[mlp::DWJ_MAX], tk[mlp::DWJ_MAX];
+    int64_t splits[mlp::DWJ_MAX], rps[mlp::DWJ_MAX];
+};
+static void dwj_plan(const rt_linear_bwd_args* args, int n_args, DwJointPlan& P) {
+    rt_linear_bwd_args small[mlp::DWJ_MAX];
+    int small_of[mlp::DWJ_MAX], ns = 0;
+    for (int g = 0; g < n_args; ++g) {
+        P.body[g] = dwj_body(args[g]);
+        P.tn[g] = P.tk[g] = 1u;
+        P.splits[g] = 0;
+        P.rps[g] = mlp::DW_R;
+        if (P.body[g] == 0) { small_of[ns] = g; small[ns++] = args[g]; }
+    }
+    int64_t blocks_small = 0;
+    if (ns) {
+        unsigned tn[mlp::DWJ_MAX], tk[mlp::DWJ_MAX];
+        int64_t sp[mlp::DWJ_MAX], rps = mlp::DW_R;
+        dw_plan(small, ns, true, tn, tk, sp, rps, RT_DWJ_BLOCKS_SMALLK, RT_DWJ_CAP_SMALLK);
+        for (int i = 0; i < ns; ++i) {
+            const int g = small_of[i];
+            P.tn[g] = tn[i]; P.tk[g] = tk[i]; P.splits[g] = sp[i]; P.rps[g] = rps;
+            blocks_small += static_cast<int64_t>(tn[i]) * tk[i] * sp[i];
+        }
+    }
+    int64_t work = 0, rmax = mlp::DW_R;
+    for (int g = 0; g < n_args; ++g) {
+        if (P.body[g] != 1) continue;
+        P.tn[g] = static_cast<unsigned>((args[g].n + 63) / 64);
+        P.tk[g] = static_cast<unsigned>((args[g].k + 63) / 64);
+        work += args[g].m * P.tn[g] * P.tk[g];
+        rmax = args[g].m > rmax ? args[g].m : rmax;
+    }
+    if (work > 0) {
+        int64_t target = RT_DWJ_SLOTS - blocks_small;
+        target = target > RT_DWJ_MIN_BLOCKS ? target : RT_DWJ_MIN_BLOCKS;
+        int64_t rps = (work + target - 1) / target;
+        rps = (rps + mlp::DW_R - 1) / mlp::DW_R * mlp::DW_R;
+        rmax = (rmax + mlp::DW_R - 1) / mlp::DW_R * mlp::DW_R;
+        for (;; rps += mlp::DW_R) {
+            int64_t blocks = 0;
+            for (int g = 0; g < n_args; ++g)
+                if (P.body[g] == 1) blocks += ((args[g].m + rps - 1) / rps) * P.tn[g] * P.tk[g];
+            if (blocks <= target || rps >= rmax) break;
+        }
+        for (int g = 0; g < n_args; ++g)
+            if (P.body[g] == 1) { P.rps[g] = rps; P.splits[g] = args[g].m > 0 ? (args[g].m + rps - 1) / rps : 0; }
+    }
+    for (int g = 0; g < n_args; ++g) {
+        if (P.body[g] >= 0) continue;
+        int64_t sp = 0;
+        dw_plan(&args[g], 1, args[g].k <= 32, &P.tn[g], &P.tk[g], &sp, P.rps[g]);
+        P.splits[g] = sp;
+    }
+}
+
+static int dwj_validate(const rt_linear_bwd_args* args, int n_args) {
+    if (!args || n_args < 1 || n_args > mlp::DWJ_MAX) return RT_ERR_INVALID;
+    for (int g = 0; g < n_args; ++g) {
+        const int v = validate_bwd(&args[g]);
+        if (v) return v;
+        if (args[g].ids && args[g].prev_mode != 0) return RT_ERR_UNSUPPORTED;
+        if (args[g].fold_src && args[g].fold_in == 1) return RT_ERR_INVALID;
+    }
+    return RT_OK;
+}
+
+#ifdef RT_NO_AIN
+#define RT_DWJ_NO_AIN(args, n_args)                                                        \
+    rt_linear_bwd_args noa[mlp::DWJ_MAX];                                                  \
+    for (int g = 0; g < n_args; ++g) { noa[g] = args[g]; noa[g].a_in = nullptr; }          \
+    args = noa;
+#else
+#define RT_DWJ_NO_AIN(args, n_args)
+#endif
+
+extern "C" int rt_linear_bwd_dw_joint_splits(const rt_linear_bwd_args* args, int n_args, int64_t* splits) {
+    if (!splits) return RT_ERR_INVALID;
+    const int v = dwj_validate(args, n_args);
+    if (v) return v;
+#ifdef RT_NO_DW_PART
+    return RT_ERR_UNSUPPORTED;
+#endif
+    RT_DWJ_NO_AIN(args, n_args)
+    DwJointPlan P;
+    dwj_plan(args, n_args, P);
+    for (int g = 0; g < n_args; ++g) splits[g] = P.splits[g];
+    return RT_OK;
+}
+
+extern "C" int rt_linear_bwd_dw_f32_joint(const rt_linear_bwd_args* args, int n_args, void* stream) {
+    const int v = dwj_validate(args, n_args);
+    if (v) return v;
+    RT_DWJ_NO_AIN(args, n_args)
+    DwJointPlan P;
+    dwj_plan(args, n_args, P);
+    hipStream_t st = as_stream(stream);
+    mlp::DwJointLaunch L{};
+    bool vs = true;
+    size_t lds = 0;
+    int64_t total = 0;
+    for (int body = 0; body < 2; ++body) {
+        for (int g = 0; g < n_args; ++g) {
+            if (P.body[g] != body) continue;
+            const int64_t nb = static_cast<int64_t>(P.tn[g]) * P.tk[g] * P.splits[g];
+            if (nb == 0) continue;
+            total += nb;
+            if (total > (1ll << 30)) return RT_ERR_UNSUPPORTED;
+            const int s = L.nsets++;
+            L.a[s] = args[g];
+            L.rps[s] = P.rps[g];
+            L.tn[s] = P.tn[g];
+            L.tk[s] = P.tk[g];
+            L.end[s] = static_cast<unsigned>(total);
+            L.body[s] = static_cast<unsigned char>(body);
+            size_t need = mlp::dw_lds_floats(body ? 64 : 128, body ? 64 : 32, 0, body == 0) * sizeof(float);
+            if (body == 0) {
+                vs = vs && dw_vec(args[g]);
+                if (args[g].ids && !args[g].a_in) need += static_cast<size_t>(P.rps[g]) * sizeof(int);
+            }
+            lds = need > lds ? need : lds;
+        }
+    }
+    if (total > 0) {
+        const dim3 grid(static_cast<unsigned>(total));
+        if (vs) hipLaunchKernelGGL(mlp::linear_bwd_dw_joint_kernel<true>, grid, dim3(mlp::DW_NT), lds, st, L);
+        else hipLaunchKernelGGL(mlp::linear_bwd_dw_joint_kernel<false>, grid, dim3(mlp::DW_NT), lds, st, L);
+        const int rc = check_launch("linear_bwd_dw_joint_kernel");
+        if (rc) return rc;
+    }
+    for (int g = 0; g < n_args; ++g) {
+        if (P.body[g] >= 0) continue;
+        const int rc = dw_launch(&args[g], 1, dz_fusable(args[g]), st);
+        if (rc) return rc;
+    }
+    return RT_OK;
+}
+
 #ifdef RT_PHASE_PROBE
 extern "C" int rt_probe_setup(void* buf, unsigned cap) {
     unsigned long long* p = static_cast<unsigned long long*>(buf);
diff --git a/real-time-recommendation-system-with-feature-store_amd/csrc/optim.hip b/real-time-recommendation-system-with-feature-store_amd/csrc/optim.hip
--- a/real-time-recommendation-system-with-feature-store_amd/csrc/optim.hip
+++ b/real-time-recommendation-system-with-feature-store_amd/csrc/optim.hip
@@ -34,6 +34,79 @@
     if ((threadIdx.x & 63) == 0) red[threadIdx.x >> 6] = s;
     __syncthreads();
     if (threadIdx.x == 0) atomicAdd(&out[t], red[0] + red[1] + red[2] + red[3]);
+}
+
+constexpr int kFoldBatch = 32;
+struct FoldTable {
+    rt_grad_fold f[RT_GRAD_FOLD_MAX];
+    unsigned first[RT_GRAD_FOLD_MAX + 1];
+    int n;
+};
+
+__global__ __launch_bounds__(256) void grad_sqnorm_fold_kernel(float* __restrict__ g,
+                                                               const int64_t* __restrict__ offsets, int n_tensors,
+                                                               double* __restrict__ out, int32_t* step_counter,
+                                                               int64_t* seed_counter, FoldTable F) {
+    __shared__ double red[4];
+    const int t = blockIdx.y;
+    if (blockIdx.x == 0 && t == 0 && threadIdx.x == 0) {
+        if (step_counter) *step_counter += 1;
+        if (seed_counter) *seed_counter += 1;
+    }
+    double s = 0.0;
+    int dst = t;
+    if (t < n_tensors) {
+#pragma unroll
+        for (int f = 0; f < RT_GRAD_FOLD_MAX; ++f)
+            if (f < F.n && F.f[f].tensor == t) return;
+        const int64_t lo = offsets[t], hi = offsets[t + 1];
+        if (lo + static_cast<int64_t>(blockIdx.x) * kChunk >= hi) return;
+        for (int64_t c0 = lo + static_cast<int64_t>(blockIdx.x) * kChunk; c0 < hi;
+             c0 += static_cast<int64_t>(gridDim.x) * kChunk) {
+            const int64_t c1 = (c0 + kChunk) < hi ? (c0 + kChunk) : hi;
+#pragma unroll 4
+            for (int64_t e = c0 + threadIdx.x; e < c1; e += 256) {
+                const double v = g[e];
+                s += v * v;
+            }
+        }
+    } else {
+        const unsigned fb = static_cast<unsigned>(t - n_tensors) * gridDim.x + blockIdx.x;
+        if (fb >= F.first[RT_GRAD_FOLD_MAX]) return;
+        rt_grad_fold d = F.f[0];
+        unsigned first = 0;
+#pragma unroll
+        for (int f = 1; f < RT_GRAD_FOLD_MAX; ++f)
+            if (f < F.n && fb >= F.first[f]) { d = F.f[f]; first = F.first[f]; }
+        dst = d.tensor;
+        const int64_t n4 = d.words / 4;
+        const int64_t e4 = static_cast<int64_t>(fb - first) * 256 + threadIdx.x;
+        if (e4 < n4) {
+            float4* gp = reinterpret_cast<float4*>(g + d.dst_off) + e4;
+            const float4 g0 = *gp;
+            const float4* p = reinterpret_cast<const float4*>(d.part) + e4;
+            float4 acc = make_float4(0.f, 0.f, 0.f, 0.f);
+            for (int s0 = 0; s0 < d.splits; s0 += kFoldBatch) {
+                float4 v[kFoldBatch];
+#pragma unroll
+                for (int j = 0; j < kFoldBatch; ++j)
+                    v[j] = s0 + j < d.splits ? p[static_cast<int64_t>(s0 + j) * n4] : make_float4(0.f, 0.f, 0.f, 0.f);
+#pragma unroll
+                for (int j = 0; j < kFoldBatch; ++j) {
+                    if (s0 + j == 0) acc = v[0];
+                    else if (s0 + j < d.splits) { acc.x += v[j].x; acc.y += v[j].y; acc.z += v[j].z; acc.w += v[j].w; }
+                }
+            }
+            const float4 o = make_float4(g0.x + acc.x, g0.y + acc.y, g0.z + acc.z, g0.w + acc.w);
+            *gp = o;
+            s = static_cast<double>(o.x) * o.x + static_cast<double>(o.y) * o.y + static_cast<double>(o.z) * o.z +
+                static_cast<double>(o.w) * o.w;
+        }
+    }
+    s = wave_sum(s);
+    if ((threadIdx.x & 63) == 0) red[threadIdx.x >> 6] = s;
+    __syncthreads();
+    if (threadIdx.x == 0) atomicAdd(&out[dst], red[0] + red[1] + red[2] + red[3]);
 }
 
 __global__ __launch_bounds__(256) void clip_adam_kernel(float* __restrict__ p, float* __restrict__ g,
@@ -97,6 +170,34 @@
     return check_launch("grad_sqnorm_kernel");
 }
 
+extern "C" int rt_grad_sqnorm_fold(float* grads, const int64_t* offsets, int n_tensors, double* sumsq_out,
+                                   int32_t* step_counter, int64_t* seed_counter, const rt_grad_fold* folds,
+                                   int n_folds, void* stream) {
+    if (n_tensors < 0 || (n_tensors > 0 && (!grads || !offsets || !sumsq_out))) return RT_ERR_INVALID;
+    if (n_folds < 0 || n_folds > RT_GRAD_FOLD_MAX || (n_folds > 0 && !folds)) return RT_ERR_INVALID;
+    if (n_tensors == 0) return n_folds ? RT_ERR_INVALID : RT_OK;
+    optim::FoldTable F{};
+    F.n = n_folds;
+    unsigned blocks = 0;
+    for (int f = 0; f < n_folds; ++f) {
+        const rt_grad_fold& d = folds[f];
+        if (!d.part || d.words <= 0 || d.words % 4 != 0 || d.dst_off < 0 || d.dst_off % 4 != 0 || d.splits < 1 ||
+            d.tensor < 0 || d.tensor >= n_tensors || (reinterpret_cast<uintptr_t>(d.part) & 15) ||
+            (reinterpret_cast<uintptr_t>(grads) & 15) || d.words > (1ll << 36))
+            return RT_ERR_INVALID;
+        for (int e = 0; e < f; ++e)
+            if (folds[e].tensor == d.tensor) return RT_ERR_INVALID;
+        F.f[f] = d;
+        F.first[f] = blocks;
+        blocks += static_cast<unsigned>((d.words / 4 + 255) / 256);
+    }
+    for (int f = n_folds; f <= RT_GRAD_FOLD_MAX; ++f) F.first[f] = blocks;
+    const dim3 grid(64, static_cast<unsigned>(n_tensors) + (blocks + 63) / 64);
+    hipLaunchKernelGGL(optim::grad_sqnorm_fold_kernel, grid, dim3(256), 0, as_stream(stream), grads, offsets,
+                       n_tensors, sumsq_out, step_counter, seed_counter, F);
+    return check_launch("grad_sqnorm_fold_kernel");
+}
+
 extern "C" int rt_clip_adam_step(float* params, float* grads, float* exp_avg, float* exp_avg_sq, int64_t n,
                                  const double* sumsq, int n_tensors, float max_norm, float lr, const float* lr_dev,
                                  float beta1, float beta2, float eps, float weight_decay, int step,
diff --git a/real-time-recommendation-system-with-feature-store_amd/rtrec_amd/models/fused.py b/real-time-recommendation-system-with-feature-store_amd/rtrec_amd/models/fused.py
--- a/real-time-recommendation-system-with-feature-store_amd/rtrec_amd/models/fused.py
+++ b/real-time-recommendation-system-with-feature-store_amd/rtrec_amd/models/fused.py
@@ -380,23 +380,96 @@
     layers, dsrc, keep = _backward_plan(blocks, ctx, dout, slab, want_dsrc, seed_offset, stats_arena, attach)
     st = _stream(dout)
     groups = [[a] for a in layers]
+    if dw_joint_enabled():
+        _launch_bwd_joint(groups, st, None)
+        return dsrc
     keep += _plan_partials(groups, dout.device)
     for g in groups:
         _launch_bwd(g, st)
     return dsrc
 
 
-def chain_backward_pair(first: tuple, second: tuple) -> None:
+def chain_backward_pair(first: tuple, second: tuple, fold_sink: Optional["FoldSink"] = None) -> None:
     l1, _, keep1 = _backward_plan(*first)
     l2, _, keep2 = _backward_plan(*second)
     st = _stream(first[2])
     if len(l1) == len(l2):
         groups = [[a, b] for a, b in zip(l1, l2)]
+        if dw_joint_enabled():
+            _launch_bwd_joint(groups, st, fold_sink)
+            return
         keep1 += _plan_partials(groups, first[2].device)
     else:
         groups = [[a] for a in l1 + l2]
     for g in groups:
         _launch_bwd(g, st)
+
+
+def dw_joint_enabled() -> bool:
+    lib = native.lib()
+    return (os.environ.get("RTREC_DW_LEGACY", "0") != "1" and hasattr(lib, "rt_linear_bwd_dw_f32_joint")
+            and hasattr(lib, "rt_linear_bwd_dw_joint_splits") and hasattr(lib, "rt_linear_bwd_dz_fused"))
+
+
+class FoldSink:
+
+    def __init__(self, slab: ParamSlab):
+        self.slab = slab
+        self.buf: Optional[torch.Tensor] = None
+        self.retired: list = []
+        self.folds: list = []
+
+    def begin(self) -> None:
+        self.folds = []
+
+    def place(self, sets: list, splits: list) -> None:
+        grad = self.slab.grad
+        index = {o: i for i, o in enumerate(self.slab.offsets)}
+        plan, total = [], 0
+        for a, sp in zip(sets, splits):
+            words = a.n * a.k
+            off = (a.dw - grad.data_ptr()) // 4
+            if sp < 1 or words % 4 or off not in index or len(plan) >= native.GRAD_FOLD_MAX:
+                continue
+            plan.append((a, sp, words, off, total))
+            total += sp * words
+        if self.buf is None or self.buf.numel() < total:
+            if self.buf is not None:
+                self.retired.append(self.buf)
+            self.buf = torch.empty(max(total, 64), dtype=torch.float32, device=grad.device)
+        base = self.buf.data_ptr()
+        for a, sp, words, off, start in plan:
+            a.dw_part = base + 4 * start
+            self.folds.append(native.GradFold(a.dw_part, off, words, sp, index[off]))
+
+
+def _launch_bwd_joint(groups: list, st, sink: Optional[FoldSink]) -> None:
+    lib = native.lib()
+    for g in groups:
+        arr = (LinearBwdArgs * len(g))(*g)
+        if lib.rt_linear_bwd_dz_fused(arr, len(g)):
+            continue
+        for a in g:
+            a.fuse_dz = 0
+        _launch_dz(g, st)
+    sets = [a for g in groups for a in g]
+    chunks = [sets[i:i + native.DW_JOINT_MAX] for i in range(0, len(sets), native.DW_JOINT_MAX)]
+    if sink is not None:
+        cand = {id(a) for g in groups[:-1] for a in g}
+        part_sets, part_splits = [], []
+        for ch in chunks:
+            splits = (ctypes.c_int64 * len(ch))()
+            if lib.rt_linear_bwd_dw_joint_splits((LinearBwdArgs * len(ch))(*ch), len(ch), splits) != 0:
+                continue
+            for a, sp in zip(ch, splits):
+                if id(a) in cand:
+                    part_sets.append(a)
+                    part_splits.append(int(sp))
+        sink.place(part_sets, part_splits)
+    with TIMER.region("linear_bwd_dw", flops=sum(2.0 * a.m * a.k * a.n for a in sets),
+                      bytes_=sum(4.0 * (a.m * a.n + a.m * a.k + a.n * a.k) for a in sets)):
+        for ch in chunks:
+            call("rt_linear_bwd_dw_f32_joint", (LinearBwdArgs * len(ch))(*ch), len(ch), st)
 
 
 def _plan_partials(groups: list, dev) -> list:
@@ -427,18 +500,26 @@
 
 
 def _launch_bwd(group: list, st) -> None:
-    da = [a.g_prev is not None or a.dsrc is not None for a in group]
-    flops = sum((2.0 if d else 0.0) * a.m * a.k * a.n for a, d in zip(group, da))
-    nbytes = sum(4.0 * (3 * a.m * a.n + (2 * a.m * a.k if d else 0) + a.n * a.k) for a, d in zip(group, da))
     arr = (LinearBwdArgs * len(group))(*group)
     lib = native.lib()
     fused = hasattr(lib, "rt_linear_bwd_dz_fused") and lib.rt_linear_bwd_dz_fused(arr, len(group))
     if not fused:
-        with TIMER.region("linear_bwd_dz", flops=flops, bytes_=nbytes):
-            call("rt_linear_bwd_dz_f32_multi", arr, len(group), st)
+        _launch_dz(group, st)
+    _launch_dw(group, st)
+
+
+def _launch_dz(group: list, st) -> None:
+    da = [a.g_prev is not None or a.dsrc is not None for a in group]
+    flops = sum((2.0 if d else 0.0) * a.m * a.k * a.n for a, d in zip(group, da))
+    nbytes = sum(4.0 * (3 * a.m * a.n + (2 * a.m * a.k if d else 0) + a.n * a.k) for a, d in zip(group, da))
+    with TIMER.region("linear_bwd_dz", flops=flops, bytes_=nbytes):
+        call("rt_linear_bwd_dz_f32_multi", (LinearBwdArgs * len(group))(*group), len(group), st)
+
+
+def _launch_dw(group: list, st) -> None:
     with TIMER.region("linear_bwd_dw", flops=sum(2.0 * a.m * a.k * a.n for a in group),
                       bytes_=sum(4.0 * (a.m * a.n + a.m * a.k + a.n * a.k) for a in group)):
-        call("rt_linear_bwd_dw_f32_multi", arr, len(group), st)
+        call("rt_linear_bwd_dw_f32_multi", (LinearBwdArgs * len(group))(*group), len(group), st)
 
 
 def _backward_plan(blocks: List[Block], ctx: ChainCtx, dout: torch.Tensor, slab: ParamSlab,
diff --git a/real-time-recommendation-system-with-feature-store_amd/rtrec_amd/native.py b/real-time-recommendation-system-with-feature-store_amd/rtrec_amd/native.py
--- a/real-time-recommendation-system-with-feature-store_amd/rtrec_amd/native.py
+++ b/real-time-recommendation-system-with-feature-store_amd/rtrec_amd/native.py
@@ -63,6 +63,14 @@
         ("fold_src", vp), ("fold_dst", vp), ("fold_words", c_i64), ("fold_splits", c_int), ("fold_in", c_int),
         ("wt_planes", vp),
     ]
+
+
+class GradFold(ctypes.Structure):
+    _fields_ = [("part", vp), ("dst_off", c_i64), ("words", c_i64), ("splits", c_int), ("tensor", c_int)]
+
+
+GRAD_FOLD_MAX = 8
+DW_JOINT_MAX = 6
 
 
 SIGNATURES = {
@@ -97,6 +105,8 @@
     "rt_linear_fwd_f32_multi": (c_int, [ctypes.POINTER(LinearFwdArgs), c_int, vp]),
     "rt_linear_bwd_dz_f32_multi": (c_int, [ctypes.POINTER(LinearBwdArgs), c_int, vp]),
     "rt_linear_bwd_dw_f32_multi": (c_int, [ctypes.POINTER(LinearBwdArgs), c_int, vp]),
+    "rt_linear_bwd_dw_f32_joint": (c_int, [ctypes.POINTER(LinearBwdArgs), c_int, vp]),
+    "rt_linear_bwd_dw_joint_splits": (c_int, [ctypes.POINTER(LinearBwdArgs), c_int, ctypes.POINTER(c_i64)]),
     "rt_twotower_loss_workspace_bytes": (c_size, [c_i64, c_int]),
     "rt_twotower_loss_fwd_bwd": (c_int, [vp, vp, vp, c_int, c_i64, c_int, c_int, c_f32, vp, vp, c_f32,
                                          c_f32, vp, vp, vp, vp, vp, vp, vp, c_size, vp]),
@@ -106,6 +116,7 @@
     "rt_inbatch_loss_fwd_bwd": (c_int, [vp, vp, c_int, c_i64, c_i64, c_int, c_i64, c_f32, vp, vp, vp, vp, c_size, vp]),
     "rt_similarity_f32": (c_int, [vp, vp, c_i64, c_int, c_f32, vp, vp, vp, vp]),
     "rt_grad_sqnorm": (c_int, [vp, vp, c_int, vp, vp, vp, vp]),
+    "rt_grad_sqnorm_fold": (c_int, [vp, vp, c_int, vp, vp, vp, ctypes.POINTER(GradFold), c_int, vp]),
     "rt_clip_adam_step": (c_int, [vp, vp, vp, vp, c_i64, vp, c_int, c_f32, c_f32, vp, c_f32, c_f32, c_f32,
                                   c_f32, c_int, vp, vp, c_i64, vp]),
     "rt_l2_augment_f32": (c_int, [vp, c_i64, c_int, vp, c_int, c_int, vp]),
diff --git a/real-time-recommendation-system-with-feature-store_amd/rtrec_amd/training/fused_step.py b/real-time-recommendation-system-with-feature-store_amd/rtrec_amd/training/fused_step.py
--- a/real-time-recommendation-system-with-feature-store_amd/rtrec_amd/training/fused_step.py
+++ b/real-time-recommendation-system-with-feature-store_amd/rtrec_amd/training/fused_step.py
@@ -7,7 +7,7 @@
 import torch
 
 from .. import kernels, native
-from ..models.fused import (blocks_from_sequential, chain_backward, chain_backward_pair, chain_forward,
+from ..models.fused import (FoldSink, blocks_from_sequential, chain_backward, chain_backward_pair, chain_forward,
                             chain_forward_pair, stats_arena_size)
 from ..models.two_tower import TwoTowerModel
 from ..native import call, ptr
@@ -46,6 +46,7 @@
         self._sb_user, self._sb_pos, self._sb_neg = (self.dropout_seed * 4 + r for r in (1, 2, 3))
         self._loss_ws: Optional[torch.Tensor] = None
         self._loss_ws_retired = []
+        self._fold = FoldSink(self.slab)
         ua = stats_arena_size(blocks_from_sequential(model.user_tower.mlp))
         ia = stats_arena_size(blocks_from_sequential(model.item_tower.mlp))
         self._arena_sizes = [ua, ia, ia, ua, ia, ia]
@@ -171,9 +172,11 @@
                  ptr(du), ptr(dp), ptr(dq),
                  ptr(slab.grad_of(ubias)) if ubias is not None else None,
                  ptr(slab.grad_of(ibias)) if ibias is not None else None, ptr(ws), ws.numel(), st)
+        self._fold.begin()
         if merged:
             chain_backward_pair((ib, pq, dpq, slab, False, so, self.a_pqb, False),
-                                (ub, u, du, slab, False, so, self.a_ub, False))
+                                (ub, u, du, slab, False, so, self.a_ub, False),
+                                fold_sink=self._fold if self.pg is None else None)
         else:
             s_u.wait_stream(main)
             with torch.cuda.stream(s_u):
@@ -203,16 +206,31 @@
                 self.slab.grad.mul_(1.0 / dist.get_world_size(self.pg))
 
     def _update(self):
+        nb = self.slab.data.numel() * 4.0
+        with TIMER.region("clip_adam", flops=0.0, bytes_=nb * 7):
+            self._fold_norm()
+            self._adam()
+        return self.loss_buf
+
+    def _fold_norm(self):
         slab = self.slab
         st = native.stream_of(slab.data)
-        nb = slab.data.numel() * 4.0
-        with TIMER.region("clip_adam", flops=0.0, bytes_=nb * 7):
+        folds = self._fold.folds
+        if folds:
+            arr = (native.GradFold * len(folds))(*folds)
+            call("rt_grad_sqnorm_fold", ptr(slab.grad), ptr(slab.tensor_offsets()), len(slab.params),
+                 ptr(self.sumsq), ptr(self.step_dev), ptr(self.seed_dev), arr, len(folds), st)
+            self._fold.begin()
+        else:
             call("rt_grad_sqnorm", ptr(slab.grad), ptr(slab.tensor_offsets()), len(slab.params), ptr(self.sumsq),
                  ptr(self.step_dev), ptr(self.seed_dev), st)
-            call("rt_clip_adam_step", ptr(slab.data), ptr(slab.grad), ptr(self.exp_avg), ptr(self.exp_avg_sq),
-                 slab.data.numel(), ptr(self.sumsq), len(slab.params), self.max_norm, self.lr, ptr(self.lr_dev),
-                 self.b1, self.b2, self.eps, self.wd, 1, ptr(self.step_dev), ptr(self.arena), self.arena.numel(), st)
-        return self.loss_buf
+
+    def _adam(self):
+        slab = self.slab
+        st = native.stream_of(slab.data)
+        call("rt_clip_adam_step", ptr(slab.data), ptr(slab.grad), ptr(self.exp_avg), ptr(self.exp_avg_sq),
+             slab.data.numel(), ptr(self.sumsq), len(slab.params), self.max_norm, self.lr, ptr(self.lr_dev),
+             self.b1, self.b2, self.eps, self.wd, 1, ptr(self.step_dev), ptr(self.arena), self.arena.numel(), st)
 
     def __call__(self, user_src: torch.Tensor, pos_src: torch.Tensor, neg_src: Optional[torch.Tensor],
                  user_ids: Optional[torch.Tensor] = None, pos_ids: Optional[torch.Tensor] = None,
```

After: 4.908 billion pairs/s, median of 6. 1.1x the previous value.
